# CityU-AIM-Group/HTD

Hardware: AMD Instinct MI355X
Metric: images/sec (1333x800) HTD-R50 train step (higher is better)
Workload: dtype f32; 1 GPU; HTD ResNet-50 FPN fp32 train step fwd+bwd+SGD, batch 4/GPU @ 1333x800 (padded 1344x800), random-init weights, 2000 RPN proposals/img, 512 RoIs/img/stage; global_batch=4, parallelism=dp1, stage2_positives=158, proposals=random-init RPN (few positives: the regression branch is nearly idle)

## Files before the change

htd_amd/csrc/conv_x3.hip:

```cpp
#include <algorithm>
#include <mutex>
#include <type_traits>
#include <unordered_map>

#include <stdlib.h>

#include "common.h"

namespace {

using f32x16 = __attribute__((ext_vector_type(16))) float;
using bf16x8 = __attribute__((ext_vector_type(8))) __bf16;
using bf16x2 = __attribute__((ext_vector_type(2))) __bf16;
using f32x2 = __attribute__((ext_vector_type(2))) float;
using f32x4 = __attribute__((ext_vector_type(4))) float;

using f16x8 = __attribute__((ext_vector_type(8))) _Float16;
using f16x2 = __attribute__((ext_vector_type(2))) _Float16;

constexpr int XK = 16;
constexpr int NCH = 6;

struct H2Scale { float s, inv; };
__device__ __forceinline__ H2Scale h2_scale(const float *amax)
// ... 9 lines not shown
    c.v = __builtin_convertvector(f32x2{a, b}, f16x2);
    h = c.u;
    const f32x2 back = __builtin_convertvector(c.v, f32x2);
    c.v = __builtin_convertvector(f32x2{a - back[0], b - back[1]}, f16x2);
    l = c.u;
}

__device__ __forceinline__ void split3x2(float a, float b, unsigned &h, unsigned &m, unsigned &l)
{
    union { bf16x2 v; unsigned u; } c;
    c.v = __builtin_convertvector(f32x2{a, b}, bf16x2);
    h = c.u;
    const float ra = a - __uint_as_float(h << 16), rb = b - __uint_as_float(h & 0xffff0000u);
    c.v = __builtin_convertvector(f32x2{ra, rb}, bf16x2);
    m = c.u;
    c.v = __builtin_convertvector(f32x2{ra - __uint_as_float(m << 16), rb - __uint_as_float(m & 0xffff0000u)}, bf16x2);
    l = c.u;
}

#ifndef HTD_X3P_EARLY
#define HTD_X3P_EARLY 1
#endif
#ifndef HTD_X3H_NB
#define HTD_X3H_NB 2
#endif
#ifndef HTD_X3H_FRAG_FIRST
#define HTD_X3H_FRAG_FIRST 1
#endif
#ifndef HTD_X3H_OCC4
#define HTD_X3H_OCC4 0
#endif

template <int N>
__device__ __forceinline__ void wait_vm()
{
    asm volatile("s_waitcnt vmcnt(%0)" ::"n"(N) : "memory");
}
__device__ __forceinline__ void landed(f32x4 &a) { asm volatile("" : "+v"(a)::"memory"); }

__device__ __forceinline__ void lds_dma16(const void *src, unsigned lds_dst)
{
    unsigned keep;
    asm volatile("s_mov_b32 %0, m0\n\ts_mov_b32 m0, %2\n\ts_nop 0\n\tglobal_load_lds_dwordx4 %1, off\n\ts_mov_b32 m0, %0"
                 : "=&s"(keep)
                 : "v"(src), "s"(lds_dst)
                 : "memory");
}

using u32x2 = __attribute__((ext_vector_type(2))) unsigned;
template <int OFF>
__device__ __forceinline__ void lds_store8(unsigned addr, unsigned lo, unsigned hi)
{
    const u32x2 v = {lo, hi};
    asm volatile("ds_write_b64 %0, %1 offset:%2" ::"v"(addr), "v"(v), "n"(OFF) : "memory");
}

struct X3Params {
    const float *x;
    const uint4 *wp;
    const float *bias, *residual, *mask_src;
    float *y;
    int Hx, Wx;
    int Ho, Wo;
    int Ci, Co, Cop;
    int kh;
    int stride;
    int ntl;
    int tl_dy[9], tl_dx[9], tl_w[9];
    int o_step, o_h0, o_w0, oH, oW;
    int relu;
    int res_H, res_W;
    float res_sh, res_sw;
    int64_t M;
    int mt, nt;
    int ncs;
    int tiles_a, splits_a, sps_a, splits_b, sps_b;
    int64_t m_rem0;
    float *partial;
    const uint4 *xp;
    uint4 *yp;
    int64_t xp_rows, yp_rows;
    const float *amax, *wscale;
    float *amax_out;
};

__device__ __forceinline__ void block_absmax_out(float mx, float *out, float *red, unsigned seen)
{
    unsigned bits = (mx != mx) ? 0x7fc00000u : __float_as_uint(mx);
    for (int o = 32; o > 0; o >>= 1) bits = max(bits, (unsigned)__shfl_xor((int)bits, o));
    __syncthreads();
    if ((threadIdx.x & 63) == 0) reinterpret_cast<unsigned *>(red)[threadIdx.x >> 6] = bits;
    __syncthreads();
    if (threadIdx.x == 0) {
        const unsigned *r = reinterpret_cast<const unsigned *>(red);
        bits = max(max(r[0], r[1]), max(r[2], r[3]));
        if (bits > seen) __hip_atomic_fetch_max(reinterpret_cast<unsigned *>(out), bits, __ATOMIC_RELAXED, __HIP_MEMORY_SCOPE_AGENT);
    }
}
__device__ __forceinline__ void wave_absmax_out(float mx, float *out, unsigned seen)
{
    unsigned bits = (mx != mx) ? 0x7fc00000u : __float_as_uint(mx);
    for (int o = 32; o > 0; o >>= 1) bits = max(bits, (unsigned)__shfl_xor((int)bits, o));
    if ((threadIdx.x & 63) == 0 && bits > seen)
        __hip_atomic_fetch_max(reinterpret_cast<unsigned *>(out), bits, __ATOMIC_RELAXED, __HIP_MEMORY_SCOPE_AGENT);
}
__device__ __forceinline__ float absmax4(float mx, float4 v)
{
    const float m = fmaxf(fmaxf(fabsf(v.x), fabsf(v.y)), fmaxf(fabsf(v.z), fabsf(v.w)));
    const bool nan = (v.x != v.x) | (v.y != v.y) | (v.z != v.z) | (v.w != v.w);
    return nan ? __uint_as_float(0x7fc00000u) : ((mx != mx) ? mx : fmaxf(mx, m));
}

__device__ __forceinline__ void emit_planes4(uint4 *yp, int64_t rows, int64_t m, int n, float4 v)
{
    unsigned h0, m0, l0, h1, m1, l1;
    split3x2(v.x, v.y, h0, m0, l0);
    split3x2(v.z, v.w, h1, m1, l1);
    char *d = reinterpret_cast<char *>(yp + ((int64_t)(n >> 4) * NCH + ((n >> 3) & 1)) * rows + m) + ((n >> 2) & 1) * 8;
    *reinterpret_cast<uint2 *>(d) = make_uint2(h0, h1);
    *reinterpret_cast<uint2 *>(d + 2 * rows * 16) = make_uint2(m0, m1);
    *reinterpret_cast<uint2 *>(d + 4 * rows * 16) = make_uint2(l0, l1);
}

template <int BM, int KW>
struct Geo {
    static constexpr int RUN = BM + KW - 1;
    static constexpr int PITCH = ((RUN + 1 + 3) / 8) * 8 + 4;
    static constexpr int PASSES = (RUN + 63) / 64;
};

__device__ __forceinline__ int64_t x3_out_off(const X3Params &p, int64_t m, int n)
{
    if (p.o_step == 0) return m * p.Co + n;
    const unsigned mm = (unsigned)m, wo = mm % (unsigned)p.Wo, t = mm / (unsigned)p.Wo;
    const unsigned ho = t % (unsigned)p.Ho, b = t / (unsigned)p.Ho;
    return (((int64_t)b * p.oH + p.o_h0 + p.o_step * (int)ho) * p.oW + p.o_w0 + p.o_step * (int)wo) * p.Co + n;
}

template <int WGM, int WGN, int TM, int TN, bool MF16, typename Acc>
__device__ __forceinline__ void x3_epilogue(const X3Params &p, Acc &acc, uint4 *lds, int64_t m0, int n0, bool part, bool region_b,
                                            int split)
{
    constexpr int BN = WGN * TN * 32;
    constexpr int EPI_STRIDE = BN + 4, EPI_ROWS = WGM * 32;
    constexpr int RBLK = MF16 ? 16 : 32;
    constexpr int CB = TN * 32 / RBLK;
    const int tid = threadIdx.x, lane = tid & 63, wave = tid >> 6;
    const int wm = wave / WGN, wn = wave % WGN;
    const int frow = lane & 31, fhalf = lane >> 5;
    const int lrow = MF16 ? (lane & 15) : frow;
    const int kg = lane >> 4;
    float *le = reinterpret_cast<float *>(lds);
    const bool vec_ok = (p.Co & 3) == 0;
    constexpr int V = BN / 4, RPP = 256 / V;
    float omax = 0.f;
    const unsigned oseen = (p.amax_out != nullptr && !part) ? *reinterpret_cast<const volatile unsigned *>(p.amax_out) : 0u;
    const bool scaled = p.wscale != nullptr;
    float4 cscale = make_float4(1.f, 1.f, 1.f, 1.f);
    if (scaled) {
        const float ia = h2_scale(p.amax).inv;
        const float4 w4 = *reinterpret_cast<const float4 *>(p.wscale + n0 + (tid % V) * 4);
        cscale = make_float4(w4.x * ia, w4.y * ia, w4.z * ia, w4.w * ia);
    }
#pragma unroll
    for (int i = 0; i < TM; ++i) {
        if constexpr (MF16) {
#pragma unroll
            for (int ib = 0; ib < 2; ++ib)
#pragma unroll
                for (int j = 0; j < CB; ++j)
#pragma unroll
                    for (int r = 0; r < 4; ++r)
                        le[(wm * 32 + ib * 16 + 4 * kg + r) * EPI_STRIDE + wn * TN * 32 + j * 16 + lrow] = acc[2 * i + ib][j][r];
        } else {
#pragma unroll
            for (int j = 0; j < TN; ++j)
#pragma unroll
                for (int r = 0; r < 16; ++r) {
                    const int row = wm * 32 + (r & 3) + 8 * (r >> 2) + 4 * fhalf;
                    le[row * EPI_STRIDE + (wn * TN + j) * 32 + frow] = acc[i][j][r];
                }
        }
        __syncthreads();
        const int c4 = tid % V;
        const int n = n0 + c4 * 4;
        constexpr int NPASS = EPI_ROWS / RPP;
        if (vec_ok && !part && p.res_H == 0) {
            const bool col_ok = n < p.Co;
            float4 bv = make_float4(0.f, 0.f, 0.f, 0.f);
            if (p.bias != nullptr && col_ok) bv = *reinterpret_cast<const float4 *>(p.bias + n);
            constexpr int UB = NPASS < 4 ? NPASS : 4;
#pragma unroll
            for (int pass0 = 0; pass0 < NPASS; pass0 += UB) {
                float4 v[UB], rv[UB], mv[UB];
                int64_t o[UB];
                bool ok[UB];
#pragma unroll
                for (int u = 0; u < UB; ++u) {
                    const int row = tid / V + (pass0 + u) * RPP;
                    const int64_t m = m0 + ((row >> 5) * TM + i) * 32 + (row & 31);
                    ok[u] = m < p.M && col_ok;
                    o[u] = x3_out_off(p, ok[u] ? m : 0, n) & -(int64_t)ok[u];
                    v[u] = *reinterpret_cast<const float4 *>(le + row * EPI_STRIDE + c4 * 4);
                    if (scaled) { v[u].x *= cscale.x; v[u].y *= cscale.y; v[u].z *= cscale.z; v[u].w *= cscale.w; }
                }
                if (p.residual != nullptr) {
#pragma unroll
                    for (int u = 0; u < UB; ++u) rv[u] = *reinterpret_cast<const float4 *>(p.residual + o[u]);
                }
                if (p.mask_src != nullptr) {
#pragma unroll
                    for (int u = 0; u < UB; ++u) mv[u] = *reinterpret_cast<const float4 *>(p.mask_src + o[u]);
                }
#pragma unroll
                for (int u = 0; u < UB; ++u) { v[u].x += bv.x; v[u].y += bv.y; v[u].z += bv.z; v[u].w += bv.w; }
                if (p.residual != nullptr) {
#pragma unroll
                    for (int u = 0; u < UB; ++u) { v[u].x += rv[u].x; v[u].y += rv[u].y; v[u].z += rv[u].z; v[u].w += rv[u].w; }
                }
                if (p.relu) {
#pragma unroll
                    for (int u = 0; u < UB; ++u) {
                        v[u].x = fmaxf(v[u].x, 0.f); v[u].y = fmaxf(v[u].y, 0.f); v[u].z = fmaxf(v[u].z, 0.f); v[u].w = fmaxf(v[u].w, 0.f);
                    }
                }
                if (p.mask_src != nullptr) {
#pragma unroll
                    for (int u = 0; u < UB; ++u) {
                        v[u].x = mv[u].x > 0.f ? v[u].x : 0.f; v[u].y = mv[u].y > 0.f ? v[u].y : 0.f;
                        v[u].z = mv[u].z > 0.f ? v[u].z : 0.f; v[u].w = mv[u].w > 0.f ? v[u].w : 0.f;
                    }
                }
#pragma unroll
                for (int u = 0; u < UB; ++u)
                    if (ok[u]) {
                        *reinterpret_cast<float4 *>(p.y + o[u]) = v[u];
                        omax = absmax4(omax, v[u]);
                    }
                if (p.yp != nullptr) {
#pragma unroll
                    for (int u = 0; u < UB; ++u) {
                        const int row = tid / V + (pass0 + u) * RPP;
                        if (ok[u]) emit_planes4(p.yp, p.yp_rows, m0 + ((row >> 5) * TM + i) * 32 + (row & 31), n, v[u]);
                    }
                }
            }
            if (i + 1 < TM) __syncthreads();
            continue;
        }
#pragma unroll
        for (int pass = 0; pass < NPASS; ++pass) {
            const int row = tid / V + pass * RPP;
            const int64_t m = m0 + ((row >> 5) * TM + i) * 32 + (row & 31);
            if (m >= p.M || n >= p.Co) continue;
            float4 v = *reinterpret_cast<const float4 *>(le + row * EPI_STRIDE + c4 * 4);
            if (scaled) { v.x *= cscale.x; v.y *= cscale.y; v.z *= cscale.z; v.w *= cscale.w; }
            const int64_t o = x3_out_off(p, m, n);
            if (part) {
                float *dst = region_b ? p.partial + (p.splits_a > 1 ? (int64_t)p.splits_a * p.m_rem0 * p.Co : 0) +
                                            ((int64_t)split * (p.M - p.m_rem0) + (m - p.m_rem0)) * p.Co + n
                                      : p.partial + ((int64_t)split * p.m_rem0 + m) * p.Co + n;
                if (vec_ok) *reinterpret_cast<float4 *>(dst) = v;
                else {
                    dst[0] = v.x;
                    if (n + 1 < p.Co) dst[1] = v.y;
                    if (n + 2 < p.Co) dst[2] = v.z;
                    if (n + 3 < p.Co) dst[3] = v.w;
                }
                continue;
            }
            if (vec_ok) {
                if (p.bias) {
                    const float4 bv = *reinterpret_cast<const float4 *>(p.bias + n);
                    v.x += bv.x; v.y += bv.y; v.z += bv.z; v.w += bv.w;
                }
                if (p.residual) {
                    int64_t ro = o;
                    if (p.res_H > 0) {
                        const unsigned mm = (unsigned)m, wo = mm % (unsigned)p.Wo, t = mm / (unsigned)p.Wo;
                        const unsigned ho = t % (unsigned)p.Ho, b = t / (unsigned)p.Ho;
                        const int rh = min((int)floorf(ho * p.res_sh), p.res_H - 1);
                        const int rw = min((int)floorf(wo * p.res_sw), p.res_W - 1);
                        ro = (((int64_t)b * p.res_H + rh) * p.res_W + rw) * p.Co + n;
                    }
                    const float4 rv = *reinterpret_cast<const float4 *>(p.residual + ro);
                    v.x += rv.x; v.y += rv.y; v.z += rv.z; v.w += rv.w;
                }
                if (p.relu) { v.x = fmaxf(v.x, 0.f); v.y = fmaxf(v.y, 0.f); v.z = fmaxf(v.z, 0.f); v.w = fmaxf(v.w, 0.f); }
                if (p.mask_src) {
                    const float4 mv = *reinterpret_cast<const float4 *>(p.mask_src + o);
                    v.x = mv.x > 0.f ? v.x : 0.f; v.y = mv.y > 0.f ? v.y : 0.f;
                    v.z = mv.z > 0.f ? v.z : 0.f; v.w = mv.w > 0.f ? v.w : 0.f;
                }
                *reinterpret_cast<float4 *>(p.y + o) = v;
                omax = absmax4(omax, v);
                if (p.yp != nullptr) emit_planes4(p.yp, p.yp_rows, m, n, v);
            } else {
                auto put = [&](int e, float t) {
                    if (n + e >= p.Co) return;
                    t += p.bias ? p.bias[n + e] : 0.f;
                    if (p.residual) t += p.residual[o + e];
                    if (p.relu) t = fmaxf(t, 0.f);
                    if (p.mask_src) t = p.mask_src[o + e] > 0.f ? t : 0.f;
                    p.y[o + e] = t;
                    omax = absmax4(omax, make_float4(t, 0.f, 0.f, 0.f));
                };
                put(0, v.x); put(1, v.y); put(2, v.z); put(3, v.w);
            }
        }
        if (i + 1 < TM) __syncthreads();
    }
    if (p.amax_out != nullptr && !part) block_absmax_out(omax, p.amax_out, le, oseen);
}

template <int WGM, int WGN, int TM, int TN, int KW, int NB, bool H2 = false>
constexpr int x3p_occupancy()
{
    constexpr int BM = WGM * TM * 32, BN = WGN * TN * 32;
    constexpr int NCHL = H2 ? 4 : NCH;
    constexpr int main_bytes = (2 * NCHL * Geo<BM, KW>::PITCH + NB * NCHL * BN) * 16;
    constexpr int epi_bytes = WGM * 32 * (BN + 4) * 4;
    constexpr int by_lds = 163840 / (main_bytes > epi_bytes ? main_bytes : epi_bytes);
    constexpr int by_regs = TM * TN >= 4 ? (H2 && HTD_X3H_OCC4 ? 4 : 3) : 4;
    return by_lds < by_regs ? by_lds : by_regs;
}

template <int WGM, int WGN, int TM, int TN, int KW, bool MF16, int NB, bool H2 = false>
__global__ __launch_bounds__(256, (x3p_occupancy<WGM, WGN, TM, TN, KW, NB, H2>())) void conv_x3p_kernel(X3Params p)
{
    static_assert(!(H2 && MF16), "H2: 32x32x16 form only");
    constexpr int NCHL = H2 ? 4 : NCH;
    constexpr int BM = WGM * TM * 32, BN = WGN * TN * 32;
    using G = Geo<BM, KW>;
    constexpr int PADX = (KW - 1) / 2;
    constexpr int A_VEC = NCHL * G::PITCH;
    constexpr int B_VEC = NCHL * BN;
    constexpr int MAIN_VEC = 2 * A_VEC + NB * B_VEC;
    constexpr int EPI_STRIDE = BN + 4, EPI_ROWS = WGM * 32;
    constexpr int EPI_VEC = EPI_ROWS * EPI_STRIDE / 4;
    constexpr int LDS_VEC = MAIN_VEC > EPI_VEC ? MAIN_VEC : EPI_VEC;
    __shared__ uint4 lds[LDS_VEC];
    uint4 *const lA = lds, *const lB = lds + 2 * A_VEC;
    const unsigned lds_a0 = (unsigned)(size_t)(__attribute__((address_space(3))) void *)lA;

    int bid = blockIdx.x, split = 0, sps = 0;
    bool part = false;
    const bool region_b = bid >= p.tiles_a * p.splits_a;
    if (region_b) {
        const int r = bid - p.tiles_a * p.splits_a;
        bid = p.tiles_a + r / p.splits_b;
        split = r % p.splits_b;
        part = p.splits_b > 1;
        sps = p.sps_b;
    } else if (p.splits_a > 1) {
        split = bid % p.splits_a;
        bid = bid / p.splits_a;
        part = true;
        sps = p.sps_a;
    } else {
        const int q = p.tiles_a / 8, r = p.tiles_a % 8, xcd = bid % 8, idx = bid / 8;
        bid = (xcd < r ? xcd * (q + 1) : r * (q + 1) + (xcd - r) * q) + idx;
    }
    const int tile_m = bid / p.nt, tile_n = bid % p.nt;
    const int64_t m0 = (int64_t)tile_m * BM;
    const int n0 = tile_n * BN;

    const int tid = threadIdx.x, lane = tid & 63, wave = tid >> 6;
    const int wm = wave / WGN, wn = wave % WGN;
    const int frow = lane & 31, fhalf = lane >> 5;
    const int PADY = (p.kh - 1) / 2;

    const int vcol = tid & 3, vrow = tid >> 2;
    const int a_g0 = (int)m0 + vrow - PADX;
    unsigned a_off[KW > 1 ? 1 : G::PASSES];
    bool a_in[KW > 1 ? 1 : G::PASSES];
    unsigned a_tm[KW > 1 ? 1 : G::PASSES];
    if constexpr (KW > 1) {
        a_off[0] = (unsigned)a_g0 * (unsigned)p.Ci + vcol * 4;
        a_in[0] = true;
        a_tm[0] = 0u;
    } else {
#pragma unroll
        for (int i = 0; i < G::PASSES; ++i) {
            const int64_t m = m0 + vrow + 64 * i;
            a_in[i] = vrow + 64 * i < G::RUN && m < p.M;
            const unsigned mm = a_in[i] ? (unsigned)m : 0u;
            const unsigned wo = mm % (unsigned)p.Wo, t = mm / (unsigned)p.Wo;
            const unsigned ho = t % (unsigned)p.Ho, b = t / (unsigned)p.Ho;
            a_off[i] = ((b * (unsigned)p.Hx + ho * (unsigned)p.stride) * (unsigned)p.Wx + wo * (unsigned)p.stride) *
                           (unsigned)p.Ci + vcol * 4;
            unsigned tm = 0x1ffu;
            if (p.ntl > 0) {
                tm = 0u;
                const int hb = (int)(ho * (unsigned)p.stride), wb = (int)(wo * (unsigned)p.stride);
                for (int q = 0; q < p.ntl; ++q)
                    tm |= ((unsigned)(hb + p.tl_dy[q]) < (unsigned)p.Hx && (unsigned)(wb + p.tl_dx[q]) < (unsigned)p.Wx) ? (1u << q) : 0u;
            }
            a_tm[i] = tm;
        }
    }

    constexpr int RBLK = MF16 ? 16 : 32;
    constexpr int RB = TM * 32 / RBLK, CB = TN * 32 / RBLK;
    const int lrow = MF16 ? (lane & 15) : frow;
    const int kg = lane >> 4;
    unsigned vmask[RB];
    const int a_frag0 = (wm * TM * 32 + lrow) * 16;
#pragma unroll
    for (int i = 0; i < RB; ++i) {
        const int r = wm * TM * 32 + i * RBLK + lrow;
        vmask[i] = 0xffffffffu;
// ... 262 lines not shown

    int bbuf = 0, abuf = 0, kx = 0;
    int n1shift = (ky1 - PADY) * p.Wx, n1koff = tap_koff(ky1, cs1);
    int n2shift = (ky2 - PADY) * p.Wx, n2koff = tap_koff(ky2, cs2);
    auto tap = [&](int P, bool TAIL) __attribute__((always_inline)) {
        const bool more = s + 1 < s_end, more2 = s + 2 < s_end;
        if constexpr (H2 && HTD_X3H_FRAG_FIRST) mma_tap(abuf, bbuf, kx, ky * KW, 0);
        const bool issued = issue_b();
        if (!TAIL) {
            if constexpr (KW == 1) {
#pragma unroll
                for (int i = 0; i < NP; ++i) load_pass(ky2, n2koff, i, P * NP + i, more2);
            } else {
                const bool last = kx == KW - 1;
                load_pass(last ? n2shift : n1shift, last ? n2koff : n1koff, last ? 0 : kx + 1, P, last ? more2 : more);
            }
        }
        if constexpr (EARLY) {
            if (TAIL) wait_vm<0>();
            else if (issued) wait_vm<NPT + NI_MIN>();
            else wait_vm<NPT>();
#pragma unroll
            for (int i = 0; i < NPT; ++i) landed(ra[(P ^ 1) * NPT + i]);
            mma_tap(abuf, bbuf, kx, ky * KW, (H2 && HTD_X3H_FRAG_FIRST) ? 1 : 2);
            if constexpr (KW == 1) {
#pragma unroll
                for (int i = 0; i < NP; ++i) store_pass(abuf ^ 1, i, (P ^ 1) * NP + i);
            } else {
                store_pass(abuf ^ 1, kx, P ^ 1);
            }
            constexpr int NM = RB * CB * ((MF16 || H2) ? 3 : 6);
            constexpr int PER = (NPT * 36 + NM - 1) / NM;
            __builtin_amdgcn_sched_group_barrier(0x002, 4, 0);
#pragma unroll
            for (int e = 0; e < NM; ++e) {
                __builtin_amdgcn_sched_group_barrier(0x008, 1, 0);
                __builtin_amdgcn_sched_group_barrier(0x002, PER, 0);
            }
            if (!TAIL) {
                if (DIST >= 2 && issued) wait_vm<NPT + NI_MIN>();
                else wait_vm<NPT>();
            }
        } else {
            mma_tap(abuf, bbuf, kx, ky * KW, (H2 && HTD_X3H_FRAG_FIRST) ? 1 : 2);
            if (TAIL) wait_vm<0>();
            else wait_tap(issued);
#pragma unroll
            for (int i = 0; i < NPT; ++i) landed(ra[(P ^ 1) * NPT + i]);
            if (more) {
                if constexpr (KW == 1) {
#pragma unroll
                    for (int i = 0; i < NP; ++i) store_pass(abuf ^ 1, i, (P ^ 1) * NP + i);
                } else {
                    store_pass(abuf ^ 1, kx, P ^ 1);
                }
            }
        }
        lds_barrier();
        bbuf = bbuf + 1 == NB ? 0 : bbuf + 1;
        if (++kx == KW) {
            kx = 0;
            ++s;
            abuf ^= 1;
            cs = cs1; ky = ky1;
            cs1 = cs2; ky1 = ky2;
            if (++ky2 == p.kh) { ky2 = 0; ++cs2; }
            n1shift = n2shift; n1koff = n2koff;
            n2shift = (ky2 - PADY) * p.Wx;
            n2koff = tap_koff(ky2, cs2);
        }
    };
    const int taps_total = (s_end - s_begin) * KW;
    int t = 0;
#pragma unroll 1
    for (; t + 1 < taps_total; t += 2) {
        tap(0, false);
        tap(1, false);
    }
    if (t < taps_total) tap(0, true);
    wait_vm<0>();
#pragma unroll
    for (int i = 0; i < 2 * NPT; ++i) landed(ra[i]);

    x3_epilogue<WGM, WGN, TM, TN, MF16>(p, acc, lds, m0, n0, part, region_b, split);
}

template <int WGM, int WGN, int TM, int TN, int NS>
constexpr int x3q_occupancy()
{
    constexpr int BM = WGM * TM * 32, BN = WGN * TN * 32;
    constexpr int main_bytes = NS * NCH * (BM + BN) * 16;
    constexpr int epi_bytes = WGM * 32 * (BN + 4) * 4;
    constexpr int by_lds = 163840 / (main_bytes > epi_bytes ? main_bytes : epi_bytes);
    constexpr int by_regs = TM * TN >= 4 ? 3 : 4;
    return by_lds < by_regs ? by_lds : by_regs;
}

template <int WGM, int WGN, int TM, int TN, bool MF16, int NS>
__global__ __launch_bounds__(256, (x3q_occupancy<WGM, WGN, TM, TN, NS>())) void conv_x3q_kernel(X3Params p)
{
    constexpr int BM = WGM * TM * 32, BN = WGN * TN * 32;
    constexpr int A_VEC = NCH * BM, B_VEC = NCH * BN;
    constexpr int MAIN_VEC = NS * (A_VEC + B_VEC);
    constexpr int EPI_VEC = WGM * 32 * (BN + 4) / 4;
    constexpr int LDS_VEC = MAIN_VEC > EPI_VEC ? MAIN_VEC : EPI_VEC;
    __shared__ uint4 lds[LDS_VEC];
    uint4 *const lA = lds, *const lB = lds + NS * A_VEC;
    const unsigned lds_a0 = (unsigned)(size_t)(__attribute__((address_space(3))) void *)lA;
    const unsigned lds_b0 = (unsigned)(size_t)(__attribute__((address_space(3))) void *)lB;

    int bid = blockIdx.x, split = 0, sps = 0;
    bool part = false;
    const bool region_b = bid >= p.tiles_a * p.splits_a;
    if (region_b) {
        const int r = bid - p.tiles_a * p.splits_a;
        bid = p.tiles_a + r / p.splits_b;
        split = r % p.splits_b;
        part = p.splits_b > 1;
        sps = p.sps_b;
    } else if (p.splits_a > 1) {
        split = bid % p.splits_a;
        bid = bid / p.splits_a;
        part = true;
        sps = p.sps_a;
    } else {
        const int q = p.tiles_a / 8, r = p.tiles_a % 8, xcd = bid % 8, idx = bid / 8;
        bid = (xcd < r ? xcd * (q + 1) : r * (q + 1) + (xcd - r) * q) + idx;
    }
    const int tile_m = bid / p.nt, tile_n = bid % p.nt;
    const int64_t m0 = (int64_t)tile_m * BM;
    const int n0 = tile_n * BN;

    const int tid = threadIdx.x, lane = tid & 63, wave = tid >> 6;
    const int wm = wave / WGN, wn = wave % WGN;
    const int frow = lane & 31, fhalf = lane >> 5;
    constexpr int RBLK = MF16 ? 16 : 32;
    constexpr int RB = TM * 32 / RBLK, CB = TN * 32 / RBLK;
    const int lrow = MF16 ? (lane & 15) : frow;
    const int kg = lane >> 4;
    const int a_row = (wm * TM * 32 + lrow) * 16;
    const int a_c0 = (MF16 ? kg * BM * 16 : fhalf * BM * 16) + a_row;
    const int a_c1 = MF16 ? ((kg >> 1) * 4 + (kg & 1)) * BM * 16 + a_row : 0;
    const int b_row = (wn * TN * 32 + lrow) * 16;
    const int b_c0 = (MF16 ? kg * BN * 16 : fhalf * BN * 16) + b_row;
    const int b_c1 = MF16 ? ((1 - (kg >> 1)) * 2 + (kg & 1)) * BN * 16 + b_row : 0;
    const int b_c2 = MF16 ? (((kg >> 1) ? 0 : 4) + (kg & 1)) * BN * 16 + b_row : 0;

    const int total_steps = p.ncs;
    const int s_begin = part ? split * sps : 0;
    const int s_end = part ? min(total_steps, s_begin + sps) : total_steps;

    constexpr int NIA = NCH * BM / 64, NIB = NCH * BN / 64, NI = NIA + NIB, NIW = (NI + 3) / 4;
    const int wave_u = __builtin_amdgcn_readfirstlane(wave);
    const uint4 *src[NIW];
    unsigned dst[NIW], adv[NIW];
#pragma unroll
    for (int k = 0; k < NIW; ++k) {
        const int idx = wave_u + 4 * k;
        if (idx < NIA) {
            const int chunk = idx / (BM / 64), half = idx % (BM / 64);
            src[k] = p.xp + (int64_t)chunk * p.xp_rows + m0 + half * 64 + lane;
            dst[k] = lds_a0 + (unsigned)((chunk * BM + half * 64) * 16);
            adv[k] = (unsigned)(NCH * p.xp_rows);
        } else {
            const int j = (idx < NI ? idx : NIA) - NIA, chunk = j / (BN / 64), half = j % (BN / 64);
            src[k] = p.wp + (int64_t)chunk * p.Cop + n0 + half * 64 + lane;
            dst[k] = lds_b0 + (unsigned)((chunk * BN + half * 64) * 16);
            adv[k] = (unsigned)(NCH * p.Cop);
        }
    }
    auto issue = [&](int s, int stage) __attribute__((always_inline)) {
#pragma unroll
        for (int k = 0; k < NIW; ++k) {
            const int idx = wave_u + 4 * k;
            if (NI % 4 != 0 && idx >= NI) continue;
            const unsigned st = (unsigned)stage * (unsigned)((idx < NIA ? A_VEC : B_VEC) * 16);
            lds_dma16(src[k] + (int64_t)s * adv[k], dst[k] + st);
        }
    };
    auto lds_barrier = [&]() {
        asm volatile("s_waitcnt lgkmcnt(0)" ::: "memory");
        __builtin_amdgcn_s_barrier();
        asm volatile("" ::: "memory");
    };

    using acc_t = typename std::conditional<MF16, f32x4, f32x16>::type;
    acc_t acc[RB][CB];
#pragma unroll
    for (int i = 0; i < RB; ++i)
#pragma unroll
        for (int j = 0; j < CB; ++j)
#pragma unroll
            for (int r = 0; r < (MF16 ? 4 : 16); ++r) acc[i][j][r] = 0.f;

    auto mma = [&](int stage) __attribute__((always_inline)) {
        const char *la = reinterpret_cast<const char *>(lA + stage * A_VEC);
        const char *lb = reinterpret_cast<const char *>(lB + stage * B_VEC);
        if constexpr (MF16) {
            bf16x8 fa01[RB], fa02[RB];
#pragma unroll
            for (int i = 0; i < RB; ++i) {
                fa01[i] = *reinterpret_cast<const bf16x8 *>(la + a_c0 + i * 16 * 16);
                fa02[i] = *reinterpret_cast<const bf16x8 *>(la + a_c1 + i * 16 * 16);
            }
#pragma unroll
            for (int j = 0; j < CB; ++j) {
                const bf16x8 fb01 = *reinterpret_cast<const bf16x8 *>(lb + b_c0 + j * 16 * 16);
                const bf16x8 fb10 = *reinterpret_cast<const bf16x8 *>(lb + b_c1 + j * 16 * 16);
                const bf16x8 fb20 = *reinterpret_cast<const bf16x8 *>(lb + b_c2 + j * 16 * 16);
#pragma unroll
                for (int i = 0; i < RB; ++i) {
                    acc[i][j] = __builtin_amdgcn_mfma_f32_16x16x32_bf16(fa02[i], fb20, acc[i][j], 0, 0, 0);
                    acc[i][j] = __builtin_amdgcn_mfma_f32_16x16x32_bf16(fa01[i], fb10, acc[i][j], 0, 0, 0);
                    acc[i][j] = __builtin_amdgcn_mfma_f32_16x16x32_bf16(fa01[i], fb01, acc[i][j], 0, 0, 0);
                }
            }
        } else {
            bf16x8 fa[RB][3], fb[CB][3];
#pragma unroll
            for (int i = 0; i < RB; ++i)
#pragma unroll
                for (int q = 0; q < 3; ++q) fa[i][q] = *reinterpret_cast<const bf16x8 *>(la + a_c0 + i * 32 * 16 + q * 2 * BM * 16);
#pragma unroll
            for (int j = 0; j < CB; ++j)
#pragma unroll
                for (int q = 0; q < 3; ++q) fb[j][q] = *reinterpret_cast<const bf16x8 *>(lb + b_c0 + j * 32 * 16 + q * 2 * BN * 16);
#pragma unroll
            for (int i = 0; i < RB; ++i)
#pragma unroll
                for (int j = 0; j < CB; ++j) {
                    acc[i][j] = __builtin_amdgcn_mfma_f32_32x32x16_bf16(fa[i][2], fb[j][0], acc[i][j], 0, 0, 0);
                    acc[i][j] = __builtin_amdgcn_mfma_f32_32x32x16_bf16(fa[i][0], fb[j][2], acc[i][j], 0, 0, 0);
                    acc[i][j] = __builtin_amdgcn_mfma_f32_32x32x16_bf16(fa[i][1], fb[j][1], acc[i][j], 0, 0, 0);
                    acc[i][j] = __builtin_amdgcn_mfma_f32_32x32x16_bf16(fa[i][1], fb[j][0], acc[i][j], 0, 0, 0);
                    acc[i][j] = __builtin_amdgcn_mfma_f32_32x32x16_bf16(fa[i][0], fb[j][1], acc[i][j], 0, 0, 0);
                    acc[i][j] = __builtin_amdgcn_mfma_f32_32x32x16_bf16(fa[i][0], fb[j][0], acc[i][j], 0, 0, 0);
                }
        }
    };

    constexpr int KEEP = (NS - 2) * (NI / 4);
#pragma unroll
    for (int d = 0; d < NS - 1; ++d)
        if (s_begin + d < s_end) issue(s_begin + d, d);
    if (s_begin + NS - 2 < s_end) wait_vm<KEEP>();
    else wait_vm<0>();
    lds_barrier();
    int stage = 0, pstage = NS - 1;
#pragma unroll 1
    for (int s = s_begin; s < s_end; ++s) {
        const bool more = s + NS - 1 < s_end;
        if (more) issue(s + NS - 1, pstage);
        mma(stage);
        if (more) wait_vm<KEEP>();
        else wait_vm<0>();
        lds_barrier();
        stage = stage + 1 == NS ? 0 : stage + 1;
        pstage = pstage + 1 == NS ? 0 : pstage + 1;
    }
    x3_epilogue<WGM, WGN, TM, TN, MF16>(p, acc, lds, m0, n0, part, region_b, split);
}

__global__ __launch_bounds__(256) void conv_x3p_splitk_epilogue_kernel(X3Params p)
{
    const int64_t lo = p.splits_a > 1 ? 0 : p.m_rem0 * p.Co, hi = p.splits_b > 1 ? p.M * p.Co : p.m_rem0 * p.Co;
    const int64_t na = p.m_rem0 * p.Co, nb = (p.M - p.m_rem0) * p.Co;
    const float *pb = p.partial + (p.splits_a > 1 ? (int64_t)p.splits_a * na : 0);
    float omax = 0.f;
    const unsigned oseen = p.amax_out != nullptr ? *reinterpret_cast<const volatile unsigned *>(p.amax_out) : 0u;
    for (int64_t o = lo + (int64_t)blockIdx.x * blockDim.x + threadIdx.x; o < hi; o += (int64_t)gridDim.x * blockDim.x) {
        float v = 0.f;
        if (o < na) {
            for (int k = 0; k < p.splits_a; ++k) v += p.partial[(int64_t)k * na + o];
        } else {
            for (int k = 0; k < p.splits_b; ++k) v += pb[(int64_t)k * nb + (o - na)];
        }
        const int n = (int)(o % p.Co);
        if (p.bias) v += p.bias[n];
        if (p.residual) {
            int64_t ro = p.o_step == 0 ? o : x3_out_off(p, o / p.Co, n);
            if (p.res_H > 0) {
                const int64_t m = o / p.Co;
                const unsigned mm = (unsigned)m, wo = mm % (unsigned)p.Wo, t = mm / (unsigned)p.Wo;
                const unsigned ho = t % (unsigned)p.Ho, b = t / (unsigned)p.Ho;
                const int rh = min((int)floorf(ho * p.res_sh), p.res_H - 1);
                const int rw = min((int)floorf(wo * p.res_sw), p.res_W - 1);
                ro = (((int64_t)b * p.res_H + rh) * p.res_W + rw) * p.Co + n;
            }
            v += p.residual[ro];
        }
        if (p.relu) v = fmaxf(v, 0.f);
        const int64_t oo = p.o_step == 0 ? o : x3_out_off(p, o / p.Co, n);
        if (p.mask_src) v = p.mask_src[oo] > 0.f ? v : 0.f;
        p.y[oo] = v;
        omax = absmax4(omax, make_float4(v, 0.f, 0.f, 0.f));
    }
    __shared__ float ored[4];
    if (p.amax_out != nullptr) block_absmax_out(omax, p.amax_out, ored, oseen);
}

__global__ __launch_bounds__(256) void conv_x3p_splitk_epilogue_vec_kernel(X3Params p)
{
    const int C4 = p.Co >> 2;
    const int64_t lo = p.splits_a > 1 ? 0 : p.m_rem0 * C4, hi = p.splits_b > 1 ? p.M * C4 : p.m_rem0 * C4;
    const int64_t na = p.m_rem0 * C4, nb = (p.M - p.m_rem0) * C4;
    const float4 *pa = reinterpret_cast<const float4 *>(p.partial);
    const float4 *pb = pa + (p.splits_a > 1 ? (int64_t)p.splits_a * na : 0);
    float omax = 0.f;
    const unsigned oseen = p.amax_out != nullptr ? *reinterpret_cast<const volatile unsigned *>(p.amax_out) : 0u;
    for (int64_t q = lo + (int64_t)blockIdx.x * blockDim.x + threadIdx.x; q < hi; q += (int64_t)gridDim.x * blockDim.x) {
        float4 v = make_float4(0.f, 0.f, 0.f, 0.f);
        const bool in_a = q < na;
        const float4 *src = in_a ? pa + q : pb + (q - na);
        const int64_t stride = in_a ? na : nb;
        const int splits = in_a ? p.splits_a : p.splits_b;
#pragma unroll 4
        for (int k = 0; k < splits; ++k) {
            const float4 t = src[(int64_t)k * stride];
            v.x += t.x; v.y += t.y; v.z += t.z; v.w += t.w;
        }
        const unsigned m = (unsigned)(q / C4), n = (unsigned)(q - (int64_t)m * C4) * 4u;
        const int64_t o = x3_out_off(p, (int64_t)m, (int)n);
        if (p.bias) {
            const float4 bv = *reinterpret_cast<const float4 *>(p.bias + n);
            v.x += bv.x; v.y += bv.y; v.z += bv.z; v.w += bv.w;
        }
        if (p.residual) {
            int64_t ro = o;
            if (p.res_H > 0) {
                const unsigned wo = m % (unsigned)p.Wo, t = m / (unsigned)p.Wo;
                const unsigned ho = t % (unsigned)p.Ho, b = t / (unsigned)p.Ho;
                const int rh = min((int)floorf(ho * p.res_sh), p.res_H - 1);
                const int rw = min((int)floorf(wo * p.res_sw), p.res_W - 1);
                ro = (((int64_t)b * p.res_H + rh) * p.res_W + rw) * p.Co + n;
            }
            const float4 rv = *reinterpret_cast<const float4 *>(p.residual + ro);
            v.x += rv.x; v.y += rv.y; v.z += rv.z; v.w += rv.w;
        }
        if (p.relu) { v.x = fmaxf(v.x, 0.f); v.y = fmaxf(v.y, 0.f); v.z = fmaxf(v.z, 0.f); v.w = fmaxf(v.w, 0.f); }
        if (p.mask_src) {
            const float4 mv = *reinterpret_cast<const float4 *>(p.mask_src + o);
            v.x = mv.x > 0.f ? v.x : 0.f; v.y = mv.y > 0.f ? v.y : 0.f;
            v.z = mv.z > 0.f ? v.z : 0.f; v.w = mv.w > 0.f ? v.w : 0.f;
        }
        *reinterpret_cast<float4 *>(p.y + o) = v;
        omax = absmax4(omax, v);
        if (p.yp != nullptr) emit_planes4(p.yp, p.yp_rows, (int64_t)m, (int)n, v);
    }
    __shared__ float ored[4];
    if (p.amax_out != nullptr) block_absmax_out(omax, p.amax_out, ored, oseen);
}

__device__ __forceinline__ void x3_planes_element(const float *__restrict__ w, uint4 *__restrict__ out, int Co, int taps,
                                                  int Ci, int Np, int transposed, int64_t e)
{
    const int N = transposed ? Ci : Co, K = transposed ? Co : Ci;
    const int ncs = K / XK;
    const int n = (int)(e % Np);
    const int64_t t2 = e / Np;
    const int cs = (int)(t2 % ncs), tap = (int)(t2 / ncs);
    float v[XK];
    if (n < N) {
        if (!transposed) {
            const float4 *src = reinterpret_cast<const float4 *>(w + ((int64_t)n * taps + tap) * Ci + cs * XK);
#pragma unroll
            for (int q = 0; q < 4; ++q) {
                const float4 f = src[q];
                v[4 * q] = f.x; v[4 * q + 1] = f.y; v[4 * q + 2] = f.z; v[4 * q + 3] = f.w;
            }
        } else {
#pragma unroll
            for (int k = 0; k < XK; ++k) v[k] = w[((int64_t)(cs * XK + k) * taps + (taps - 1 - tap)) * Ci + n];
        }
    } else {
#pragma unroll
        for (int k = 0; k < XK; ++k) v[k] = 0.f;
    }
    unsigned pl[3][8];
#pragma unroll
    for (int k = 0; k < 8; ++k) split3x2(v[2 * k], v[2 * k + 1], pl[0][k], pl[1][k], pl[2][k]);
    uint4 *dst = out + ((int64_t)(tap * ncs + cs) * NCH) * Np + n;
#pragma unroll
    for (int q = 0; q < 3; ++q)
#pragma unroll
        for (int h = 0; h < 2; ++h)
            dst[(int64_t)(q * 2 + h) * Np] = make_uint4(pl[q][4 * h], pl[q][4 * h + 1], pl[q][4 * h + 2], pl[q][4 * h + 3]);
}

__global__ __launch_bounds__(256) void x3_planes_kernel(const float *__restrict__ w, uint4 *__restrict__ out, int Co, int taps,
                                                        int Ci, int Np, int transposed)
{
    const int K = transposed ? Co : Ci;
    const int64_t total = (int64_t)taps * (K / XK) * Np;
    for (int64_t e = (int64_t)blockIdx.x * 256 + threadIdx.x; e < total; e += (int64_t)gridDim.x * 256)
        x3_planes_element(w, out, Co, taps, Ci, Np, transposed, e);
}

struct PlanesDesc {
    const float *w;
    uint4 *out;
    int Co, taps, Ci, transposed;
    int64_t block0;
};

__global__ __launch_bounds__(256) void x3_planes_many_kernel(const PlanesDesc *__restrict__ descs, int n)
{
    int lo = 0, hi = n - 1;
    const int64_t b = blockIdx.x;
// ... 344 lines not shown
    if (g_xtable.empty()) return -1;
    const auto it = g_xtable.find(XKey{M, Co, Ci, taps, epi});
    return it == g_xtable.end() ? -1 : it->second;
}

int choose_cfg(int64_t M, int Co, int Ci, int taps, int epi)
{
    int cfg = forced_cfg();
    if (cfg < 0) cfg = table_cfg(M, Co, Ci, taps, epi);
    if (cfg >= 0) return cfg;
    float best = -1.f;
    static const int cand[4] = {1, 3, 2, 0};
    for (int c : cand) {
        const float sc = cfg_score(c, M, Co);
        if (sc > best * 1.005f) { best = sc; cfg = c; }
    }
    return cfg;
}

static const int g_x3p_mfma = getenv("HTD_X3P_MFMA") ? atoi(getenv("HTD_X3P_MFMA")) : 0;
int x3p_mfma()
{
    if (!g_x3p_tune) return g_x3p_mfma;
    const char *e = getenv("HTD_X3P_MFMA");
    return e ? atoi(e) : 0;
}

int x3p_nb()
{
    if (!g_x3p_tune) return 0;
    const char *e = getenv("HTD_X3P_NB");
    return e ? atoi(e) : 0;
}

template <int TM, int TN, int NB>
void launch_tile_nb(const X3Params &p, int kw, dim3 grid, hipStream_t s)
{
    const int mf = x3p_mfma() ? x3p_mfma() : (kw == 1 ? 16 : 32);
    if (mf == 32) {
        if (kw == 1) hipLaunchKernelGGL((conv_x3p_kernel<2, 2, TM, TN, 1, false, NB>), grid, dim3(256), 0, s, p);
        else hipLaunchKernelGGL((conv_x3p_kernel<2, 2, TM, TN, 3, false, NB>), grid, dim3(256), 0, s, p);
    } else {
        if (kw == 1) hipLaunchKernelGGL((conv_x3p_kernel<2, 2, TM, TN, 1, true, NB>), grid, dim3(256), 0, s, p);
        else hipLaunchKernelGGL((conv_x3p_kernel<2, 2, TM, TN, 3, true, NB>), grid, dim3(256), 0, s, p);
    }
}

template <int TM, int TN>
void launch_tile(const X3Params &p, int kw, dim3 grid, hipStream_t s)
{
#ifdef HTD_X3P_DEEP
    const int nb = x3p_nb();
    if (nb == 3) return launch_tile_nb<TM, TN, 3>(p, kw, grid, s);
    if (nb >= 4) return launch_tile_nb<TM, TN, 4>(p, kw, grid, s);
#endif
    launch_tile_nb<TM, TN, 2>(p, kw, grid, s);
}

static const int g_x3q_mfma = getenv("HTD_X3Q_MFMA") ? atoi(getenv("HTD_X3Q_MFMA")) : 0;
static const int g_x3q_ns = getenv("HTD_X3Q_NS") ? atoi(getenv("HTD_X3Q_NS")) : 0;
int x3q_env(const char *name, int at_load)
{
    if (!g_x3p_tune) return at_load;
    const char *e = getenv(name);
    return e ? atoi(e) : 0;
}

template <int TM, int TN>
void launch_tile_q(const X3Params &p, dim3 grid, hipStream_t s)
{
    const int mf = x3q_env("HTD_X3Q_MFMA", g_x3q_mfma), ns = x3q_env("HTD_X3Q_NS", g_x3q_ns);
    if (mf != 32) {
        if (ns == 3) hipLaunchKernelGGL((conv_x3q_kernel<2, 2, TM, TN, true, 3>), grid, dim3(256), 0, s, p);
        else hipLaunchKernelGGL((conv_x3q_kernel<2, 2, TM, TN, true, 2>), grid, dim3(256), 0, s, p);
    } else {
        if (ns == 3) hipLaunchKernelGGL((conv_x3q_kernel<2, 2, TM, TN, false, 3>), grid, dim3(256), 0, s, p);
        else hipLaunchKernelGGL((conv_x3q_kernel<2, 2, TM, TN, false, 2>), grid, dim3(256), 0, s, p);
    }
}

int launch_x3p(X3Params p, int kw, hipStream_t s, void *workspace)
{
    const int total_steps = p.ncs * p.kh;
    const int epi = (p.residual ? 1 : 0) | (p.mask_src ? 2 : 0) | (p.amax ? 4 : 0);
    const int cfg = choose_cfg(p.M, p.Co, p.Ci, p.kh * kw + (p.ntl > 0 ? 100 : 0), epi);
    const XPlan pl = plan_x3p(cfg, p.M, p.Co, total_steps, kw, workspace != nullptr);
    p.tiles_a = pl.tiles_a; p.splits_a = pl.splits_a; p.sps_a = pl.sps_a; p.splits_b = pl.splits_b; p.sps_b = pl.sps_b;
    p.m_rem0 = pl.m_rem0;
    p.partial = (float *)workspace;
    p.mt = (int)htd::ceil_div(p.M, kXCfg[cfg].bm);
    p.nt = (int)htd::ceil_div(p.Co, kXCfg[cfg].bn);
    HTD_REQUIRE(pl.grid > 0 && pl.grid < (1ll << 31), "conv2d_x3p: bad grid");
    const dim3 grid((unsigned)pl.grid);
    if (p.amax != nullptr && kw == 3) {
        switch (cfg) {
        case 0: hipLaunchKernelGGL((conv_x3p_kernel<2, 2, 1, 1, 3, false, HTD_X3H_NB, true>), grid, dim3(256), 0, s, p); break;
        case 1: hipLaunchKernelGGL((conv_x3p_kernel<2, 2, 2, 2, 3, false, HTD_X3H_NB, true>), grid, dim3(256), 0, s, p); break;
        case 2: hipLaunchKernelGGL((conv_x3p_kernel<2, 2, 2, 1, 3, false, HTD_X3H_NB, true>), grid, dim3(256), 0, s, p); break;
        default: hipLaunchKernelGGL((conv_x3p_kernel<2, 2, 1, 2, 3, false, HTD_X3H_NB, true>), grid, dim3(256), 0, s, p); break;
        }
    } else if (p.amax != nullptr) {
        switch (cfg) {
        case 0: hipLaunchKernelGGL((conv_x3p_kernel<2, 2, 1, 1, 1, false, HTD_X3H_NB, true>), grid, dim3(256), 0, s, p); break;
        case 1: hipLaunchKernelGGL((conv_x3p_kernel<2, 2, 2, 2, 1, false, HTD_X3H_NB, true>), grid, dim3(256), 0, s, p); break;
        case 2: hipLaunchKernelGGL((conv_x3p_kernel<2, 2, 2, 1, 1, false, HTD_X3H_NB, true>), grid, dim3(256), 0, s, p); break;
        default: hipLaunchKernelGGL((conv_x3p_kernel<2, 2, 1, 2, 1, false, HTD_X3H_NB, true>), grid, dim3(256), 0, s, p); break;
        }
    } else if (p.xp != nullptr) {
        switch (cfg) {
        case 0: launch_tile_q<1, 1>(p, grid, s); break;
        case 1: launch_tile_q<2, 2>(p, grid, s); break;
        case 2: launch_tile_q<2, 1>(p, grid, s); break;
        default: launch_tile_q<1, 2>(p, grid, s); break;
        }
    } else {
        switch (cfg) {
        case 0: launch_tile<1, 1>(p, kw, grid, s); break;
        case 1: launch_tile<2, 2>(p, kw, grid, s); break;
        case 2: launch_tile<2, 1>(p, kw, grid, s); break;
        default: launch_tile<1, 2>(p, kw, grid, s); break;
        }
    }
    if (pl.partial_floats > 0) {
        const int64_t rows = (p.splits_a > 1 ? p.m_rem0 : 0) + (p.splits_b > 1 ? p.M - p.m_rem0 : 0);
        if ((p.Co & 3) == 0) {
            const unsigned rb = (unsigned)std::min<int64_t>(htd::ceil_div(rows * (p.Co >> 2), 256), p.amax_out ? 1024 : 4096);
            hipLaunchKernelGGL(conv_x3p_splitk_epilogue_vec_kernel, dim3(rb), dim3(256), 0, s, p);
        } else {
            const unsigned rb = (unsigned)std::min<int64_t>(htd::ceil_div(rows * p.Co, 256), p.amax_out ? 1024 : 4096);
            hipLaunchKernelGGL(conv_x3p_splitk_epilogue_kernel, dim3(rb), dim3(256), 0, s, p);
        }
    }
    return htd::check_launch("conv2d_x3p");
}

bool x3h_strided_ok(int Ci, int Co, int kh, int kw, int stride, int pad)
{
    static const bool on = !(getenv("HTD_X3H_STRIDED") && atoi(getenv("HTD_X3H_STRIDED")) == 0);
    return on && Ci % XK == 0 && Co >= 33 && kh == 3 && kw == 3 && stride == 2 && pad == 1;
}

bool x3p_shape_ok(int Ci, int Co, int kh, int kw, int stride, int pad, int dil)
{
    if (Ci % XK != 0 || Co < 33 || dil != 1 || kh != kw) return false;
    if (kh == 1) return pad == 0 && stride >= 1;
    return kh == 3 && stride == 1 && pad == 1;
}

}

extern "C" int htd_conv2d_x3p_supported(int Ci, int Co, int kh, int kw, int stride, int pad, int dil)
{
    return (!x3p_off() && htd::conv_math() == 1 && x3p_shape_ok(Ci, Co, kh, kw, stride, pad, dil)) ? 1 : 0;
}

int g_conv_h2 = getenv("HTD_CONV_H2") ? atoi(getenv("HTD_CONV_H2")) : 1;
extern "C" int htd_conv2d_set_h2(int on)
{
    const int prev = g_conv_h2;
    if (on == 0 || on == 1) g_conv_h2 = on;
    return prev;
}
extern "C" int htd_conv2d_x3h_supported(int Ci, int Co, int kh, int kw, int stride, int pad, int dil)
{
    return (g_conv_h2 == 1 && htd_conv2d_x3p_supported(Ci, Co, kh, kw, stride, pad, dil)) ? 1 : 0;
}
extern "C" int htd_conv2d_x3h_strided_supported(int Ci, int Co, int kh, int kw, int stride, int pad, int dil)
{
    return (g_conv_h2 == 1 && !x3p_off() && htd::conv_math() == 1 && dil == 1 && x3h_strided_ok(Ci, Co, kh, kw, stride, pad)) ? 1 : 0;
}

extern "C" int htd_conv2d_x3p_tile_table_set(int64_t M, int Co, int Ci, int taps, int epi, int cfg)
{
    HTD_REQUIRE(M > 0 && Co > 0 && Ci > 0 && taps > 0 && epi >= 0 && epi < 8 && cfg < 4,
                "x3p_tile_table_set: bad entry M=%lld Co=%d Ci=%d taps=%d epi=%d cfg=%d", (long long)M, Co, Ci, taps, epi, cfg);
    std::lock_guard<std::mutex> lock(g_xtable_mutex);
    if (cfg < 0) g_xtable.erase(XKey{M, Co, Ci, taps, epi});
// ... 72 lines not shown
                       (const PlanesDescH *)desc, n);
    return htd::check_launch("x3h_planes_many");
}

extern "C" int htd_absmax(const float *x, int64_t n, float *amax, void *stream)
{
    HTD_REQUIRE(x && amax && n > 0 && ((uintptr_t)x & 15) == 0, "absmax: bad arguments");
    const unsigned blocks = (unsigned)std::min<int64_t>(htd::ceil_div(n >> 2, (int64_t)256 * 8) + 1, 2048);
    hipLaunchKernelGGL(absmax_kernel, dim3(blocks), dim3(256), 0, (hipStream_t)stream, x, n, (unsigned *)amax);
    return htd::check_launch("absmax");
}

extern "C" int htd_conv2d_x3_planes_many(const void *desc, int n, int64_t total_blocks, void *stream)
{
    static_assert(sizeof(PlanesDesc) == 40, "PlanesDesc layout is part of the ABI");
    HTD_REQUIRE(desc && n > 0 && total_blocks > 0 && total_blocks < (1ll << 31), "x3_planes_many: bad arguments");
    hipLaunchKernelGGL(x3_planes_many_kernel, dim3((unsigned)total_blocks), dim3(256), 0, (hipStream_t)stream,
                       (const PlanesDesc *)desc, n);
    return htd::check_launch("x3_planes_many");
}

extern "C" int64_t htd_conv2d_x3p_workspace_bytes(int64_t M, int Co, int Ci, int kh, int kw)
{
    int64_t need = 0;
    for (int cfg = 0; cfg < 4; ++cfg) need = std::max(need, plan_x3p(cfg, M, Co, (Ci / XK) * kh, kw, true).partial_floats * 4);
    return need;
}

extern "C" int64_t htd_act_planes_rows(int64_t M) { return M > 0 ? act_rows(M) : 0; }

extern "C" int64_t htd_act_planes_bytes(int64_t M, int C)
{
    if (M <= 0 || C <= 0 || C % XK != 0) return 0;
    return (int64_t)(C / XK) * NCH * act_rows(M) * 16;
}

extern "C" int htd_act_planes(const float *x, void *planes, int64_t M, int C, void *stream)
{
    HTD_REQUIRE(x && planes && M > 0 && C > 0 && C % XK == 0, "act_planes: bad arguments (C %% 16)");
    const unsigned blocks = (unsigned)std::min<int64_t>(htd::ceil_div(M * (C >> 3), (int64_t)256), 65536);
    hipLaunchKernelGGL(act_planes_kernel, dim3(blocks), dim3(256), 0, (hipStream_t)stream, x, (uint4 *)planes, M, C, act_rows(M));
    return htd::check_launch("act_planes");
}

extern "C" int htd_conv2d_fwd_x3q(const float *x, const void *xplanes, const void *wplanes, const float *bias,
                                  const float *residual, int res_h, int res_w, float *y, void *yplanes, float *amax_out, int B, int H,
                                  int W, int Ci, int Co, int kh, int kw, int stride, int pad, int relu, void *workspace, void *stream)
{
    HTD_REQUIRE((x || xplanes) && wplanes && y && B > 0 && H > 0 && W > 0, "conv2d_fwd_x3q: bad arguments");
    HTD_REQUIRE(x3p_shape_ok(Ci, Co, kh, kw, stride, pad, 1), "conv2d_fwd_x3q: unsupported layer Ci=%d Co=%d k=%dx%d s=%d p=%d", Ci,
                Co, kh, kw, stride, pad);
    HTD_REQUIRE(!xplanes || (kh == 1 && stride == 1), "conv2d_fwd_x3q: input planes serve 1x1 / stride-1 layers only");
    HTD_REQUIRE(!yplanes || Co % XK == 0, "conv2d_fwd_x3q: output planes need Co %% 16 == 0 (Co=%d)", Co);
    HTD_REQUIRE((res_h > 0) == (res_w > 0) && res_h >= 0 && (res_h == 0 || ((Co & 3) == 0 && residual)),
                "conv2d_fwd_x3q: bad residual up-sampling arguments");
    X3Params p{};
    p.x = x; p.wp = (const uint4 *)wplanes; p.bias = bias; p.residual = residual; p.y = y;
    p.Hx = H; p.Wx = W;
    p.Ho = (H + 2 * pad - kh) / stride + 1;
    p.Wo = (W + 2 * pad - kw) / stride + 1;
    p.Ci = Ci; p.Co = Co; p.Cop = planes_np(Co); p.kh = kh; p.stride = stride; p.relu = relu;
    p.M = (int64_t)B * p.Ho * p.Wo;
    p.ncs = Ci / XK;
    p.xp = (const uint4 *)xplanes; p.xp_rows = act_rows(p.M);
    p.yp = (uint4 *)yplanes; p.yp_rows = act_rows(p.M);
    p.amax_out = amax_out;
    HTD_REQUIRE((int64_t)B * H * W * Ci < (1ll << 31) && p.M * Co < (1ll << 40), "conv2d_fwd_x3q: operand too large");
    if (res_h > 0) {
        p.res_H = res_h; p.res_W = res_w;
        p.res_sh = (float)res_h / (float)p.Ho; p.res_sw = (float)res_w / (float)p.Wo;
    }
    return launch_x3p(p, kw, (hipStream_t)stream, workspace);
}

extern "C" int htd_conv2d_fwd_x3p(const float *x, const void *wplanes, const float *bias, const float *residual, int res_h,
                                  int res_w, float *y, int B, int H, int W, int Ci, int Co, int kh, int kw, int stride, int pad,
                                  int relu, void *workspace, void *stream)
{
    HTD_REQUIRE(x, "conv2d_fwd_x3p: bad arguments");
    return htd_conv2d_fwd_x3q(x, nullptr, wplanes, bias, residual, res_h, res_w, y, nullptr, nullptr, B, H, W, Ci, Co, kh, kw, stride,
                              pad, relu, workspace, stream);
}

extern "C" int htd_conv2d_bwd_data_x3q(const float *gy, const void *gyplanes, const void *wplanesT, const float *mask_src,
                                       const float *accum, float *gx, void *gxplanes, float *amax_out, int B, int H, int W, int Ci,
                                       int Co, int kh, int kw, int pad, void *workspace, void *stream)
{
    HTD_REQUIRE((gy || gyplanes) && wplanesT && gx && B > 0 && H > 0 && W > 0, "conv2d_bwd_data_x3q: bad arguments");
    HTD_REQUIRE(x3p_shape_ok(Co, Ci, kh, kw, 1, pad, 1), "conv2d_bwd_data_x3q: unsupported layer Ci=%d Co=%d k=%dx%d p=%d", Ci, Co,
                kh, kw, pad);
    HTD_REQUIRE(!gyplanes || kh == 1, "conv2d_bwd_data_x3q: gradient planes serve 1x1 layers only");
    HTD_REQUIRE(!gxplanes || Ci % XK == 0, "conv2d_bwd_data_x3q: output planes need Ci %% 16 == 0 (Ci=%d)", Ci);
    X3Params p{};
    p.x = gy; p.wp = (const uint4 *)wplanesT; p.residual = accum; p.mask_src = mask_src; p.y = gx;
    p.Hx = H; p.Wx = W; p.Ho = H; p.Wo = W;
    p.Ci = Co; p.Co = Ci; p.Cop = planes_np(Ci); p.kh = kh; p.stride = 1;
    p.M = (int64_t)B * H * W;
    p.ncs = Co / XK;
    p.xp = (const uint4 *)gyplanes; p.xp_rows = act_rows(p.M);
    p.yp = (uint4 *)gxplanes; p.yp_rows = act_rows(p.M);
    p.amax_out = amax_out;
    HTD_REQUIRE((int64_t)B * H * W * Co < (1ll << 31), "conv2d_bwd_data_x3q: operand too large");
    return launch_x3p(p, kw, (hipStream_t)stream, workspace);
}

extern "C" int htd_conv2d_bwd_data_x3p(const float *gy, const void *wplanesT, const float *mask_src, const float *accum,
                                       float *gx, int B, int H, int W, int Ci, int Co, int kh, int kw, int pad, void *workspace,
                                       void *stream)
{
    HTD_REQUIRE(gy, "conv2d_bwd_data_x3p: bad arguments");
    return htd_conv2d_bwd_data_x3q(gy, nullptr, wplanesT, mask_src, accum, gx, nullptr, nullptr, B, H, W, Ci, Co, kh, kw, pad,
                                   workspace, stream);
}

extern "C" int htd_conv2d_fwd_x3h(const float *x, const float *amax, const void *wplanes, const float *bias, const float *residual,
                                  int res_h, int res_w, float *y, void *yplanes, float *amax_out, int B, int H, int W, int Ci,
                                  int Co, int kh, int kw, int stride, int pad, int relu, void *workspace, void *stream)
{
    HTD_REQUIRE(!yplanes || Co % XK == 0, "conv2d_fwd_x3h: output planes need Co %% 16 == 0 (Co=%d)", Co);
    HTD_REQUIRE(x && amax && wplanes && y && B > 0 && H > 0 && W > 0, "conv2d_fwd_x3h: bad arguments");
    const bool taps = x3h_strided_ok(Ci, Co, kh, kw, stride, pad);
    HTD_REQUIRE(taps || x3p_shape_ok(Ci, Co, kh, kw, stride, pad, 1), "conv2d_fwd_x3h: unsupported layer Ci=%d Co=%d k=%dx%d s=%d p=%d",
                Ci, Co, kh, kw, stride, pad);
    HTD_REQUIRE(!taps || (!yplanes && res_h == 0), "conv2d_fwd_x3h: strided 3x3 layers write no planes and take no up-sampled residual");
    HTD_REQUIRE((res_h > 0) == (res_w > 0) && res_h >= 0 && (res_h == 0 || ((Co & 3) == 0 && residual)),
                "conv2d_fwd_x3h: bad residual up-sampling arguments");
    X3Params p{};
    p.x = x; p.wp = (const uint4 *)wplanes; p.bias = bias; p.residual = residual; p.y = y;
    p.Hx = H; p.Wx = W;
    p.Ho = (H + 2 * pad - kh) / stride + 1;
    p.Wo = (W + 2 * pad - kw) / stride + 1;
    p.Ci = Ci; p.Co = Co; p.Cop = planes_np(Co); p.kh = kh; p.stride = stride; p.relu = relu;
    p.M = (int64_t)B * p.Ho * p.Wo;
    p.ncs = Ci / XK;
    p.amax = amax;
    p.wscale = reinterpret_cast<const float *>(p.wp + planes_vec(kh * kw, Ci, p.Cop));
    p.yp = (uint4 *)yplanes; p.yp_rows = act_rows(p.M);
    p.amax_out = amax_out;
    HTD_REQUIRE((int64_t)B * H * W * Ci < (1ll << 31) && p.M * Co < (1ll << 40), "conv2d_fwd_x3h: operand too large");
    if (res_h > 0) {
        p.res_H = res_h; p.res_W = res_w;
        p.res_sh = (float)res_h / (float)p.Ho; p.res_sw = (float)res_w / (float)p.Wo;
    }
    if (taps) {
        p.kh = p.ntl = kh * kw;
        for (int t = 0; t < p.ntl; ++t) { p.tl_dy[t] = t / kw - pad; p.tl_dx[t] = t % kw - pad; p.tl_w[t] = t; }
        return launch_x3p(p, 1, (hipStream_t)stream, workspace);
    }
    return launch_x3p(p, kw, (hipStream_t)stream, workspace);
}

extern "C" int htd_conv2d_bwd_data_x3h(const float *gy, const float *amax, const void *wplanesT, const float *mask_src,
                                       const float *accum, float *gx, void *gxplanes, float *amax_out, int B, int H, int W,
                                       int Ci, int Co, int kh, int kw, int pad, void *workspace, void *stream)
{
    HTD_REQUIRE(!gxplanes || Ci % XK == 0, "conv2d_bwd_data_x3h: output planes need Ci %% 16 == 0 (Ci=%d)", Ci);
    HTD_REQUIRE(gy && amax && wplanesT && gx && B > 0 && H > 0 && W > 0, "conv2d_bwd_data_x3h: bad arguments");
    HTD_REQUIRE(x3p_shape_ok(Co, Ci, kh, kw, 1, pad, 1), "conv2d_bwd_data_x3h: unsupported layer Ci=%d Co=%d k=%dx%d p=%d", Ci, Co, kh,
                kw, pad);
    X3Params p{};
    p.x = gy; p.wp = (const uint4 *)wplanesT; p.residual = accum; p.mask_src = mask_src; p.y = gx;
    p.Hx = H; p.Wx = W; p.Ho = H; p.Wo = W;
    p.Ci = Co; p.Co = Ci; p.Cop = planes_np(Ci); p.kh = kh; p.stride = 1;
    p.M = (int64_t)B * H * W;
    p.ncs = Co / XK;
    p.amax = amax;
    p.wscale = reinterpret_cast<const float *>(p.wp + planes_vec(kh * kw, Co, p.Cop));
    p.yp = (uint4 *)gxplanes; p.yp_rows = act_rows(p.M);
    p.amax_out = amax_out;
    HTD_REQUIRE((int64_t)B * H * W * Co < (1ll << 31), "conv2d_bwd_data_x3h: operand too large");
    return launch_x3p(p, kw, (hipStream_t)stream, workspace);
}

namespace {
struct StridedClass { int ntaps; int dy[9], dx[9], w[9]; int Ho, Wo; };
int strided_classes(int H, int W, int kh, int kw, int stride, int pad, StridedClass *cls)
{
    int n = 0;
    for (int c = 0; c < stride * stride; ++c) {
        const int ph = c / stride, pw = c % stride;
        StridedClass &q = cls[c];
        q.ntaps = 0;
        q.Ho = ph < H ? (H - ph + stride - 1) / stride : 0;
        q.Wo = pw < W ? (W - pw + stride - 1) / stride : 0;
        if (q.Ho == 0 || q.Wo == 0) continue;
        for (int ky = 0; ky < kh; ++ky) {
            const int ry = ph + pad - ky;
            if (((ry % stride) + stride) % stride != 0) continue;
            for (int kx = 0; kx < kw; ++kx) {
                const int rx = pw + pad - kx;
                if (((rx % stride) + stride) % stride != 0) continue;
                q.dy[q.ntaps] = ry >= 0 ? ry / stride : -((-ry) / stride);
                q.dx[q.ntaps] = rx >= 0 ? rx / stride : -((-rx) / stride);
                q.w[q.ntaps] = (kh - 1 - ky) * kw + (kw - 1 - kx);
                ++q.ntaps;
            }
        }
        n += q.ntaps > 0;
    }
    return n;
}
bool x3h_strided_dgrad_ok(int Ci, int Co, int kh, int kw, int stride, int pad)
{
    static const bool on = !(getenv("HTD_X3H_STRIDED") && atoi(getenv("HTD_X3H_STRIDED")) == 0);
    return on && Co % XK == 0 && Ci >= 33 && stride == 2 && ((kh == 3 && kw == 3 && pad == 1) || (kh == 1 && kw == 1 && pad == 0));
}
}

extern "C" int htd_conv2d_bwd_data_x3h_strided_supported(int Ci, int Co, int kh, int kw, int stride, int pad, int dil)
{
    return (g_conv_h2 == 1 && !x3p_off() && htd::conv_math() == 1 && dil == 1 && x3h_strided_dgrad_ok(Ci, Co, kh, kw, stride, pad)) ? 1 : 0;
}

extern "C" int64_t htd_conv2d_bwd_data_x3h_strided_workspace_bytes(int B, int H, int W, int Ci, int Co, int kh, int kw, int stride, int pad)
{
    if (!x3h_strided_dgrad_ok(Ci, Co, kh, kw, stride, pad) || B <= 0 || H <= 0 || W <= 0) return 0;
    StridedClass cls[4];
    strided_classes(H, W, kh, kw, stride, pad, cls);
    int64_t need = 0;
    for (int c = 0; c < stride * stride; ++c)
        if (cls[c].ntaps > 0)
            need = std::max(need, htd_conv2d_x3p_workspace_bytes((int64_t)B * cls[c].Ho * cls[c].Wo, Ci, Co, cls[c].ntaps, 1));
    return need;
}

extern "C" int htd_conv2d_bwd_data_x3h_strided(const float *gy, const float *amax, const void *wplanesT, const float *mask_src,
                                               float *gx, float *amax_out, int B, int H, int W, int Ci, int Co, int kh, int kw,
                                               int stride, int pad, void *workspace, void *stream)
{
    HTD_REQUIRE(gy && amax && wplanesT && gx && B > 0 && H > 0 && W > 0, "conv2d_bwd_data_x3h_strided: bad arguments");
    HTD_REQUIRE(x3h_strided_dgrad_ok(Ci, Co, kh, kw, stride, pad), "conv2d_bwd_data_x3h_strided: unsupported layer Ci=%d Co=%d k=%dx%d s=%d p=%d",
                Ci, Co, kh, kw, stride, pad);
    const int Ho = (H + 2 * pad - kh) / stride + 1, Wo = (W + 2 * pad - kw) / stride + 1;
    HTD_REQUIRE(Ho > 0 && Wo > 0 && (int64_t)B * Ho * Wo * Co < (1ll << 31) && (int64_t)B * H * W * Ci < (1ll << 40),
                "conv2d_bwd_data_x3h_strided: bad sizes");
    StridedClass cls[4];
    const int live = strided_classes(H, W, kh, kw, stride, pad, cls);
    if (live < stride * stride) {
        if (hipMemsetAsync(gx, 0, (size_t)B * H * W * Ci * 4, (hipStream_t)stream) != hipSuccess) {
            htd::set_error("conv2d_bwd_data_x3h_strided: memset failed");
            return HTD_ERR_LAUNCH;
        }
    }
    X3Params p{};
    p.x = gy; p.wp = (const uint4 *)wplanesT; p.mask_src = mask_src; p.y = gx;
    p.Hx = Ho; p.Wx = Wo;
    p.Ci = Co; p.Co = Ci; p.Cop = planes_np(Ci); p.stride = 1;
    p.ncs = Co / XK;
    p.amax = amax;
    p.wscale = reinterpret_cast<const float *>(p.wp + planes_vec(kh * kw, Co, p.Cop));
    p.amax_out = amax_out;
    p.o_step = stride; p.oH = H; p.oW = W;
    for (int c = 0; c < stride * stride; ++c) {
        const StridedClass &q = cls[c];
        if (q.ntaps == 0) continue;
        X3Params r = p;
        r.Ho = q.Ho; r.Wo = q.Wo;
        r.M = (int64_t)B * q.Ho * q.Wo;
        r.kh = r.ntl = q.ntaps;
        for (int t = 0; t < q.ntaps; ++t) { r.tl_dy[t] = q.dy[t]; r.tl_dx[t] = q.dx[t]; r.tl_w[t] = q.w[t]; }
        r.o_h0 = c / stride; r.o_w0 = c % stride;
        const int st = launch_x3p(r, 1, (hipStream_t)stream, workspace);
        if (st) return st;
    }
    return HTD_OK;
}
```

htd_amd/dense.py:

```python
import os

import torch
from torch.autograd import Function
from torch.autograd.function import once_differentiable
from torch.multiprocessing.reductions import StorageWeakRef as _StorageWeakRef

from . import capi
from .mmcv_ops import chain_outputs

CL = torch.channels_last
_P = capi.ptr
_S = capi.current_stream_ptr


def _out_hw(H, W, kh, kw, stride, pad, dil):
    return ((H + 2 * pad - (dil * (kh - 1) + 1)) // stride + 1, (W + 2 * pad - (dil * (kw - 1) + 1)) // stride + 1)


def _need_gpu(t, name):
    if not t.is_cuda:
        raise NotImplementedError(f'{name}: only GPU tensors are supported (libhtd_amd.so has no CPU path)')


def _splitk_ws(M, Co, Cred, kh, kw, device):
# ... 198 lines not shown


def _x3h_ok(Cred, Cout, kh, kw, stride, padding, dilation, dtype):
    return dtype == torch.float32 and (kh == 3 or H2_1X1) and \
        bool(capi.lib().htd_conv2d_x3h_supported(Cred, Cout, kh, kw, stride, padding, dilation))


def _amax_slot(device):
    ent = _AMAX_POOL.get(device.index)
    if ent is None or ent[1] >= _AMAX_SLOTS:
        ent = [torch.zeros(_AMAX_SLOTS, device=device, dtype=torch.float32), 0]
        _AMAX_POOL[device.index] = ent
    slot = ent[0][ent[1]:ent[1] + 1]
    ent[1] += 1
    return slot


def absmax(x):
    slot = _amax_slot(x.device)
    capi.call('htd_absmax', _P(x), x.numel(), _P(slot), _S(), work=('byte', 4.0 * x.numel()))
    return slot


H2_GUARD = H2_CHECK or os.environ.get('HTD_H2_GUARD', '0') == '1'
_H2_LAUNCHES = []


def _h2_guard(am_in, out_slot):
    if H2_GUARD and out_slot is not None:
        _H2_LAUNCHES.append((am_in, out_slot))


def h2_check(device=None):
    pairs, _H2_LAUNCHES[:] = list(_H2_LAUNCHES), []
    if not pairs:
        return
    a = torch.cat([p[0].reshape(1) for p in pairs])
    b = torch.cat([p[1].reshape(1) for p in pairs])
    bad = torch.isfinite(a) & ~torch.isfinite(b)
    if bool(bad.any()):
        i = int(torch.nonzero(bad)[0])
        raise RuntimeError(f'htd_amd: H2 convolution launch {i} of {len(pairs)} was given a maximum ({float(a[i])}) smaller than its input '
                           'tensor holds (stale _htd_amax): its output contains infinities')


H2_TRACE = {} if os.environ.get('HTD_H2_TRACE', '0') == '1' else None


def _h2_trace(what, t, weight):
    if H2_TRACE is not None:
        import traceback
        fr = [f for f in traceback.extract_stack(limit=12) if 'dense.py' not in f.filename]
        key = (what, tuple(t.shape), tuple(weight.shape), f'{os.path.basename(fr[-1].filename)}:{fr[-1].lineno}' if fr else '?',
               'grad_fn' if t.grad_fn is not None else ('attr-stale' if hasattr(t, '_htd_amax') else 'no-attr'))
        H2_TRACE[key] = H2_TRACE.get(key, 0) + 1


H2_VIEWS = os.environ.get('HTD_H2_VIEWS', '1') != '0'
_AMAX_BY_PTR = {}


def _dense_layout(t):
    if t.is_contiguous() or (t.dim() == 4 and t.is_contiguous(memory_format=CL)):
        return True
    want = 1
    for size, stride in sorted(((sz, st) for sz, st in zip(t.shape, t.stride()) if sz != 1), key=lambda p: p[1]):
        if stride != want:
            return False
        want *= size
    return True


def tag_amax(t, slot):
    t._htd_amax = (slot, t.data_ptr(), t.numel(), t._version)
    if H2_VIEWS:
        st = t.untyped_storage()
        _AMAX_BY_PTR[t.data_ptr()] = (slot, t.numel(), t._version, st._cdata, _StorageWeakRef(st))


def drop_amax(t):
    if t is not None:
        if hasattr(t, '_htd_amax'):
            del t._htd_amax
        _AMAX_BY_PTR.pop(t.data_ptr(), None)


def carried_amax(t):
    a = getattr(t, '_htd_amax', None)
    if a is None and H2_VIEWS:
        e = _AMAX_BY_PTR.get(t.data_ptr())
        if e is not None and e[1] == t.numel() and e[2] == t._version and not e[4].expired() and \
                t.untyped_storage()._cdata == e[3] and _dense_layout(t):
            a = (e[0], t.data_ptr(), e[1], e[2])
    if a is None or a[1] != t.data_ptr() or a[2] != t.numel() or a[3] != t._version:
        return None
    if H2_CHECK:
        fresh = absmax(t)
        if not torch.equal(fresh, a[0]) and not (torch.isnan(fresh).item() and torch.isnan(a[0]).item()):
            raise RuntimeError(f'stale carried maximum: {float(a[0])} against {float(fresh)} on a tensor of shape {tuple(t.shape)}')
    return a[0]


_STEP_PLANES = {}


def _planes_key(w, transposed):
    return _flip_key(w) + (bool(transposed), )


_ALSO_WANTED = set()


def _planes_h2(w, transposed):
    Co, Ci, kh, kw = w.shape
    cred, cout = (Co, Ci) if transposed else (Ci, Co)
    return kh == kw and _x3h_ok(cred, cout, kh, kw, 1, kh // 2, 1, w.dtype)


def x3_planes(weight, transposed, h2=None):
    if h2 is None:
        h2 = _planes_h2(weight, transposed)
    key = _planes_key(weight, transposed) + (bool(h2), )
    hit = _STEP_PLANES.get(key)
    if hit is not None:
        return hit[1]
    _ALSO_WANTED.add((tuple(weight.shape), bool(transposed), bool(h2)))
    Co, Ci, kh, kw = weight.shape
    nbytes = capi.lib().htd_conv2d_x3_planes_bytes(Co, kh, kw, Ci, int(transposed))
    planes = torch.empty(nbytes // 4, device=weight.device, dtype=torch.int32)
    capi.call('htd_conv2d_x3h_planes' if h2 else 'htd_conv2d_x3_planes', _P(weight), _P(planes), Co, kh, kw, Ci, int(transposed), _S())
    _STEP_PLANES[key] = (weight, planes)
    return planes


def _planes_wanted(w, transposed):
    Co, Ci, kh, kw = w.shape
    cred, cout = (Co, Ci) if transposed else (Ci, Co)
    return w.is_cuda and w.dtype == torch.float32 and kh == kw and kh in (1, 3) and w.is_contiguous(memory_format=CL) and \
        bool(capi.lib().htd_conv2d_x3p_supported(cred, cout, kh, kw, 1, kh // 2, 1))


def planes_many(items):
    import numpy as np
    todo, seen = [], set()
    for w, tr in items:
        w4 = w if w.dim() == 4 else w.view(w.size(0), w.size(1), 1, 1)
        if not _planes_wanted(w4, tr):
            continue
        h2 = _planes_h2(w4, tr)
        for v in ((h2, ) if (tuple(w4.shape), bool(tr), not h2) not in _ALSO_WANTED else (h2, not h2)):
            key = _planes_key(w4, tr) + (v, )
            if key not in _STEP_PLANES and key not in seen:
                seen.add(key)
                todo.append((key, w4, tr))
    if not todo:
        return
    L = capi.lib()
    dev = todo[0][1].device
    for h2 in (False, True):
        part = [t for t in todo if t[0][-1] == h2]
        if not part:
            continue
        sizes = [L.htd_conv2d_x3_planes_bytes(w.size(0), w.size(2), w.size(3), w.size(1), int(tr)) // 4 for _, w, tr in part]
        flat = torch.empty(sum(sizes), device=dev, dtype=torch.int32)
        desc = np.zeros((len(part), 6 if h2 else 5), dtype=np.int64)
        off = block0 = row0 = 0
        for i, ((key, w, tr), n32) in enumerate(zip(part, sizes)):
# ... 149 lines not shown
                  _P(ws), _S(), key='htd_conv2d_fwd_x3p', work=work)
        if out_slot is not None:
            tag_amax(y, out_slot)
        return (y, yp) if emit else y
    work = ('flop', flops, 4.0 * (x.numel() + weight.numel() + y.numel() + (y.numel() if residual is not None else 0)))
    if x.dtype == torch.float32 and rh == 0 and \
            capi.lib().htd_conv2d_x3h_strided_supported(Ci, Co, kh, kw, stride, padding, dilation):
        am = carried_amax(x)
        if am is None:
            _h2_trace('fwd', x, weight)
            if kh * kw * Co >= H2_ABSMAX_MIN_WORK and x.numel() >= H2_ABSMAX_MIN_ELEMS:
                am = absmax(x)
        if am is not None:
            nb = capi.lib().htd_conv2d_x3p_workspace_bytes(B * Ho * Wo, Co, Ci, kh * kw, 1)
            ws = torch.empty(nb // 4, device=x.device, dtype=torch.float32) if nb > 0 else None
            out_slot = _amax_slot(x.device)
            capi.call('htd_conv2d_fwd_x3h', _P(x), _P(am), _P(x3_planes(weight, False, True)), _P(bias), _P(residual), 0, 0, _P(y), None,
                      _P(out_slot), B, H, W, Ci, Co, kh, kw, stride, padding, int(bool(relu)), _P(ws), _S(), work=work)
            tag_amax(y, out_slot)
            _h2_guard(am, out_slot)
            return y
    if _igemm_emits(y, Co):
        slot = _amax_slot(x.device)
        capi.call('htd_conv2d_fwd_amax', _P(x), _P(weight), _P(bias), _P(residual), rh, rw, _P(y), _P(slot), B, H, W, Ci, Co, kh, kw,
                  stride, padding, dilation, int(bool(relu)), _P(_splitk_ws(B * Ho * Wo, Co, Ci, kh, kw, x.device)), _S(),
                  key='htd_conv2d_fwd', work=work)
        tag_amax(y, slot)
        return y
    capi.call('htd_conv2d_fwd', _P(x), _P(weight), _P(bias), _P(residual), rh, rw, _P(y), B, H, W, Ci, Co, kh, kw, stride,
              padding, dilation, int(bool(relu)), _P(_splitk_ws(B * Ho * Wo, Co, Ci, kh, kw, x.device)), _S(), work=work)
    return y


def _igemm_emits(y, C):
    return y.dtype == torch.float32 and C >= 64 and emits('igemm')


def _colsum_raw(g, y=None, bias=None):
    B, Co, Ho, Wo = g.shape
    gm = torch.empty_like(g, memory_format=CL) if y is not None else g
    gb = grad_out(bias) if bias is not None else torch.empty(Co, device=g.device, dtype=g.dtype)
    if g.numel() == 0:
        return gm, gb.zero_()
    ws = torch.empty(2048 * Co, device=g.device, dtype=g.dtype)
    work = ('byte', 4.0 * B * Ho * Wo * Co * (3 if y is not None else 1))
    if _mask_emits(g):
        slot = _amax_slot(g.device)
        capi.call('htd_bias_grad_relu_mask_amax', _P(g), _P(y), _P(gm) if y is not None else None, _P(gb), B * Ho * Wo, Co,
                  _P(ws), _P(slot), _S(), key='htd_bias_grad_relu_mask', work=work)
        tag_amax(gm, slot)
    else:
        capi.call('htd_bias_grad_relu_mask', _P(g), _P(y), _P(gm) if y is not None else None, _P(gb), B * Ho * Wo, Co,
                  _P(ws), _S(), work=work)
    return gm, gb


H2_EMIT_OFF = frozenset(v for v in os.environ.get('HTD_H2_EMIT_OFF', '').split(',') if v)


def emits(kind):
    return kind not in H2_EMIT_OFF and capi.lib().htd_conv2d_set_h2(-1) == 1


def _mask_emits(g):
    return g.dtype == torch.float32 and emits('mask')


def _mask_raw(g, y):
    B, Co, Ho, Wo = g.shape
    gm = torch.empty_like(g, memory_format=CL)
    if g.numel() == 0:
        return gm
    if _mask_emits(g):
        slot = _amax_slot(g.device)
        capi.call('htd_bias_grad_relu_mask_amax', _P(g), _P(y), _P(gm), None, B * Ho * Wo, Co, None, _P(slot), _S(),
                  key='htd_bias_grad_relu_mask', work=('byte', 12.0 * B * Ho * Wo * Co))
        tag_amax(gm, slot)
    else:
        capi.call('htd_bias_grad_relu_mask', _P(g), _P(y), _P(gm), None, B * Ho * Wo, Co, None, _S(),
                  work=('byte', 12.0 * B * Ho * Wo * Co))
    return gm


def _dgrad_raw(g, weight, x_shape, stride, padding, dilation, mask_src=None, accum=None, wT=None, g_planes=None, emit=None):
    gx = _dgrad_raw_(g, weight, x_shape, stride, padding, dilation, mask_src, accum, wT, g_planes, bool(emit))
    if emit is not None:
        return gx if isinstance(gx, tuple) else (gx, None)
    return gx


def _dgrad_raw_(g, weight, x_shape, stride, padding, dilation, mask_src, accum, wT, g_planes, emit):
    B, Ci, H, W = x_shape
    Co, _, kh, kw = weight.shape
    Ho, Wo = g.shape[2], g.shape[3]
    if B == 0:
        return torch.empty((0, Ci, H, W), device=g.device, dtype=g.dtype, memory_format=CL)
    if stride == 1 and _x3p_ok(Co, Ci, kh, kw, 1, padding, dilation, g.dtype):
        gx = torch.empty((B, Ci, H, W), device=g.device, dtype=g.dtype, memory_format=CL)
        nb = capi.lib().htd_conv2d_x3p_workspace_bytes(B * H * W, Ci, Co, kh, kw)
        ws = torch.empty(nb // 4, device=g.device, dtype=torch.float32) if nb > 0 else None
        use_gp = g_planes is not None and kh == 1
        gxp = _act_planes_buf(B * H * W, Ci, g.device) if (emit and Ci % 16 == 0) else None
        work = ('flop', 2.0 * B * Ho * Wo * Co * kh * kw * Ci,
                4.0 * (g.numel() + weight.numel() + gx.numel() * (1 + (mask_src is not None) + (accum is not None))))
        h2 = _x3h_ok(Co, Ci, kh, kw, 1, padding, dilation, g.dtype)
        out_slot = _amax_slot(g.device) if h2 else None
        if h2:
            am = carried_amax(g)
            if am is None:
                _h2_trace('dgrad', g, weight)
            if am is None and kh * kw * Ci >= H2_ABSMAX_MIN_WORK and g.numel() >= H2_ABSMAX_MIN_ELEMS:
                am = absmax(g)
            if am is not None:
                capi.call('htd_conv2d_bwd_data_x3h', _P(g), _P(am), _P(x3_planes(weight, True, True)), _P(mask_src), _P(accum), _P(gx),
                          _P(gxp), _P(out_slot), B, H, W, Ci, Co, kh, kw, padding, _P(ws), _S(), work=work)
                tag_amax(gx, out_slot)
                _h2_guard(am, out_slot)
                return (gx, gxp) if emit else gx
        capi.call('htd_conv2d_bwd_data_x3q', _P(g), _P(g_planes) if use_gp else None, _P(x3_planes(weight, True, False)), _P(mask_src),
                  _P(accum), _P(gx), _P(gxp), _P(out_slot), B, H, W, Ci, Co, kh, kw, padding, _P(ws), _S(),
                  key='htd_conv2d_bwd_data_x3p', work=work)
        if out_slot is not None:
            tag_amax(gx, out_slot)
        return (gx, gxp) if emit else gx
    if stride != 1 and accum is None and g.dtype == torch.float32 and \
            capi.lib().htd_conv2d_bwd_data_x3h_strided_supported(Ci, Co, kh, kw, stride, padding, dilation):
        am = carried_amax(g)
        if am is None:
            _h2_trace('dgrad', g, weight)
            if kh * kw * Ci >= H2_ABSMAX_MIN_WORK and g.numel() >= H2_ABSMAX_MIN_ELEMS:
                am = absmax(g)
        if am is not None:
            gx = torch.empty((B, Ci, H, W), device=g.device, dtype=g.dtype, memory_format=CL)
            nb = capi.lib().htd_conv2d_bwd_data_x3h_strided_workspace_bytes(B, H, W, Ci, Co, kh, kw, stride, padding)
            ws = torch.empty(nb // 4, device=g.device, dtype=torch.float32) if nb > 0 else None
            out_slot = _amax_slot(g.device)
            capi.call('htd_conv2d_bwd_data_x3h_strided', _P(g), _P(am), _P(x3_planes(weight, True, True)), _P(mask_src), _P(gx),
                      _P(out_slot), B, H, W, Ci, Co, kh, kw, stride, padding, _P(ws), _S(), key='htd_conv2d_bwd_data_x3h',
                      work=('flop', 2.0 * B * Ho * Wo * Co * kh * kw * Ci,
                            4.0 * (g.numel() + weight.numel() + gx.numel() * (1 + (mask_src is not None)))))
            tag_amax(gx, out_slot)
            _h2_guard(am, out_slot)
            return gx
    gd, Cod = g, Co
    if Co % 8 != 0:
        Cod = Co + (-Co) % 8
        gd = torch.empty((B, Cod, Ho, Wo), device=g.device, dtype=g.dtype, memory_format=CL)
        if gd.numel():
            capi.call('htd_pad_channels', _P(g), _P(gd), B * Ho * Wo, Co, Cod, _S())
    if wT is None or Cod != Co:
        key = _flip_key(weight)
        hit = _STEP_FLIPS.get(key) if Cod == Co else None
        wT = hit[1] if hit is not None else None
        if wT is None:
            wT = torch.empty(Ci * kh * kw * Cod, device=g.device, dtype=g.dtype)
            if Cod != Co:
                capi.call('htd_conv2d_flip_weights_padded', _P(weight), _P(wT), Co, Cod, kh, kw, Ci, _S())
            else:
                capi.call('htd_conv2d_flip_weights', _P(weight), _P(wT), Co, kh, kw, Ci, _S())
                _STEP_FLIPS[key] = (weight, wT)
    gx = torch.empty((B, Ci, H, W), device=g.device, dtype=g.dtype, memory_format=CL)
    work = ('flop', 2.0 * B * Ho * Wo * Co * kh * kw * Ci,
            4.0 * (g.numel() + weight.numel() + gx.numel() * (1 + (mask_src is not None) + (accum is not None))))
    if _igemm_emits(gx, Ci):
        slot = _amax_slot(g.device)
        capi.call('htd_conv2d_bwd_data_amax', _P(gd), _P(wT), _P(mask_src), _P(accum), _P(gx), _P(slot), B, H, W, Ci, Cod, kh, kw,
                  stride, padding, dilation, _P(_splitk_ws(B * H * W, Ci, Cod, kh, kw, g.device)), _S(),
                  key='htd_conv2d_bwd_data', work=work)
        tag_amax(gx, slot)
        return gx
    capi.call('htd_conv2d_bwd_data', _P(gd), _P(wT), _P(mask_src), _P(accum), _P(gx), B, H, W, Ci, Cod, kh, kw, stride,
              padding, dilation, _P(_splitk_ws(B * H * W, Ci, Cod, kh, kw, g.device)), _S(), work=work)
    return gx


SINK_ACCUMULATE = os.environ.get('HTD_SINK_ACC', '1') != '0'


H2_WGRAD = os.environ.get('HTD_H2_WGRAD', '1') != '0'


def _wgrad_amax(x, g, weight, stride, padding, dilation):
    if not H2_WGRAD or x.dtype != torch.float32:
        return None
    B, Ci, H, W = x.shape
    Co, _, kh, kw = weight.shape
    if B * g.size(2) * g.size(3) == 0 or \
            not capi.lib().htd_conv2d_bwd_weight_h2_supported(B, H, W, Ci, Co, kh, kw, stride, padding, dilation):
        return None
    ax, ag = carried_amax(x), carried_amax(g)
    if ax is None:
        _h2_trace('wgrad x', x, weight)
    if ag is None:
        _h2_trace('wgrad g', g, weight)
    if (ax is None and (kh * kw * Co < H2_ABSMAX_MIN_WORK or x.numel() < H2_ABSMAX_MIN_ELEMS)) or \
            (ag is None and (kh * kw * Ci < H2_ABSMAX_MIN_WORK or g.numel() < H2_ABSMAX_MIN_ELEMS)):
        return None
    return (ax if ax is not None else absmax(x)), (ag if ag is not None else absmax(g))


def _wgrad_launch(x, g, weight, stride, padding, dilation, bias, amax=None):
    B, Ci, H, W = x.shape
    Co, _, kh, kw = weight.shape
    Ho, Wo = g.shape[2], g.shape[3]
    aw = grad_sink_again(weight) if SINK_ACCUMULATE else None
    ab = grad_sink_again(bias) if (aw is not None and torch.is_tensor(bias)) else None
    if aw is not None and (bias is None or ab is not None) and B * Ho * Wo > 0:
        nbytes = capi.lib().htd_conv2d_wgrad_workspace_bytes(B, H, W, Ci, Co, kh, kw, stride, padding, dilation)
        ws = torch.empty(nbytes // 4 + 1, device=g.device, dtype=g.dtype)
        work = ('flop', 2.0 * B * Ho * Wo * Co * kh * kw * Ci, 4.0 * (x.numel() + g.numel() + aw.numel()))
        if amax is not None:
            capi.call('htd_conv2d_bwd_weight_h2', _P(x), _P(g), _P(amax[0]), _P(amax[1]), _P(aw), _P(ab), B, H, W, Ci, Co, kh, kw,
                      stride, padding, dilation, 1, _P(ws), _S(), work=work)
        else:
            capi.call('htd_conv2d_bwd_weight_acc', _P(x), _P(g), _P(aw), _P(ab), B, H, W, Ci, Co, kh, kw, stride, padding,
                      dilation, _P(ws), _S(), key='htd_conv2d_bwd_weight', work=work)
        ent = _GRAD_SINK.get(weight.data_ptr())
        return None, None, not (ent is not None and ent[2] is _TEMP_USED)
    gw, sink_w = grad_out2(weight)
    gb, sink_b = (None, True)
    if bias is not None:
        gb, sink_b = grad_out2(bias) if torch.is_tensor(bias) else (torch.empty(Co, device=g.device, dtype=g.dtype), False)
    if B * Ho * Wo == 0:
        gw.zero_()
        if gb is not None:
            gb.zero_()
        return gw, gb, sink_w and sink_b
    nbytes = capi.lib().htd_conv2d_wgrad_workspace_bytes(B, H, W, Ci, Co, kh, kw, stride, padding, dilation)
    ws = torch.empty(nbytes // 4 + 1, device=g.device, dtype=g.dtype)
    work = ('flop', 2.0 * B * Ho * Wo * Co * kh * kw * Ci, 4.0 * (x.numel() + g.numel() + gw.numel()))
    if amax is not None:
        capi.call('htd_conv2d_bwd_weight_h2', _P(x), _P(g), _P(amax[0]), _P(amax[1]), _P(gw), _P(gb), B, H, W, Ci, Co, kh, kw,
                  stride, padding, dilation, 0, _P(ws), _S(), work=work)
    else:
        capi.call('htd_conv2d_bwd_weight', _P(x), _P(g), _P(gw), _P(gb), B, H, W, Ci, Co, kh, kw, stride, padding,
                  dilation, _P(ws), _S(), work=work)
    return gw, gb, sink_w and sink_b


def _wgrad_raw(x, g, weight, stride, padding, dilation, bias=None, overlap=True):
    amax = _wgrad_amax(x, g, weight, stride, padding, dilation)
    if not overlap or not OVERLAP_WGRAD or (capi.profiling() and not _OVERLAP_IN_PROFILE):
        if OVERLAP_WGRAD and _SIDE and SINK_ACCUMULATE and grad_sink_again(weight) is not None:
            torch.cuda.current_stream().wait_stream(side_stream(g.device))
        return _wgrad_launch(x, g, weight, stride, padding, dilation, bias, amax)[:2]
    main, side = torch.cuda.current_stream(), side_stream(g.device)
    side.wait_stream(main)
    x.record_stream(side)
    g.record_stream(side)
    with torch.cuda.stream(side):
        gw, gb, sinks = _wgrad_launch(x, g, weight, stride, padding, dilation, bias, amax)
    if not sinks and not side_consumed(weight):
        if gw is not None:
            gw.record_stream(main)
        if gb is not None:
            gb.record_stream(main)
        main.wait_stream(side)
    return gw, gb


def _dgrad_joined(galias, g, weight, x_shape, stride, padding, dilation):
    fuse = galias is not None and stride == 1 and galias.dtype == g.dtype and tuple(galias.shape) == tuple(x_shape)
    gx = _dgrad_raw(g, weight, x_shape, stride, padding, dilation, accum=galias.contiguous(memory_format=CL) if fuse else None)
    return gx if (galias is None or fuse) else gx + galias


class Conv2dFunction(Function):
    @staticmethod
    def forward(ctx, x, weight, bias, residual, stride, padding, dilation, relu, res_up=False, chain=False):
        _need_gpu(x, 'conv2d')
        src = x
        x = x.contiguous(memory_format=CL)
        weight = weight.contiguous(memory_format=CL)
        res = residual.contiguous(memory_format=CL) if residual is not None else None
        b = bias.contiguous() if bias is not None else None
        y = _fwd_raw(x, weight, b, res, stride, padding, dilation, relu, res_up)
        ctx.save_for_backward(x, weight, y if relu else None)
        ctx.cfg = (stride, padding, dilation, bool(relu), bias is not None, residual is not None)
        ctx.res_up = tuple(res.shape) if (res_up and res is not None) else None
        ctx.bias_ref = b
        return chain_outputs(ctx, y, (src, ), chain)

    @staticmethod
    @once_differentiable
    def backward(ctx, g, galias=None):
        x, weight, y = ctx.saved_tensors
        stride, padding, dilation, relu, has_bias, has_res = ctx.cfg
        if g is None:
            return (galias, ) + (None, ) * 9
        g = g.contiguous(memory_format=CL)
        need_x, need_w, need_b, need_r = ctx.needs_input_grad[:4]
        gb = gw = None
        want_b = has_bias and need_b
        if relu:
            if want_b and not need_w:
                g, gb = _colsum_raw(g, y, ctx.bias_ref)
            else:
                g = _mask_raw(g, y)
        elif want_b and not need_w:
            gb = _colsum_raw(g, None, ctx.bias_ref)[1]
        gx = _dgrad_joined(galias, g, weight, x.shape, stride, padding, dilation) if need_x else None
        aliases_g = has_res and need_r and ctx.res_up is None
        if need_w:
            gw, gb = _wgrad_raw(x, g, weight, stride, padding, dilation, ctx.bias_ref if want_b else None,
                                overlap=not aliases_g)
        gr = None
        if has_res and need_r:
            gr = g
            if ctx.res_up is not None:
                rB, rC, rh, rw = ctx.res_up
                gr = torch.empty((rB, rC, rh, rw), device=g.device, dtype=g.dtype, memory_format=CL)
                capi.call('htd_upsample_nearest_bwd', _P(g), _P(gr), rB, g.size(2), g.size(3), rh, rw, rC, _S(),
                          work=('byte', 4.0 * (g.numel() + gr.numel())))
        return gx, gw, (gb if (has_bias and need_b) else None), gr, None, None, None, None, None, None


class ConvReluHeadFunction(Function):

    @staticmethod
    def forward(ctx, x, w1, b1, w2, b2, padding, chain):
        _need_gpu(x, 'conv_relu_head')
        src = x
        x = x.contiguous(memory_format=CL)
        w1, w2 = w1.contiguous(memory_format=CL), w2.contiguous(memory_format=CL)
        b1 = b1.contiguous() if b1 is not None else None
        b2 = b2.contiguous() if b2 is not None else None
        h = _fwd_raw(x, w1, b1, None, 1, padding, 1, True)
        y = _fwd_raw(h, w2, b2, None, 1, 0, 1, False)
        ctx.save_for_backward(x, w1, w2, h)
        ctx.cfg = (int(padding), b1, b2)
        return chain_outputs(ctx, y, (src, ), chain)

    @staticmethod
    @once_differentiable
    def backward(ctx, gy, galias=None):
        x, w1, w2, h = ctx.saved_tensors
        padding, b1, b2 = ctx.cfg
        if gy is None:
            return (galias, ) + (None, ) * 6
        need_x, need_w1, need_b1, need_w2, need_b2 = ctx.needs_input_grad[:5]
        gy = gy.contiguous(memory_format=CL)
        gw1 = gb1 = gw2 = gb2 = None
        if need_w2:
            gw2, gb2 = _wgrad_raw(h, gy, w2, 1, 0, 1, b2 if (need_b2 and b2 is not None) else None)
        elif need_b2 and b2 is not None:
            gb2 = _colsum_raw(gy, None, b2)[1]
        gh = _dgrad_raw(gy, w2, h.shape, 1, 0, 1, mask_src=h)
        if need_w1:
            gw1, gb1 = _wgrad_raw(x, gh, w1, 1, padding, 1, b1 if (need_b1 and b1 is not None) else None)
        elif need_b1 and b1 is not None:
            gb1 = _colsum_raw(gh, None, b1)[1]
        gx = _dgrad_joined(galias, gh, w1, x.shape, 1, padding, 1) if need_x else galias
        return gx, gw1, gb1, gw2, gb2, None, None


def conv_relu_head(x, w1, b1, w2, b2, padding=1, chain=False):
    return ConvReluHeadFunction.apply(x, w1, b1, w2, b2, int(padding), bool(chain))



def _gconv_pack(weight, groups, transpose):
    C, cg, kh, kw = weight.shape
    n = capi.lib().htd_gconv2d_packed_floats(C, groups, kh, kw)
    if n <= 0:
        raise ValueError(f'grouped conv2d: {C} channels in {groups} groups is unsupported')
    wp = torch.empty(n, device=weight.device, dtype=weight.dtype)
    capi.call('htd_gconv2d_pack_weights', _P(weight), _P(wp), C, groups, kh, kw, int(transpose), _S())
    return wp


def _gconv_fwd_raw(x, wp, bias, geom, relu, cols_shape=None):
    C, groups, kh, kw, stride, padding, dilation = geom
    B, H, W = cols_shape if cols_shape is not None else (x.size(0), x.size(2), x.size(3))
    Ho, Wo = _out_hw(H, W, kh, kw, stride, padding, dilation)
    y = torch.empty((B, C, Ho, Wo), device=x.device, dtype=x.dtype, memory_format=CL)
    capi.call('htd_gconv2d_fwd', _P(x), _P(wp), _P(bias), _P(y), B, H, W, C, groups, kh, kw, stride, padding, dilation,
              int(bool(relu)), int(cols_shape is not None), _S(),
              work=('flop', 2.0 * B * Ho * Wo * C * kh * kw * (C // groups), 4.0 * (x.numel() + y.numel())))
    return y


def _gconv_dgrad_raw(g, wpT, geom, x_shape, cols=False):
    C, groups, kh, kw, stride, padding, dilation = geom
    B, _, H, W = x_shape
    M = g.size(0) * g.size(2) * g.size(3)
    gx = torch.empty((M, kh * kw, C), device=g.device, dtype=g.dtype) if cols else \
        torch.empty((B, C, H, W), device=g.device, dtype=g.dtype, memory_format=CL)
    capi.call('htd_gconv2d_bwd_data', _P(g), _P(wpT), _P(gx), B, H, W, C, groups, kh, kw, stride, padding, dilation,
              int(cols), _S(), work=('flop', 2.0 * M * C * kh * kw * (C // groups), 4.0 * (g.numel() + gx.numel())))
    return gx


def _gconv_wgrad_raw(x, g, weight, geom, x_shape, cols=False):
    C, groups, kh, kw, stride, padding, dilation = geom
    B, _, H, W = x_shape
    gw = grad_out(weight)
    nbytes = capi.lib().htd_gconv2d_wgrad_workspace_bytes(B, H, W, C, groups, kh, kw, stride, padding, dilation)
    ws = torch.empty(nbytes // 4 + 1, device=g.device, dtype=g.dtype)
    M = g.size(0) * g.size(2) * g.size(3)
    capi.call('htd_gconv2d_bwd_weight', _P(x), _P(g), _P(gw), B, H, W, C, groups, kh, kw, stride, padding, dilation,
              int(cols), _P(ws), _S(), work=('flop', 2.0 * M * C * kh * kw * (C // groups), 4.0 * (x.numel() + g.numel())))
    return gw


class GroupedConv2dFunction(Function):

    @staticmethod
    def forward(ctx, x, weight, bias, stride, padding, dilation, groups, relu):
        _need_gpu(x, 'grouped conv2d')
        x = x.contiguous(memory_format=CL)
        weight = weight.contiguous(memory_format=CL)
        C, cg, kh, kw = weight.shape
        if x.size(1) != C or cg * groups != C:
            raise ValueError(f'grouped conv2d: input {tuple(x.shape)}, weight {tuple(weight.shape)}, groups {groups}')
        if x.dtype != torch.float32:
            raise TypeError('grouped conv2d runs in fp32')
        geom = (C, groups, kh, kw, stride, padding, dilation)
        b = bias.contiguous() if bias is not None else None
        y = _gconv_fwd_raw(x, _gconv_pack(weight, groups, False), b, geom, relu)
        ctx.save_for_backward(x, weight, y if relu else None)
        ctx.geom, ctx.relu, ctx.bias_ref = geom, bool(relu), b
        return y

    @staticmethod
    @once_differentiable
    def backward(ctx, g):
        x, weight, y = ctx.saved_tensors
        g = g.contiguous(memory_format=CL)
        need_x, need_w, need_b = ctx.needs_input_grad[:3]
        gb = None
        if ctx.bias_ref is not None and need_b:
            g, gb = _colsum_raw(g, y if ctx.relu else None, ctx.bias_ref)
        elif ctx.relu:
            g = _mask_raw(g, y)
        gx = _gconv_dgrad_raw(g, _gconv_pack(weight, ctx.geom[1], True), ctx.geom, x.shape) if need_x else None
        gw = _gconv_wgrad_raw(x, g, weight, ctx.geom, x.shape) if need_w else None
        return gx, gw, gb, None, None, None, None, None


def grouped_conv2d(x, weight, bias=None, stride=1, padding=0, dilation=1, groups=1, relu=False):
    return GroupedConv2dFunction.apply(x, weight, bias, int(stride), int(padding), int(dilation), int(groups), bool(relu))


class ResStageFunction(Function):

    @staticmethod
    def forward(ctx, x, strides, dilation, has_ds, *params):
        _need_gpu(x, 'res_stage')
        x = x.contiguous(memory_format=CL)
        params = [t.contiguous(memory_format=CL) if t.dim() == 4 else t.contiguous() for t in params]
        saved, k = [], 0
        for stride, ds in zip(strides, has_ds):
            w1, b1, w2, b2, w3, b3 = params[k:k + 6]
            k += 6
            h1 = _fwd_raw(x, w1, b1, None, 1, 0, 1, True)
            h2, h2p = _fwd_raw(h1, w2, b2, None, stride, dilation, dilation, True,
                               emit=_planes_pay(w3, rows=h1.size(0) * (h1.size(2) // stride) * (h1.size(3) // stride)))
            if ds:
                wd, bd = params[k:k + 2]
                k += 2
                idn = _fwd_raw(x, wd, bd, None, stride, 0, 1, False)
            else:
                idn = x
            out = _fwd_raw(h2, w3, b3, idn, 1, 0, 1, True, x_planes=h2p)
            saved += [x, h1, h2, out]
            x = out
        ctx.save_for_backward(*saved, *params)
        ctx.cfg = (strides, dilation, has_ds)
        ctx.flipped = [take_flipped(t) if t.dim() == 4 else None for t in params]
        return x

    @staticmethod
    @once_differentiable
    def backward(ctx, g):
        strides, dilation, has_ds = ctx.cfg
        nb = len(strides)
        saved, params = ctx.saved_tensors[:4 * nb], ctx.saved_tensors[4 * nb:]
        flipped = ctx.flipped
        offs, k = [], 0
        for ds in has_ds:
            offs.append(k)
            k += 8 if ds else 6
        need = ctx.needs_input_grad
        grads = [None] * len(params)
        g = g.contiguous(memory_format=CL)
        premasked = False
        for i in range(nb - 1, -1, -1):
            x, h1, h2, out = saved[4 * i:4 * i + 4]
            k, stride, ds = offs[i], strides[i], has_ds[i]
            w1, b1, w2, b2, w3, b3 = params[k:k + 6]
            pneed = need[4 + k:4 + k + (8 if ds else 6)]
            first = i == 0
            need_x = need[0] if first else True
            gm3 = g if premasked else _mask_raw(g, out)
            gb3 = None
            if pneed[4]:
                grads[k + 4], gb3 = _wgrad_raw(h2, gm3, w3, 1, 0, 1, True if (pneed[5] or (ds and pneed[7])) else None)
            elif pneed[5] or (ds and pneed[7]):
                gb3 = _colsum_raw(gm3)[1]
            grads[k + 5] = gb3 if pneed[5] else None
            gm2 = _dgrad_raw(gm3, w3, h2.shape, 1, 0, 1, mask_src=h2, wT=flipped[k + 4])
            if pneed[2]:
                grads[k + 2], gb2 = _wgrad_raw(h1, gm2, w2, stride, dilation, dilation, True if pneed[3] else None)
            else:
                gb2 = _colsum_raw(gm2)[1] if pneed[3] else None
            grads[k + 3] = gb2 if pneed[3] else None
            gm1, gm1p = _dgrad_raw(gm2, w2, h1.shape, stride, dilation, dilation, mask_src=h1, wT=flipped[k + 2],
                                   emit=bool(need_x and _planes_pay(w1, True, rows=h1.size(0) * h1.size(2) * h1.size(3))))
            if pneed[0]:
                grads[k], gb1 = _wgrad_raw(x, gm1, w1, 1, 0, 1, True if pneed[1] else None)
            else:
                gb1 = _colsum_raw(gm1)[1] if pneed[1] else None
            grads[k + 1] = gb1 if pneed[1] else None
            acc = gm3
            if ds:
                wd = params[k + 6]
                if pneed[6]:
                    grads[k + 6] = _wgrad_raw(x, gm3, wd, stride, 0, 1)[0]
                grads[k + 7] = gb3 if pneed[7] else None
                acc = _dgrad_raw(gm3, wd, x.shape, stride, 0, 1, wT=flipped[k + 6]) if need_x else None
            if need_x:
                g = _dgrad_raw(gm1, w1, x.shape, 1, 0, 1, mask_src=None if first else x, accum=acc, wT=flipped[k],
                               g_planes=gm1p)
                premasked = not first
            else:
                g = None
        return (g, None, None, None, *grads)


def conv2d_bf16(x, weight, bias=None, stride=1, padding=0, dilation=1, relu=False, residual=None, res_up=False):
    _need_gpu(x, 'conv2d_bf16')
    if x.dtype != torch.bfloat16 or weight.dtype != torch.bfloat16:
        raise TypeError('conv2d_bf16: x and weight must be bfloat16')
    x = x.contiguous(memory_format=CL)
    weight = weight.contiguous(memory_format=CL)
    B, Ci, H, W = x.shape
    Co, _, kh, kw = weight.shape
    Ho, Wo = _out_hw(H, W, kh, kw, stride, padding, dilation)
    y = torch.empty((B, Co, Ho, Wo), device=x.device, dtype=torch.bfloat16, memory_format=CL)
    b = bias.float().contiguous() if bias is not None else None
    res = residual.to(torch.bfloat16).contiguous(memory_format=CL) if residual is not None else None
    if res_up and res is not None:
        if res.size(0) != B or res.size(1) != Co or res.size(2) > Ho or res.size(3) > Wo:
            raise ValueError('conv2d_bf16: up-sampled residual %s does not fit the output %s' % (tuple(res.shape), tuple(y.shape)))
        capi.call('htd_conv2d_fwd_bf16_up', _P(x), _P(weight), _P(b), _P(res), res.size(2), res.size(3), _P(y), B, H, W, Ci,
                  Co, kh, kw, int(stride), int(padding), int(dilation), int(bool(relu)), _S(), key='htd_conv2d_fwd_bf16',
                  work=('flop', 2.0 * B * Ho * Wo * Co * kh * kw * Ci, 2.0 * (x.numel() + weight.numel() + y.numel() + res.numel())))
        return y
    capi.call('htd_conv2d_fwd_bf16', _P(x), _P(weight), _P(b), _P(res), _P(y), B, H, W, Ci, Co, kh, kw, int(stride),
              int(padding), int(dilation), int(bool(relu)), _S(),
              work=('flop', 2.0 * B * Ho * Wo * Co * kh * kw * Ci,
                    2.0 * (x.numel() + weight.numel() + y.numel() * (2 if res is not None else 1))))
    return y


def conv2d_wgrad_bf16(x, gy, weight_shape, stride=1, padding=0, dilation=1, with_bias=False, weight=None, bias=None):
    _need_gpu(x, 'conv2d_wgrad_bf16')
    x = x.contiguous(memory_format=CL)
    gy = gy.contiguous(memory_format=CL)
    B, Ci, H, W = x.shape
    Co, _, kh, kw = weight_shape
    gw = None
    if weight is not None and weight.dtype == torch.float32 and tuple(weight.shape) == tuple(weight_shape):
        gw = grad_out2(weight)[0]
        if not (gw.dim() == 4 and gw.is_contiguous(memory_format=CL)):
            gw = None
    if gw is None:
        gw = torch.empty((Co, Ci, kh, kw), device=x.device, dtype=torch.float32, memory_format=CL)
    nbytes = capi.lib().htd_conv2d_wgrad_bf16_workspace_bytes(B, H, W, Ci, Co, kh, kw, stride, padding, dilation)
    ws = torch.empty(nbytes // 4 + 1, device=x.device, dtype=torch.float32)
    if with_bias:
        gb = grad_out2(bias)[0] if (bias is not None and bias.dtype == torch.float32 and bias.numel() == Co) else \
            torch.empty(Co, device=x.device, dtype=torch.float32)
        capi.call('htd_conv2d_bwd_weight_bf16_bias', _P(x), _P(gy), _P(gw), _P(gb), B, H, W, Ci, Co, kh, kw, int(stride),
                  int(padding), int(dilation), _P(ws), _S(), key='htd_conv2d_bwd_weight_bf16',
                  work=('flop', 2.0 * gy.numel() * kh * kw * Ci, 2.0 * (x.numel() + gy.numel()) + 4.0 * gw.numel()))
        return gw, gb
    capi.call('htd_conv2d_bwd_weight_bf16', _P(x), _P(gy), _P(gw), B, H, W, Ci, Co, kh, kw, int(stride), int(padding),
              int(dilation), _P(ws), _S(), work=('flop', 2.0 * gy.numel() * kh * kw * Ci, 2.0 * (x.numel() + gy.numel()) + 4.0 * gw.numel()))
    return gw


BF16 = torch.bfloat16


def _prep_bf16(weight, want_wT=True):
    weight = weight.contiguous(memory_format=CL)
    Co, Ci, kh, kw = weight.shape
    wb = torch.empty((Co, Ci, kh, kw), device=weight.device, dtype=BF16, memory_format=CL)
    wT = torch.empty((Ci, Co, kh, kw), device=weight.device, dtype=BF16, memory_format=CL) if want_wT else None
    capi.call('htd_weights_prep_bf16', _P(weight), _P(wb), _P(wT), Co, kh, kw, Ci, _S())
    return wb, wT


def _prep_bf16_many(items):
    import numpy as np
    if not items:
        return []
    ws = [w.contiguous(memory_format=CL) for w, _ in items]
    dev = ws[0].device
    total = sum(w.numel() * (2 if want else 1) for w, (_, want) in zip(ws, items))
    flat = torch.empty(total, device=dev, dtype=BF16)
    desc = np.zeros((len(ws), 6), dtype=np.int64)
    out, off, tile0 = [], 0, 0
    for i, (w, (_, want)) in enumerate(zip(ws, items)):
        Co, Ci, kh, kw = w.shape
        wb = flat[off:off + w.numel()].view(Co, kh, kw, Ci).permute(0, 3, 1, 2)
        off += w.numel()
        wT = None
        if want:
# ... 130 lines not shown
        ctx.save_for_backward(*saved, *params)
        ctx.wTs = wTs
        ctx.cfg = (strides, dilation, has_ds)
        return x

    @staticmethod
    @once_differentiable
    def backward(ctx, g):
        strides, dilation, has_ds = ctx.cfg
        nb = len(strides)
        saved, params = ctx.saved_tensors[:4 * nb], ctx.saved_tensors[4 * nb:]
        wTs = ctx.wTs
        offs, k = [], 0
        for ds in has_ds:
            offs.append(k)
            k += 8 if ds else 6
        need = ctx.needs_input_grad
        grads = [None] * len(params)
        g = g.to(BF16).contiguous(memory_format=CL)
        premasked = False
        for i in range(nb - 1, -1, -1):
            x, h1, h2, out = saved[4 * i:4 * i + 4]
            wT1, wT2, wT3, wTd = wTs[4 * i:4 * i + 4]
            k, stride, ds = offs[i], strides[i], has_ds[i]
            w1, b1, w2, b2, w3, b3 = params[k:k + 6]
            pneed = need[4 + k:4 + k + (8 if ds else 6)]
            first = i == 0
            need_x = need[0] if first else True
            gm3 = g if premasked else torch.ops.aten.threshold_backward(g, out, 0)
            want_b3 = pneed[5] or (ds and pneed[7])
            gb3 = None
            if pneed[4] and want_b3 and w3.size(0) % 8 == 0:
                grads[k + 4], gb3 = conv2d_wgrad_bf16(h2, gm3, w3.shape, 1, 0, 1, with_bias=True)
            else:
                if pneed[4]:
                    grads[k + 4] = conv2d_wgrad_bf16(h2, gm3, w3.shape, 1, 0, 1)
                gb3 = _colsum_bf16_raw(gm3) if want_b3 else None
            grads[k + 5] = gb3 if pneed[5] else None
            gm2 = _dgrad_bf16_raw(gm3, wT3, 1, 0, 1, mask_src=h2)
            if pneed[2] and pneed[3]:
                grads[k + 2], grads[k + 3] = conv2d_wgrad_bf16(h1, gm2, w2.shape, stride, dilation, dilation, with_bias=True)
            else:
                if pneed[2]:
                    grads[k + 2] = conv2d_wgrad_bf16(h1, gm2, w2.shape, stride, dilation, dilation)
                grads[k + 3] = _colsum_bf16_raw(gm2) if pneed[3] else None
            gm1 = _dgrad_bf16_any(gm2, wT2, w2, h1.shape, 3, stride, dilation, dilation, mask_src=h1)
            if pneed[0] and pneed[1]:
                grads[k], grads[k + 1] = conv2d_wgrad_bf16(x, gm1, w1.shape, 1, 0, 1, with_bias=True)
            else:
                if pneed[0]:
                    grads[k] = conv2d_wgrad_bf16(x, gm1, w1.shape, 1, 0, 1)
                grads[k + 1] = _colsum_bf16_raw(gm1) if pneed[1] else None
            acc = gm3
            if ds:
                wd = params[k + 6]
                if pneed[6]:
                    grads[k + 6] = conv2d_wgrad_bf16(x, gm3, wd.shape, stride, 0, 1)
                grads[k + 7] = gb3 if pneed[7] else None
                acc = _dgrad_bf16_any(gm3, wTd, wd, x.shape, 1, stride, 0, 1) if need_x else None
            if need_x:
                g = _dgrad_bf16_raw(gm1, wT1, 1, 0, 1, mask_src=None if first else x, accum=acc)
                premasked = not first
            else:
                g = None
        ctx.wTs = None
        return (g, None, None, None, *grads)


def conv2d_bf16_autograd(x, weight, bias=None, stride=1, padding=0, dilation=1, relu=False, residual=None, residual_up=False):
    return Conv2dBf16Function.apply(x, weight, bias, residual, int(stride), int(padding), int(dilation), bool(relu),
                                    bool(residual_up))


def _pad_channels(x, weight, mult=8):
    Ci = x.size(1)
    pad = (-Ci) % mult
    if pad == 0:
        return x, weight
    x = torch.nn.functional.pad(x, (0, 0, 0, 0, 0, pad))
    weight = torch.nn.functional.pad(weight, (0, 0, 0, 0, 0, pad))
    return x.contiguous(memory_format=CL), weight.contiguous(memory_format=CL)


def conv2d(x, weight, bias=None, stride=1, padding=0, dilation=1, relu=False, residual=None, residual_up=False, chain=False):
    if isinstance(stride, (tuple, list)):
        stride, padding, dilation = stride[0], padding[0], dilation[0]
    if x.size(1) % 8 != 0:
        assert not chain
        stem = (STEM7 and x.size(1) == 3 and tuple(weight.shape) == (64, 3, 7, 7) and int(stride) == 2 and int(padding) == 3 and
                int(dilation) == 1 and residual is None and not x.requires_grad and x.dtype == torch.float32 and x.is_cuda and
                capi.lib().htd_conv2d_set_math(-1) == 1)
        x, weight = _pad_channels(x, weight, 4 if stem else 8)
    return Conv2dFunction.apply(x, weight, bias, residual, int(stride), int(padding), int(dilation), relu,
                                bool(residual_up), bool(chain))


def linear(x, weight, bias=None, relu=False):
    M, K = x.shape
    N = weight.size(0)
    if M == 0:
        return x.new_zeros(0, N) + (0 * weight.sum())
    if K % 8 != 0:
        pad = (-K) % 8
        x = torch.nn.functional.pad(x, (0, pad))
        weight = torch.nn.functional.pad(weight, (0, pad))
        K += pad
    x4 = x.contiguous().view(M, 1, 1, K).permute(0, 3, 1, 2)
    w4 = weight.contiguous().view(N, 1, 1, K).permute(0, 3, 1, 2)
    if x.dtype == torch.bfloat16 and K % 32 == 0 and N % 8 == 0:
        y = Conv2dBf16Function.apply(x4, w4, bias, None, 1, 0, 1, relu)
    else:
        y = Conv2dFunction.apply(x4.float() if x.dtype != torch.float32 else x4, w4, bias, None, 1, 0, 1, relu)
    return y.permute(0, 2, 3, 1).reshape(M, N)


BGEMM_BWD_LIMITS = os.environ.get('HTD_BGEMM_BWD_LIMITS', '1') != '0'


class BatchedGemmNT(Function):

    @staticmethod
    def _run(a, b, counts=None, limit=0):
        G, M, K = a.shape
        N = b.size(1)
        c = torch.empty(G, M, N, device=a.device, dtype=a.dtype)
        if counts is not None and limit and M % 128 == 0:
            capi.call('htd_bgemm_nt_counts', _P(a), _P(b), _P(c), G, M, N, K, _P(counts), int(limit), _S(),
                      work=('flop', 2.0 * G * M * N * K))
        else:
            capi.call('htd_bgemm_nt', _P(a), _P(b), _P(c), G, M, N, K, _S(), work=('flop', 2.0 * G * M * N * K))
        return c

    @staticmethod
    def forward(ctx, a, b, counts=None, limit=0):
        _need_gpu(a, 'bgemm_nt')
        ctx.gram = a is b
        a, b = a.contiguous(), b.contiguous()
        ctx.save_for_backward(a, b)
        ctx.counts, ctx.limit = counts, int(limit)
        return BatchedGemmNT._run(a, b, counts, limit)

    @staticmethod
    @once_differentiable
    def backward(ctx, gc):
        a, b = ctx.saved_tensors
        gc = gc.contiguous()
        ga = gb = None
        counts, lim = (ctx.counts, ctx.limit) if BGEMM_BWD_LIMITS else (None, 0)
        lim_a = (lim & 1) | ((lim & 4) >> 1) | ((lim & 2) << 1)
        lim_b = ((lim & 2) >> 1) | ((lim & 4) >> 1) | ((lim & 1) << 2)
        if ctx.gram and ctx.needs_input_grad[0] and ctx.needs_input_grad[1]:
            return BatchedGemmNT._run(gc + gc.transpose(1, 2), a.transpose(1, 2).contiguous(), counts, lim_a), None, None, None
        if ctx.needs_input_grad[0]:
            ga = BatchedGemmNT._run(gc, b.transpose(1, 2).contiguous(), counts, lim_a)
        if ctx.needs_input_grad[1]:
            gb = BatchedGemmNT._run(gc.transpose(1, 2).contiguous(), a.transpose(1, 2).contiguous(), counts, lim_b)
        return ga, gb, None, None


def bgemm_nt(a, b, counts=None, limit=0):
    return BatchedGemmNT.apply(a, b, counts, int(limit))


def roofline_report(prof, peak_tflops, peak_gbs, peak_bf16_tflops=2500.0):
    prof = dict(prof)
    parts = [prof.pop(k) for k in ('htd_conv2d_fwd', 'htd_conv2d_bwd_data') if k in prof]
    if parts:
        prof['conv_igemm_kernel (htd_conv2d_fwd + htd_conv2d_bwd_data)'] = (
            sum(p[0] for p in parts), sum(p[1] for p in parts), 'flop', sum(p[3] for p in parts), sum(p[4] for p in parts))
    parts = [prof.pop(k) for k in ('htd_conv2d_fwd_x3p', 'htd_conv2d_bwd_data_x3p') if k in prof]
    if parts:
        prof['conv_x3p_kernel (htd_conv2d_fwd_x3p + htd_conv2d_bwd_data_x3p)'] = (
            sum(p[0] for p in parts), sum(p[1] for p in parts), 'flop', sum(p[3] for p in parts), sum(p[4] for p in parts))
    parts = [prof.pop(k) for k in ('htd_conv2d_fwd_bf16', 'htd_conv2d_dgrad_bf16') if k in prof]
    if parts:
        prof['conv_bf16_kernel (htd_conv2d_fwd_bf16 + htd_conv2d_dgrad_bf16)'] = (
            sum(p[0] for p in parts), sum(p[1] for p in parts), 'flop', sum(p[3] for p in parts), sum(p[4] for p in parts))
# ... 38 lines not shown
```

htd_amd/detector/bricks.py:

```python
import torch
import torch.nn as nn
import torch.nn.functional as F

from .. import mmcv_ops as M
from ..registry import CONV_LAYERS

CL = torch.channels_last


def dense_conv2d(x, weight, bias=None, stride=1, padding=0, dilation=1, relu=False, residual=None, residual_up=False,
                 chain=False):
    from .. import dense
    if x.dtype == torch.bfloat16:
        y = dense.conv2d_bf16_autograd(x, weight, bias, stride, padding, dilation, relu, residual, residual_up)
        return (y, x) if chain else y
    return dense.conv2d(x, weight, bias, stride, padding, dilation, relu, residual, residual_up, chain)


@CONV_LAYERS.register_module('Conv')
@CONV_LAYERS.register_module('Conv2d')
class Conv2d(nn.Conv2d):

    def __init__(self, *args, **kwargs):
        super().__init__(*args, **kwargs)
        assert self.padding_mode == 'zeros'
        assert self.groups == 1 or (self.in_channels == self.out_channels and self.bias is None), \
            'grouped convs: the in == out, bias-free 3x3 of the ResNeXt bottleneck'
        self.weight.data = self.weight.data.contiguous(memory_format=CL)

    def _apply(self, fn, recurse=True):
        super()._apply(fn, recurse)
        self.weight.data = self.weight.data.contiguous(memory_format=CL)
        return self

    def forward(self, x, relu=False, residual=None, weight=None, bias=None, residual_up=False, chain=False):
        w = self.weight if weight is None else weight
        b = self.bias if bias is None else bias
        if self.groups > 1:
            from .. import dense
            assert residual is None and not chain
            dt = x.dtype
            y = dense.grouped_conv2d(x.float() if dt != torch.float32 else x, w, b, self.stride[0], self.padding[0],
                                     self.dilation[0], self.groups, relu)
            return y.to(dt) if dt != torch.float32 else y
        return dense_conv2d(x, w, b, self.stride[0], self.padding[0], self.dilation[0], relu, residual, residual_up, chain)


@CONV_LAYERS.register_module('ConvWS')
class ConvWS2d(Conv2d):

    def __init__(self, in_channels, out_channels, kernel_size, stride=1, padding=0, dilation=1, groups=1, bias=True,
                 eps=1e-5):
        super().__init__(in_channels, out_channels, kernel_size, stride=stride, padding=padding, dilation=dilation,
                         groups=groups, bias=bias)
        self.eps = eps

    def standardized_weight(self):
        return M.weight_standardize(self.weight, self.eps)

    def forward(self, x, relu=False, residual=None, weight=None, bias=None, residual_up=False, chain=False):
        assert weight is None, 'ConvWS2d standardises its own weight'
        return super().forward(x, relu=relu, residual=residual, weight=self.standardized_weight(), bias=bias,
                               residual_up=residual_up, chain=chain)


def build_conv_layer(cfg, *args, **kwargs):
    cfg_ = dict(type='Conv2d') if cfg is None else dict(cfg)
    layer_type = cfg_.pop('type')
    cls = CONV_LAYERS.get(layer_type)
    if cls is None:
        raise KeyError(f'Unrecognized conv type {layer_type}')
    return cls(*args, **kwargs, **cfg_)


def build_norm_layer(cfg, num_features, postfix=''):
    cfg_ = dict(cfg)
    layer_type = cfg_.pop('type')
    requires_grad = cfg_.pop('requires_grad', True)
    cfg_.setdefault('eps', 1e-5)
    if layer_type in ('BN', 'BN2d'):
        layer, abbr = nn.BatchNorm2d(num_features, **cfg_), 'bn'
    elif layer_type == 'GN':
        assert 'num_groups' in cfg_
        layer, abbr = nn.GroupNorm(num_channels=num_features, **cfg_), 'gn'
    else:
        raise KeyError(f'Unrecognized norm type {layer_type}')
    for p in layer.parameters():
        p.requires_grad = requires_grad
    return abbr + str(postfix), layer


class _BNFold(torch.autograd.Function):

    @staticmethod
    def forward(ctx, w, gamma, beta, mean, var, eps):
        from .. import capi
        w = w.contiguous(memory_format=CL)
        Co = w.size(0)
        K = w.numel() // Co
        wf = torch.empty_like(w, memory_format=CL)
        bf = torch.empty(Co, device=w.device, dtype=w.dtype)
        capi.call('htd_bn_fold_fwd', capi.ptr(w), capi.ptr(gamma), capi.ptr(beta), capi.ptr(mean), capi.ptr(var),
                  float(eps), capi.ptr(wf), capi.ptr(bf), Co, K, capi.current_stream_ptr())
        ctx.save_for_backward(w, gamma, mean, var)
        ctx.eps = float(eps)
        ctx.beta_ref = beta
        from .. import dense
        dense.mark_side_consumed(wf)
        return wf, bf

    @staticmethod
    @torch.autograd.function.once_differentiable
    def backward(ctx, gwf, gbf):
        from .. import capi
        w, gamma, mean, var = ctx.saved_tensors
        Co = w.size(0)
        K = w.numel() // Co
        gwf = gwf.contiguous(memory_format=CL)
        gbf = gbf.contiguous()
        from .. import dense

        def launch():
            (gw, s1), (gg, s2), (gb, s3) = dense.grad_out2(w), dense.grad_out2(gamma), dense.grad_out2(ctx.beta_ref)
            capi.call('htd_bn_fold_bwd', capi.ptr(w), capi.ptr(gamma), capi.ptr(mean), capi.ptr(var), ctx.eps,
                      capi.ptr(gwf), capi.ptr(gbf), capi.ptr(gw), capi.ptr(gg), capi.ptr(gb), Co, K,
                      capi.current_stream_ptr())
            return (gw, gg, gb), s1 and s2 and s3
        if not dense.OVERLAP_WGRAD or (capi.profiling() and not dense._OVERLAP_IN_PROFILE):
            return launch()[0] + (None, None, None)
        main, side = torch.cuda.current_stream(), dense.side_stream(gwf.device)
        side.wait_stream(main)
        gwf.record_stream(side)
        gbf.record_stream(side)
        with torch.cuda.stream(side):
            outs, all_sinks = launch()
        if not all_sinks:
            for t in outs:
                t.record_stream(main)
            main.wait_stream(side)
        return outs + (None, None, None)


class _BNFoldMany(torch.autograd.Function):

    @staticmethod
    def forward(ctx, eps, want_flips, want_planes, *tensors):
# ... 199 lines not shown
```

htd_amd/detector/fpn.py:

```python
import os

import torch
import torch.nn as nn
import torch.nn.functional as F

from ..registry import NECKS
from .bricks import ConvModule, xavier_init


FUSED_TOP_DOWN = os.environ.get('HTD_FPN_FUSED', '1') != '0'


@NECKS.register_module()
class FPN(nn.Module):
    def __init__(self, in_channels, out_channels, num_outs, start_level=0, end_level=-1, add_extra_convs=False,
                 extra_convs_on_inputs=True, relu_before_extra_convs=False, no_norm_on_lateral=False, conv_cfg=None,
                 norm_cfg=None, act_cfg=None, upsample_cfg=dict(mode='nearest')):
        super().__init__()
        assert isinstance(in_channels, list)
        self.in_channels, self.out_channels = in_channels, out_channels
        self.num_ins, self.num_outs = len(in_channels), num_outs
        self.upsample_cfg = dict(upsample_cfg)
        if end_level == -1:
            self.backbone_end_level = self.num_ins
            assert num_outs >= self.num_ins - start_level
        else:
            self.backbone_end_level = end_level
            assert end_level <= len(in_channels) and num_outs == end_level - start_level
        self.start_level, self.end_level = start_level, end_level
        self.relu_before_extra_convs, self.no_norm_on_lateral = relu_before_extra_convs, no_norm_on_lateral
        assert isinstance(add_extra_convs, (str, bool))
        if isinstance(add_extra_convs, str):
            assert add_extra_convs in ('on_input', 'on_lateral', 'on_output')
        elif add_extra_convs:
            add_extra_convs = 'on_input' if extra_convs_on_inputs else 'on_output'
        self.add_extra_convs = add_extra_convs
        self.lateral_convs = nn.ModuleList()
        self.fpn_convs = nn.ModuleList()
        for i in range(self.start_level, self.backbone_end_level):
            self.lateral_convs.append(ConvModule(in_channels[i], out_channels, 1, conv_cfg=conv_cfg,
                                                 norm_cfg=norm_cfg if not no_norm_on_lateral else None,
                                                 act_cfg=act_cfg, inplace=False))
            self.fpn_convs.append(ConvModule(out_channels, out_channels, 3, padding=1, conv_cfg=conv_cfg,
                                             norm_cfg=norm_cfg, act_cfg=act_cfg, inplace=False))
        extra_levels = num_outs - self.backbone_end_level + self.start_level
        if self.add_extra_convs and extra_levels >= 1:
            for i in range(extra_levels):
                cin = in_channels[self.backbone_end_level - 1] if i == 0 and self.add_extra_convs == 'on_input' else out_channels
                self.fpn_convs.append(ConvModule(cin, out_channels, 3, stride=2, padding=1, conv_cfg=conv_cfg, norm_cfg=norm_cfg,
                                                 act_cfg=act_cfg, inplace=False))

    def _extra_levels(self, inputs, laterals, outs):
        n = len(self.lateral_convs)
        if self.num_outs <= n:
            return outs
        if not self.add_extra_convs:
            for _ in range(self.num_outs - n):
                outs.append(outs[-1][:, :, ::2, ::2])
            return outs
        source = dict(on_input=inputs[self.backbone_end_level - 1], on_lateral=laterals[-1], on_output=outs[-1])
        outs.append(self.fpn_convs[n](source[self.add_extra_convs]))
        for i in range(n + 1, self.num_outs):
            outs.append(self.fpn_convs[i](F.relu(outs[-1]) if self.relu_before_extra_convs else outs[-1]))
        return outs

    def init_weights(self):
        for m in self.modules():
            if isinstance(m, nn.Conv2d):
                xavier_init(m, distribution='uniform')

    def _fused_top_down(self, inputs):
        if not inputs[0].is_cuda or inputs[0].dtype not in (torch.float32, torch.bfloat16) or \
                any(t.dtype != inputs[0].dtype for t in inputs) or \
                self.upsample_cfg.get('mode', 'nearest') != 'nearest' or \
                self.out_channels % 4 != 0 or not getattr(self, 'fused_top_down', FUSED_TOP_DOWN):
            return False
        if 'scale_factor' in self.upsample_cfg:
            sf = self.upsample_cfg['scale_factor']
            shapes = [t.shape[2:] for t in inputs[self.start_level:self.backbone_end_level]]
            if any(int(b[0] * sf) != a[0] or int(b[1] * sf) != a[1] for a, b in zip(shapes[:-1], shapes[1:])):
                return False
        return all(not m.with_norm and not m.with_activation for m in self.lateral_convs)

    def forward(self, inputs):
        assert len(inputs) == len(self.in_channels)
        n = len(self.lateral_convs)
        if self._fused_top_down(inputs):
            laterals, outs_chain = [None] * n, [None] * n
            chain = inputs[0].is_cuda and inputs[0].dtype == torch.float32 and torch.is_grad_enabled() and \
                self.add_extra_convs != 'on_lateral' and \
                all(not c.with_norm and not c.with_activation and getattr(c, 'compute_dtype', None) is None
                    for c in self.fpn_convs[:n])
            for i in range(n - 1, -1, -1):
                m = self.lateral_convs[i]
                up = laterals[i + 1] if i + 1 < n else None
                laterals[i] = m.conv(inputs[i + self.start_level], residual=up, residual_up=up is not None)
                if chain and i > 0:
                    outs_chain[i], laterals[i] = self.fpn_convs[i].conv(laterals[i], chain=True)
            if chain:
                outs = [outs_chain[i] if i > 0 else self.fpn_convs[0](laterals[0]) for i in range(n)]
                return tuple(self._extra_levels(inputs, laterals, outs))
        else:
            laterals = [conv(inputs[i + self.start_level]) for i, conv in enumerate(self.lateral_convs)]
            for i in range(n - 1, 0, -1):
                if 'scale_factor' in self.upsample_cfg:
                    up = F.interpolate(laterals[i], **self.upsample_cfg)
                else:
                    up = F.interpolate(laterals[i], size=laterals[i - 1].shape[2:], **self.upsample_cfg)
                laterals[i - 1] = laterals[i - 1] + up
        outs = [self.fpn_convs[i](laterals[i]) for i in range(n)]
        return tuple(self._extra_levels(inputs, laterals, outs))
```

htd_amd/detector/resnet.py:

```python
import math
import os

import torch
import torch.nn as nn
from torch.nn.modules.batchnorm import _BatchNorm

from .. import mmcv_ops as M
from ..dense import ResStageBf16Function, ResStageFunction
from ..registry import BACKBONES
from .bricks import ConvWS2d, build_conv_layer, build_norm_layer, constant_init, frozen_bn_fold, frozen_bn_fold_many, kaiming_init

CL = torch.channels_last
FUSE_BF16_STAGE = os.environ.get('HTD_BF16_STAGE', '1') != '0'


def conv_bn(conv, bn, x, relu=False, residual=None):
    if isinstance(bn, nn.GroupNorm):
        y = conv(x)
        if y.is_cuda and y.dtype == torch.float32:
            return M.group_norm_map(y, bn.weight, bn.bias, bn.num_groups, bn.eps, relu, residual)
        y = bn(y)
        if residual is not None:
            y = y + residual
        return torch.relu(y) if relu else y
    if isinstance(conv, ConvWS2d):
        raise NotImplementedError('ConvWS under a BatchNorm: no config has it (the BN fold would have to follow the standardisation)')
    if bn.training:
        y = bn(conv(x))
        if residual is not None:
            y = y + residual
        return torch.relu(y) if relu else y
    w, b = frozen_bn_fold(conv.weight, bn)
    return conv(x, relu=relu, residual=residual, weight=w, bias=b)


class Bottleneck(nn.Module):
    expansion = 4

    def __init__(self, inplanes, planes, stride=1, dilation=1, downsample=None, style='pytorch', with_cp=False,
                 conv_cfg=None, norm_cfg=dict(type='BN'), dcn=None, plugins=None, groups=1, base_width=4,
                 base_channels=64):
        super().__init__()
        assert style in ['pytorch', 'caffe']
        assert dcn is None or isinstance(dcn, dict)
        assert plugins is None, 'plugins are outside the HTD path'
        self.inplanes, self.planes, self.stride, self.dilation = inplanes, planes, stride, dilation
        self.style, self.with_cp, self.conv_cfg, self.norm_cfg = style, with_cp, conv_cfg, norm_cfg
        self.dcn, self.with_dcn = dcn, dcn is not None
        self.conv1_stride, self.conv2_stride = (1, stride) if style == 'pytorch' else (stride, 1)
        self.groups = groups
        width = planes if groups == 1 else math.floor(planes * (base_width / base_channels)) * groups
        self.width = width
        gkw = dict(groups=groups) if groups != 1 else {}
        self.norm1_name, norm1 = build_norm_layer(norm_cfg, width, postfix=1)
        self.norm2_name, norm2 = build_norm_layer(norm_cfg, width, postfix=2)
        self.norm3_name, norm3 = build_norm_layer(norm_cfg, planes * self.expansion, postfix=3)
        self.conv1 = build_conv_layer(conv_cfg, inplanes, width, kernel_size=1, stride=self.conv1_stride, bias=False)
        self.add_module(self.norm1_name, norm1)
        fallback_on_stride = False
        if self.with_dcn:
            dcn = dict(dcn)
            fallback_on_stride = dcn.pop('fallback_on_stride', False)
        if not self.with_dcn or fallback_on_stride:
            self.conv2 = build_conv_layer(conv_cfg, width, width, kernel_size=3, stride=self.conv2_stride,
                                          padding=dilation, dilation=dilation, bias=False, **gkw)
        else:
            assert conv_cfg is None, 'conv_cfg must be None for DCN'
            self.conv2 = build_conv_layer(dcn, width, width, kernel_size=3, stride=self.conv2_stride,
                                          padding=dilation, dilation=dilation, bias=False, **gkw)
        self.add_module(self.norm2_name, norm2)
        self.conv3 = build_conv_layer(conv_cfg, width, planes * self.expansion, kernel_size=1, bias=False)
        self.add_module(self.norm3_name, norm3)
        self.relu = nn.ReLU(inplace=True)
        self.downsample = downsample

    @property
    def norm1(self):
        return getattr(self, self.norm1_name)

    @property
    def norm2(self):
        return getattr(self, self.norm2_name)

    @property
    def norm3(self):
        return getattr(self, self.norm3_name)

    def forward(self, x):
        out = conv_bn(self.conv1, self.norm1, x, relu=True)
        if hasattr(self.conv2, 'conv_offset') and (self.norm2.training or not out.is_cuda or
                                                   not getattr(self, 'fuse_dcn_bn', True) or
                                                   type(self.conv2).__name__ != 'DeformConv2dPack'):
            out = torch.relu(self.norm2(self.conv2(out)))
        elif hasattr(self.conv2, 'conv_offset'):
            w, b = frozen_bn_fold(self.conv2.weight, self.norm2)
            dt = out.dtype
            if dt == torch.bfloat16 and self.groups == 1:
                out = self.conv2(out, relu=True, weight=w, bias=b)
            else:
                out = self.conv2(out.float() if dt != torch.float32 else out, relu=True, weight=w, bias=b)
                out = out.to(dt) if dt != torch.float32 else out
        else:
            out = conv_bn(self.conv2, self.norm2, out, relu=True)
        identity = x if self.downsample is None else conv_bn(self.downsample[0], self.downsample[1], x)
        return conv_bn(self.conv3, self.norm3, out, relu=True, residual=identity)


class ResLayer(nn.Sequential):
    def __init__(self, block, inplanes, planes, num_blocks, stride=1, avg_down=False, conv_cfg=None,
                 norm_cfg=dict(type='BN'), downsample_first=True, **kwargs):
        assert not avg_down and downsample_first, 'ResNetV1d / hourglass variants are outside the HTD path'
        self.block = block
        downsample = None
        if stride != 1 or inplanes != planes * block.expansion:
            downsample = nn.Sequential(
                build_conv_layer(conv_cfg, inplanes, planes * block.expansion, kernel_size=1, stride=stride, bias=False),
                build_norm_layer(norm_cfg, planes * block.expansion)[1])
        layers = [block(inplanes=inplanes, planes=planes, stride=stride, downsample=downsample, conv_cfg=conv_cfg,
                        norm_cfg=norm_cfg, **kwargs)]
        inplanes = planes * block.expansion
        for _ in range(1, num_blocks):
            layers.append(block(inplanes=inplanes, planes=planes, stride=1, conv_cfg=conv_cfg, norm_cfg=norm_cfg,
                                **kwargs))
        super().__init__(*layers)

    def _fusable(self):
        for blk in self:
            if not isinstance(blk, Bottleneck) or blk.with_dcn or blk.style != 'pytorch' or blk.groups != 1:
                return False
            bns = [blk.norm1, blk.norm2, blk.norm3] + ([blk.downsample[1]] if blk.downsample is not None else [])
            if any(bn.training or not isinstance(bn, nn.BatchNorm2d) for bn in bns):
                return False
        return True

    def forward(self, x):
        if not x.is_cuda or x.dtype not in (torch.float32, torch.bfloat16) or not self._fusable() or \
                (x.dtype == torch.bfloat16 and not FUSE_BF16_STAGE):
            return super().forward(x)
        pairs = []
        for blk in self:
            pairs += [(blk.conv1.weight, blk.norm1), (blk.conv2.weight, blk.norm2), (blk.conv3.weight, blk.norm3)]
            if blk.downsample is not None:
                pairs.append((blk.downsample[0].weight, blk.downsample[1]))
        params = frozen_bn_fold_many(pairs, want_flips=x.dtype == torch.float32 and
                                     (x.requires_grad or any(w.requires_grad for w, _ in pairs)),
                                     want_planes=x.dtype == torch.float32)
        strides, has_ds = tuple(blk.conv2_stride for blk in self), tuple(blk.downsample is not None for blk in self)
        stage = ResStageFunction if x.dtype == torch.float32 else ResStageBf16Function
        return stage.apply(x, strides, self[0].dilation, has_ds, *params)


@BACKBONES.register_module()
class ResNet(nn.Module):
    arch_settings = {50: (Bottleneck, (3, 4, 6, 3)), 101: (Bottleneck, (3, 4, 23, 3)), 152: (Bottleneck, (3, 8, 36, 3))}

    def __init__(self, depth, in_channels=3, stem_channels=None, base_channels=64, num_stages=4,
                 strides=(1, 2, 2, 2), dilations=(1, 1, 1, 1), out_indices=(0, 1, 2, 3), style='pytorch',
                 deep_stem=False, avg_down=False, frozen_stages=-1, conv_cfg=None,
                 norm_cfg=dict(type='BN', requires_grad=True), norm_eval=True, dcn=None,
                 stage_with_dcn=(False, False, False, False), plugins=None, with_cp=False, zero_init_residual=True):
        super().__init__()
        if depth not in self.arch_settings:
            raise KeyError(f'invalid depth {depth} for resnet')
        assert not deep_stem and not avg_down and plugins is None
        self.depth = depth
        stem_channels = base_channels if stem_channels is None else stem_channels
        self.stem_channels, self.base_channels, self.num_stages = stem_channels, base_channels, num_stages
        assert 1 <= num_stages <= 4
        self.strides, self.dilations = strides, dilations
        assert len(strides) == len(dilations) == num_stages
        self.out_indices = out_indices
        assert max(out_indices) < num_stages
        self.style, self.deep_stem, self.avg_down, self.frozen_stages = style, deep_stem, avg_down, frozen_stages
        self.conv_cfg, self.norm_cfg, self.with_cp, self.norm_eval = conv_cfg, norm_cfg, with_cp, norm_eval
        self.dcn, self.stage_with_dcn = dcn, stage_with_dcn
        if dcn is not None:
            assert len(stage_with_dcn) == num_stages
        self.zero_init_residual = zero_init_residual
        self.block, stage_blocks = self.arch_settings[depth]
        self.stage_blocks = stage_blocks[:num_stages]
        self.inplanes = stem_channels
        self.conv1 = build_conv_layer(conv_cfg, in_channels, stem_channels, kernel_size=7, stride=2, padding=3,
                                      bias=False)
        self.norm1_name, norm1 = build_norm_layer(norm_cfg, stem_channels, postfix=1)
        self.add_module(self.norm1_name, norm1)
        self.relu = nn.ReLU(inplace=True)
        self.maxpool = nn.MaxPool2d(kernel_size=3, stride=2, padding=1)
        self.res_layers = []
        for i, num_blocks in enumerate(self.stage_blocks):
            planes = base_channels * 2**i
            res_layer = self.make_res_layer(block=self.block, inplanes=self.inplanes, planes=planes,
                                            num_blocks=num_blocks, stride=strides[i], dilation=dilations[i],
                                            style=style, avg_down=avg_down, with_cp=with_cp, conv_cfg=conv_cfg,
                                            norm_cfg=norm_cfg, dcn=self.dcn if self.stage_with_dcn[i] else None)
            self.inplanes = planes * self.block.expansion
            name = f'layer{i + 1}'
            self.add_module(name, res_layer)
            self.res_layers.append(name)
        self._freeze_stages()
        self.feat_dim = self.block.expansion * base_channels * 2**(len(self.stage_blocks) - 1)

    def make_res_layer(self, **kwargs):
        return ResLayer(**kwargs)

    @property
    def norm1(self):
        return getattr(self, self.norm1_name)

    def _freeze_stages(self):
        if self.frozen_stages >= 0:
            self.norm1.eval()
            for m in [self.conv1, self.norm1]:
                for p in m.parameters():
                    p.requires_grad = False
        for i in range(1, self.frozen_stages + 1):
            m = getattr(self, f'layer{i}')
            m.eval()
            for p in m.parameters():
                p.requires_grad = False

    def init_weights(self, pretrained=None):
        if isinstance(pretrained, str):
            from ..checkpoint import load_checkpoint
            load_checkpoint(self, pretrained, strict=False)
        elif pretrained is None:
            for m in self.modules():
                if isinstance(m, nn.Conv2d):
                    kaiming_init(m)
                elif isinstance(m, (_BatchNorm, nn.GroupNorm)):
                    constant_init(m, 1)
            if self.dcn is not None:
                for m in self.modules():
                    if isinstance(m, Bottleneck) and hasattr(m.conv2, 'conv_offset'):
                        constant_init(m.conv2.conv_offset, 0)
            if self.zero_init_residual:
                for m in self.modules():
                    if isinstance(m, Bottleneck):
                        constant_init(m.norm3, 0)
        else:
            raise TypeError('pretrained must be a str or None')

    def forward(self, x):
        x = x.contiguous(memory_format=CL)
        x = conv_bn(self.conv1, self.norm1, x, relu=True)
        mp = self.maxpool
        if x.is_cuda and x.size(1) % 4 == 0 and not mp.ceil_mode and mp.dilation == 1:
            x = M.max_pool2d(x, mp.kernel_size, mp.stride, mp.padding)
        else:
            x = mp(x)
        if getattr(self, 'compute_dtype', torch.float32) == torch.bfloat16 and x.is_cuda:
            x = x.to(torch.bfloat16)
        outs = []
        for i, name in enumerate(self.res_layers):
            x = getattr(self, name)(x)
            if i in self.out_indices:
                outs.append(x)
        return tuple(outs)

    def train(self, mode=True):
        super().train(mode)
        self._freeze_stages()
        if mode and self.norm_eval:
            for m in self.modules():
                if isinstance(m, _BatchNorm):
                    m.eval()
        return self


@BACKBONES.register_module()
class ResNeXt(ResNet):

    def __init__(self, groups=1, base_width=4, **kwargs):
        self.groups, self.base_width = groups, base_width
        super().__init__(**kwargs)

    def make_res_layer(self, **kwargs):
        return ResLayer(groups=self.groups, base_width=self.base_width, base_channels=self.base_channels, **kwargs)
```

include/htd_amd.h:

```cpp
#ifndef HTD_AMD_H
#define HTD_AMD_H

#include <stdint.h>

#ifdef __cplusplus
extern "C" {
#endif

#define HTD_OK 0
#define HTD_ERR_ARG 1
#define HTD_ERR_LAUNCH 2

const char *htd_last_error(void);
#define HTD_ABI_VERSION 8
int htd_abi_version(void);

int htd_roi_align_fwd(const float *feat, const float *rois, const int64_t *roi_level, int level,
                      float *out, int64_t n, int B, int C, int H, int W, int ph, int pw, float spatial_scale,
                      int sampling_ratio, int aligned, void *stream);
int htd_roi_align_bwd(const float *grad_out, const float *rois, const int64_t *roi_level, int level,
                      float *grad_feat, int64_t n, int B, int C, int H, int W, int ph, int pw,
                      float spatial_scale, int sampling_ratio, int aligned, void *stream);
int htd_roi_align_levels_fwd(const float *const *feats, const int *H, const int *W, const float *scales, int L,
                             const float *rois, const int64_t *roi_level, float *out, int64_t n, int B, int C, int ph, int pw,
// ... 67 lines not shown
int64_t htd_conv2d_workspace_bytes(int64_t M, int Co, int Ci, int kh, int kw);
int htd_conv2d_set_math(int mode);
int htd_conv2d_tile_table_set(int64_t M, int Co, int Ci, int taps, int epi, int cfg);
int htd_conv2d_tile_table_clear(void);
int htd_conv2d_tile_query(int64_t M, int Co, int Ci, int taps, int epi);
int htd_conv2d_fwd(const float *x, const float *w, const float *bias, const float *residual, int res_h,
                   int res_w, float *y, int B, int H, int W, int Ci, int Co, int kh, int kw, int stride,
                   int pad, int dil, int relu, void *workspace, void *stream);
int htd_bgemm_nt(const float *a, const float *b, float *c, int G, int M, int N, int K, void *stream);
int htd_bgemm_nt_counts(const float *a, const float *b, float *c, int G, int M, int N, int K, const int64_t *counts, int limit,
                        void *stream);
int htd_conv2d_flip_weights(const float *w, float *wT, int Co, int kh, int kw, int Ci, void *stream);
int htd_conv2d_flip_weights_padded(const float *w, float *wT, int Co, int Co_padded, int kh, int kw, int Ci, void *stream);
int htd_pad_channels(const float *x, float *y, int64_t rows, int C, int C_padded, void *stream);
int htd_conv2d_bwd_data(const float *gy, const float *wT, const float *mask_src, const float *accum, float *gx,
                        int B, int H, int W, int Ci, int Co, int kh, int kw, int stride, int pad, int dil,
                        void *workspace, void *stream);
int htd_conv2d_fwd_amax(const float *x, const float *w, const float *bias, const float *residual, int res_h, int res_w,
                        float *y, float *amax_out, int B, int H, int W, int Ci, int Co, int kh, int kw, int stride, int pad,
                        int dil, int relu, void *workspace, void *stream);
int htd_conv2d_bwd_data_amax(const float *gy, const float *wT, const float *mask_src, const float *accum, float *gx,
                             float *amax_out, int B, int H, int W, int Ci, int Co, int kh, int kw, int stride, int pad,
                             int dil, void *workspace, void *stream);
int64_t htd_conv2d_wgrad_workspace_bytes(int B, int H, int W, int Ci, int Co, int kh, int kw,
                                         int stride, int pad, int dil);
int htd_conv2d_bwd_weight(const float *x, const float *gy, float *gw, float *gbias, int B, int H, int W,
                          int Ci, int Co, int kh, int kw, int stride, int pad, int dil, void *workspace,
                          void *stream);
int htd_conv2d_bwd_weight_acc(const float *x, const float *gy, float *gw, float *gbias, int B, int H, int W, int Ci,
                              int Co, int kh, int kw, int stride, int pad, int dil, void *workspace, void *stream);
int htd_bias_grad_relu_mask(const float *g, const float *y, float *gm, float *gbias, int64_t rows,
                            int C, void *workspace, void *stream);
int htd_bias_grad_relu_mask_amax(const float *g, const float *y, float *gm, float *gbias, int64_t rows, int C,
                                 void *workspace, float *amax_out, void *stream);
int64_t htd_conv2d_stem7_workspace_bytes(void);
int htd_conv2d_stem7_fwd(const float *x, const float *w, const float *bias, float *y, int B, int H, int W, int relu,
                         void *workspace, void *stream);
int htd_conv2d_x3p_supported(int Ci, int Co, int kh, int kw, int stride, int pad, int dil);
int htd_conv2d_x3p_tile_table_set(int64_t M, int Co, int Ci, int taps, int epi, int cfg);
int htd_conv2d_x3p_tile_table_clear(void);
int htd_conv2d_x3p_tile_query(int64_t M, int Co, int Ci, int taps, int epi);
int htd_conv2d_x3p_plan_query(int cfg, int64_t M, int Co, int Ci, int kh, int kw, int64_t *out);
int64_t htd_conv2d_x3_planes_bytes(int Co, int kh, int kw, int Ci, int transposed);
int htd_conv2d_x3_planes(const float *w, void *planes, int Co, int kh, int kw, int Ci, int transposed, void *stream);
int htd_conv2d_x3_planes_many(const void *desc, int n, int64_t total_blocks, void *stream);
int64_t htd_conv2d_x3p_workspace_bytes(int64_t M, int Co, int Ci, int kh, int kw);
int htd_conv2d_fwd_x3p(const float *x, const void *wplanes, const float *bias, const float *residual, int res_h,
                       int res_w, float *y, int B, int H, int W, int Ci, int Co, int kh, int kw, int stride, int pad,
                       int relu, void *workspace, void *stream);
int htd_conv2d_bwd_data_x3p(const float *gy, const void *wplanesT, const float *mask_src, const float *accum,
                            float *gx, int B, int H, int W, int Ci, int Co, int kh, int kw, int pad, void *workspace,
                            void *stream);
int64_t htd_act_planes_rows(int64_t M);
int64_t htd_act_planes_bytes(int64_t M, int C);
int htd_act_planes(const float *x, void *planes, int64_t M, int C, void *stream);
int htd_conv2d_fwd_x3q(const float *x, const void *xplanes, const void *wplanes, const float *bias, const float *residual,
                       int res_h, int res_w, float *y, void *yplanes, float *amax_out, int B, int H, int W, int Ci, int Co, int kh, int kw,
                       int stride, int pad, int relu, void *workspace, void *stream);
int htd_conv2d_bwd_data_x3q(const float *gy, const void *gyplanes, const void *wplanesT, const float *mask_src,
                            const float *accum, float *gx, void *gxplanes, float *amax_out, int B, int H, int W, int Ci, int Co, int kh, int kw,
                            int pad, void *workspace, void *stream);

int htd_conv2d_set_h2(int on);
int htd_conv2d_bwd_weight_h2_supported(int B, int H, int W, int Ci, int Co, int kh, int kw, int stride, int pad, int dil);
int htd_conv2d_bwd_weight_h2(const float *x, const float *gy, const float *amax_x, const float *amax_g, float *gw,
                             float *gbias, int B, int H, int W, int Ci, int Co, int kh, int kw, int stride, int pad,
                             int dil, int accumulate, void *workspace, void *stream);
int htd_conv2d_x3h_supported(int Ci, int Co, int kh, int kw, int stride, int pad, int dil);
int htd_conv2d_x3h_strided_supported(int Ci, int Co, int kh, int kw, int stride, int pad, int dil);
int htd_conv2d_bwd_data_x3h_strided_supported(int Ci, int Co, int kh, int kw, int stride, int pad, int dil);
int64_t htd_conv2d_bwd_data_x3h_strided_workspace_bytes(int B, int H, int W, int Ci, int Co, int kh, int kw, int stride, int pad);
int htd_conv2d_bwd_data_x3h_strided(const float *gy, const float *amax, const void *wplanesT, const float *mask_src, float *gx,
                                    float *amax_out, int B, int H, int W, int Ci, int Co, int kh, int kw, int stride, int pad,
                                    void *workspace, void *stream);
int htd_absmax(const float *x, int64_t n, float *amax, void *stream);
int htd_conv2d_x3h_planes(const float *w, void *planes, int Co, int kh, int kw, int Ci, int transposed, void *stream);
int htd_conv2d_x3h_planes_many(const void *desc, int n, int64_t total_blocks, int64_t total_rows, void *stream);
int htd_conv2d_fwd_x3h(const float *x, const float *amax, const void *wplanes, const float *bias, const float *residual,
                       int res_h, int res_w, float *y, void *yplanes, float *amax_out, int B, int H, int W, int Ci,
                       int Co, int kh, int kw, int stride, int pad, int relu, void *workspace, void *stream);
int htd_conv2d_bwd_data_x3h(const float *gy, const float *amax, const void *wplanesT, const float *mask_src,
                            const float *accum, float *gx, void *gxplanes, float *amax_out, int B, int H, int W,
                            int Ci, int Co, int kh, int kw, int pad, void *workspace, void *stream);

int64_t htd_deform_columns_bytes(int B, int H, int W, int C, int kh, int kw, int stride, int pad, int dil);
int htd_deform_im2col(const float *x, const float *offset, const float *mask, float *columns, int B,
                      int H, int W, int C, int kh, int kw, int stride, int pad, int dil,
                      int deform_groups, void *stream);
int htd_deform_col2im(const float *x, const float *offset, const float *mask, const float *gcolumns,
                      float *gx, float *goffset, float *gmask, int B, int H, int W, int C, int kh,
                      int kw, int stride, int pad, int dil, int deform_groups, void *stream);
int htd_deform_im2col_bf16(const void *x, const float *offset, const float *mask, void *columns, int B, int H, int W,
                           int C, int kh, int kw, int stride, int pad, int dil, int deform_groups, void *stream);
int htd_deform_col2im_bf16(const void *x, const float *offset, const float *mask, const void *gcolumns, float *gx,
                           float *goffset, float *gmask, int B, int H, int W, int C, int kh, int kw, int stride, int pad,
                           int dil, int deform_groups, void *stream);

int htd_global_avg_pool_fwd(const float *x, float *out, int64_t B, int P, int C, void *stream);
int htd_global_avg_pool_bwd(const float *g, float *gx, int64_t B, int P, int C, void *stream);
int htd_global_avg_pool_bwd_acc(const float *g, float *gx, int64_t B, int P, int C, void *stream);

int htd_group_norm_relu_fwd(const float *x, const float *gamma, const float *beta, float *y,
                            float *mean, float *rstd, int64_t n, int P, int C, int G, float eps,
                            int relu, void *stream);
int htd_group_norm_relu_bwd(const float *x, const float *y, const float *gamma, const float *mean,
                            const float *rstd, const float *gy, float *gx, float *ggamma,
                            float *gbeta, int64_t n, int P, int C, int G, int relu, void *stream);
int htd_group_norm_relu_bwd_ws(const float *x, const float *y, const float *gamma, const float *mean, const float *rstd,
                               const float *gy, float *gx, float *ggamma, float *gbeta, int64_t n, int P, int C, int G,
                               int relu, void *workspace, void *stream);
int htd_group_norm_relu_fwd_amax(const float *x, const float *gamma, const float *beta, float *y, float *mean, float *rstd,
                                 int64_t n, int P, int C, int G, float eps, int relu, float *amax_out, void *stream);
int htd_group_norm_bwd_amax_supported(int P, int C, int G);
int htd_group_norm_relu_bwd_amax(const float *x, const float *y, const float *gamma, const float *mean, const float *rstd,
                                 const float *gy, float *gx, float *ggamma, float *gbeta, int64_t n, int P, int C, int G,
                                 int relu, void *workspace, float *amax_out, void *stream);
int htd_fuse_global_bwd_global_ws(const float *grad, const float *rois, float *grad_global, int64_t n, int P, int C, int B,
                                  void *workspace, void *stream);

int htd_group_norm_map_slab(int P, int C);
int64_t htd_group_norm_map_workspace_bytes(int64_t n, int P, int C, int G);
int htd_group_norm_map_fwd(const float *x, const float *residual, const float *gamma, const float *beta, float *y, float *mean,
                           float *rstd, int64_t n, int P, int C, int G, float eps, int relu, void *workspace, float *amax_out,
                           void *stream);
int htd_group_norm_map_bwd(const float *x, const float *y, const float *gamma, const float *mean, const float *rstd,
                           const float *gy, float *gx, float *gres, float *ggamma, float *gbeta, int64_t n, int P, int C, int G,
                           int relu, void *workspace, float *amax_out, void *stream);

int htd_weight_standardize_fwd(const float *w, float *w_hat, float *mean, float *inv, int Co, int K, float eps, void *stream);
int htd_weight_standardize_bwd(const float *w, const float *mean, const float *inv, const float *g_hat, float *gw, int Co, int K,
                               float eps, void *stream);

int htd_bn_fold_fwd(const float *w, const float *gamma, const float *beta, const float *mean,
                    const float *var, float eps, float *w_folded, float *b_folded, int Co, int K,
                    void *stream);
int htd_bn_fold_bwd(const float *w, const float *gamma, const float *mean, const float *var, float eps,
                    const float *gw_folded, const float *gb_folded, float *gw, float *ggamma,
                    float *gbeta, int Co, int K, void *stream);
int htd_bn_fold_many_fwd(const void *desc, int n_layers, int total_tiles, float eps, void *stream);
int htd_bn_fold_many_bwd(const void *desc, int n_layers, int total_rows, float eps, void *stream);

int64_t htd_max_iou_assign_workspace_bytes(int B, int A, int K);
int htd_max_iou_assign(const float *boxes, int box_shared, const uint8_t *box_valid, const float *gts,
                       const uint8_t *gt_valid, int B, int A, int K, float pos_iou_thr, float neg_iou_thr,
                       float min_pos_iou, int match_low_quality, int64_t *assigned, float *max_overlaps,
                       void *workspace, void *stream);

int htd_roi_targets(const float *boxes, const float *gt_boxes, const int64_t *gt_labels, const uint8_t *is_pos,
                    const uint8_t *valid, int64_t n, int num_classes, const float *means4, const float *stds4,
                    int64_t *labels, float *label_weights, float *bbox_targets, float *bbox_weights, void *stream);
int htd_delta2bbox_clip(const float *rois, const float *deltas, const float *lim_wh, const uint8_t *keep, int64_t n,
                        int64_t rows_per_img, const float *means4, const float *stds4, float wh_ratio_clip,
                        float *out, void *stream);
int htd_map_roi_levels(const float *rois, int64_t *lvls, int64_t n, int num_levels, float finest_scale, void *stream);
int htd_rpn_heads_gather(const float *const *y, const int64_t *pix, int L, int B, int C, int na, float *cls, float *reg,
                         void *stream);
int htd_rpn_heads_scatter(const float *gcls, const float *greg, float *const *gy, const int64_t *pix, int L, int B, int C,
                          int na, void *stream);
int htd_static_samples_finish(const float *gts, const uint8_t *gvalid, const int64_t *glabels, const float *props,
                              const int64_t *assigned, const int64_t *order, const int64_t *counts, int B, int K, int P,
                              int A, int S, int add_gt, float *boxes, uint8_t *valid, uint8_t *is_pos,
                              float *pos_gt_boxes, int64_t *pos_gt_labels, uint8_t *pos_is_gt, void *stream);

int htd_roi_head_loss_partial_rows(void);
int htd_roi_head_loss(const float *cls_score, const int64_t *labels, const float *label_weights, const float *bbox_pred,
                      const float *bbox_targets, const float *bbox_weights, int64_t n, int NC, int num_fg, float beta,
// ... 236 lines not shown
```

Baseline: 121.6 images/sec.

## Fuse strided 1x1 dgrad into joined 1x1 dgrad epilogue and chain ResNet stages

Adds an accum2 operand to the 1x1 data-gradient conv epilogues, so a compact strided 1x1 dgrad result is added at stride-aligned positions instead of being written through a memset and scatter pass. ResNet stages can now chain with the next stage and the FPN laterals, passing stage outputs and a ReLU mask so backward gradients are merged in one kernel rather than through separate accumulation passes. This is meant to cut memsets, extra full-tensor read/write passes and kernel launches in the backbone backward. In exchange it adds new kernel instantiations, a smaller epilogue unroll when accum2 is on, and more complex autograd plumbing.

```diff
diff --git a/htd_amd/csrc/conv_x3.hip b/htd_amd/csrc/conv_x3.hip
--- a/htd_amd/csrc/conv_x3.hip
+++ b/htd_amd/csrc/conv_x3.hip
@@ -115,7 +115,22 @@
     int64_t xp_rows, yp_rows;
     const float *amax, *wscale;
     float *amax_out;
+    const float *accum2;
+    int a2_step, a2_H, a2_W;
 };
+
+__device__ __forceinline__ int64_t x3_a2_off(const X3Params &p, int64_t m, int n)
+{
+    const unsigned mm = (unsigned)m, wo = mm % (unsigned)p.Wo, t = mm / (unsigned)p.Wo;
+    const unsigned ho = t % (unsigned)p.Ho, b = t / (unsigned)p.Ho, s = (unsigned)p.a2_step;
+    if (ho % s != 0 || wo % s != 0) return -1;
+    return (((int64_t)b * p.a2_H + ho / s) * p.a2_W + wo / s) * p.Co + n;
+}
+__device__ __forceinline__ float4 x3_a2_load4(const X3Params &p, int64_t m, int n)
+{
+    const int64_t ao = x3_a2_off(p, m, n);
+    return ao >= 0 ? *reinterpret_cast<const float4 *>(p.accum2 + ao) : make_float4(0.f, 0.f, 0.f, 0.f);
+}
 
 __device__ __forceinline__ void block_absmax_out(float mx, float *out, float *red, unsigned seen)
 {
@@ -170,7 +185,7 @@
     return (((int64_t)b * p.oH + p.o_h0 + p.o_step * (int)ho) * p.oW + p.o_w0 + p.o_step * (int)wo) * p.Co + n;
 }
 
-template <int WGM, int WGN, int TM, int TN, bool MF16, typename Acc>
+template <int WGM, int WGN, int TM, int TN, bool MF16, bool A2, typename Acc>
 __device__ __forceinline__ void x3_epilogue(const X3Params &p, Acc &acc, uint4 *lds, int64_t m0, int n0, bool part, bool region_b,
                                             int split)
 {
@@ -222,10 +237,11 @@
             const bool col_ok = n < p.Co;
             float4 bv = make_float4(0.f, 0.f, 0.f, 0.f);
             if (p.bias != nullptr && col_ok) bv = *reinterpret_cast<const float4 *>(p.bias + n);
-            constexpr int UB = NPASS < 4 ? NPASS : 4;
+            constexpr int UBMAX = A2 ? 2 : 4;
+            constexpr int UB = NPASS < UBMAX ? NPASS : UBMAX;
 #pragma unroll
             for (int pass0 = 0; pass0 < NPASS; pass0 += UB) {
-                float4 v[UB], rv[UB], mv[UB];
+                float4 v[UB], rv[UB], mv[UB], av[UB];
                 int64_t o[UB];
                 bool ok[UB];
 #pragma unroll
@@ -236,6 +252,7 @@
                     o[u] = x3_out_off(p, ok[u] ? m : 0, n) & -(int64_t)ok[u];
                     v[u] = *reinterpret_cast<const float4 *>(le + row * EPI_STRIDE + c4 * 4);
                     if (scaled) { v[u].x *= cscale.x; v[u].y *= cscale.y; v[u].z *= cscale.z; v[u].w *= cscale.w; }
+                    if constexpr (A2) av[u] = ok[u] ? x3_a2_load4(p, m, n) : make_float4(0.f, 0.f, 0.f, 0.f);
                 }
                 if (p.residual != nullptr) {
 #pragma unroll
@@ -247,6 +264,10 @@
                 }
 #pragma unroll
                 for (int u = 0; u < UB; ++u) { v[u].x += bv.x; v[u].y += bv.y; v[u].z += bv.z; v[u].w += bv.w; }
+                if constexpr (A2) {
+#pragma unroll
+                    for (int u = 0; u < UB; ++u) { v[u].x += av[u].x; v[u].y += av[u].y; v[u].z += av[u].z; v[u].w += av[u].w; }
+                }
                 if (p.residual != nullptr) {
 #pragma unroll
                     for (int u = 0; u < UB; ++u) { v[u].x += rv[u].x; v[u].y += rv[u].y; v[u].z += rv[u].z; v[u].w += rv[u].w; }
@@ -306,6 +327,10 @@
                 if (p.bias) {
                     const float4 bv = *reinterpret_cast<const float4 *>(p.bias + n);
                     v.x += bv.x; v.y += bv.y; v.z += bv.z; v.w += bv.w;
+                }
+                if constexpr (A2) {
+                    const float4 av = x3_a2_load4(p, m, n);
+                    v.x += av.x; v.y += av.y; v.z += av.z; v.w += av.w;
                 }
                 if (p.residual) {
                     int64_t ro = o;
@@ -329,9 +354,11 @@
                 omax = absmax4(omax, v);
                 if (p.yp != nullptr) emit_planes4(p.yp, p.yp_rows, m, n, v);
             } else {
+                const int64_t ao = A2 ? x3_a2_off(p, m, n) : -1;
                 auto put = [&](int e, float t) {
                     if (n + e >= p.Co) return;
                     t += p.bias ? p.bias[n + e] : 0.f;
+                    if constexpr (A2) t += ao >= 0 ? p.accum2[ao + e] : 0.f;
                     if (p.residual) t += p.residual[o + e];
                     if (p.relu) t = fmaxf(t, 0.f);
                     if (p.mask_src) t = p.mask_src[o + e] > 0.f ? t : 0.f;
@@ -358,8 +385,8 @@
     return by_lds < by_regs ? by_lds : by_regs;
 }
 
-template <int WGM, int WGN, int TM, int TN, int KW, bool MF16, int NB, bool H2 = false>
-__global__ __launch_bounds__(256, (x3p_occupancy<WGM, WGN, TM, TN, KW, NB, H2>())) void conv_x3p_kernel(X3Params p)
+template <int WGM, int WGN, int TM, int TN, int KW, bool MF16, int NB, bool H2, bool A2>
+__device__ __forceinline__ void conv_x3p_body(const X3Params &p)
 {
     static_assert(!(H2 && MF16), "H2: 32x32x16 form only");
     constexpr int NCHL = H2 ? 4 : NCH;
@@ -788,7 +815,19 @@
 #pragma unroll
     for (int i = 0; i < 2 * NPT; ++i) landed(ra[i]);
 
-    x3_epilogue<WGM, WGN, TM, TN, MF16>(p, acc, lds, m0, n0, part, region_b, split);
+    x3_epilogue<WGM, WGN, TM, TN, MF16, A2>(p, acc, lds, m0, n0, part, region_b, split);
+}
+
+template <int WGM, int WGN, int TM, int TN, int KW, bool MF16, int NB, bool H2 = false>
+__global__ __launch_bounds__(256, (x3p_occupancy<WGM, WGN, TM, TN, KW, NB, H2>())) void conv_x3p_kernel(X3Params p)
+{
+    conv_x3p_body<WGM, WGN, TM, TN, KW, MF16, NB, H2, false>(p);
+}
+
+template <int WGM, int WGN, int TM, int TN, bool MF16, int NB, bool H2>
+__global__ __launch_bounds__(256, (x3p_occupancy<WGM, WGN, TM, TN, 1, NB, H2>())) void conv_x3p_a2_kernel(X3Params p)
+{
+    conv_x3p_body<WGM, WGN, TM, TN, 1, MF16, NB, H2, true>(p);
 }
 
 template <int WGM, int WGN, int TM, int TN, int NS>
@@ -802,7 +841,7 @@
     return by_lds < by_regs ? by_lds : by_regs;
 }
 
-template <int WGM, int WGN, int TM, int TN, bool MF16, int NS>
+template <int WGM, int WGN, int TM, int TN, bool MF16, int NS, bool A2 = false>
 __global__ __launch_bounds__(256, (x3q_occupancy<WGM, WGN, TM, TN, NS>())) void conv_x3q_kernel(X3Params p)
 {
     constexpr int BM = WGM * TM * 32, BN = WGN * TN * 32;
@@ -964,7 +1003,7 @@
         stage = stage + 1 == NS ? 0 : stage + 1;
         pstage = pstage + 1 == NS ? 0 : pstage + 1;
     }
-    x3_epilogue<WGM, WGN, TM, TN, MF16>(p, acc, lds, m0, n0, part, region_b, split);
+    x3_epilogue<WGM, WGN, TM, TN, MF16, A2>(p, acc, lds, m0, n0, part, region_b, split);
 }
 
 __global__ __launch_bounds__(256) void conv_x3p_splitk_epilogue_kernel(X3Params p)
@@ -983,6 +1022,10 @@
         }
         const int n = (int)(o % p.Co);
         if (p.bias) v += p.bias[n];
+        if (p.accum2) {
+            const int64_t ao = x3_a2_off(p, o / p.Co, n);
+            v += ao >= 0 ? p.accum2[ao] : 0.f;
+        }
         if (p.residual) {
             int64_t ro = p.o_step == 0 ? o : x3_out_off(p, o / p.Co, n);
             if (p.res_H > 0) {
@@ -1030,6 +1073,10 @@
         if (p.bias) {
             const float4 bv = *reinterpret_cast<const float4 *>(p.bias + n);
             v.x += bv.x; v.y += bv.y; v.z += bv.z; v.w += bv.w;
+        }
+        if (p.accum2) {
+            const float4 av = x3_a2_load4(p, (int64_t)m, (int)n);
+            v.x += av.x; v.y += av.y; v.z += av.z; v.w += av.w;
         }
         if (p.residual) {
             int64_t ro = o;
@@ -1540,7 +1587,7 @@
 int launch_x3p(X3Params p, int kw, hipStream_t s, void *workspace)
 {
     const int total_steps = p.ncs * p.kh;
-    const int epi = (p.residual ? 1 : 0) | (p.mask_src ? 2 : 0) | (p.amax ? 4 : 0);
+    const int epi = ((p.residual || p.accum2) ? 1 : 0) | (p.mask_src ? 2 : 0) | (p.amax ? 4 : 0);
     const int cfg = choose_cfg(p.M, p.Co, p.Ci, p.kh * kw + (p.ntl > 0 ? 100 : 0), epi);
     const XPlan pl = plan_x3p(cfg, p.M, p.Co, total_steps, kw, workspace != nullptr);
     p.tiles_a = pl.tiles_a; p.splits_a = pl.splits_a; p.sps_a = pl.sps_a; p.splits_b = pl.splits_b; p.sps_b = pl.sps_b;
@@ -1550,7 +1597,31 @@
     p.nt = (int)htd::ceil_div(p.Co, kXCfg[cfg].bn);
     HTD_REQUIRE(pl.grid > 0 && pl.grid < (1ll << 31), "conv2d_x3p: bad grid");
     const dim3 grid((unsigned)pl.grid);
-    if (p.amax != nullptr && kw == 3) {
+    if (p.accum2 != nullptr) {
+        HTD_REQUIRE(kw == 1 && p.o_step == 0 && p.res_H == 0, "conv2d_x3p: accum2 is an operand of the 1x1 data gradients");
+        if (p.amax != nullptr) {
+            switch (cfg) {
+            case 0: hipLaunchKernelGGL((conv_x3p_a2_kernel<2, 2, 1, 1, false, HTD_X3H_NB, true>), grid, dim3(256), 0, s, p); break;
+            case 1: hipLaunchKernelGGL((conv_x3p_a2_kernel<2, 2, 2, 2, false, HTD_X3H_NB, true>), grid, dim3(256), 0, s, p); break;
+            case 2: hipLaunchKernelGGL((conv_x3p_a2_kernel<2, 2, 2, 1, false, HTD_X3H_NB, true>), grid, dim3(256), 0, s, p); break;
+            default: hipLaunchKernelGGL((conv_x3p_a2_kernel<2, 2, 1, 2, false, HTD_X3H_NB, true>), grid, dim3(256), 0, s, p); break;
+            }
+        } else if (p.xp != nullptr) {
+            switch (cfg) {
+            case 0: hipLaunchKernelGGL((conv_x3q_kernel<2, 2, 1, 1, true, 2, true>), grid, dim3(256), 0, s, p); break;
+            case 1: hipLaunchKernelGGL((conv_x3q_kernel<2, 2, 2, 2, true, 2, true>), grid, dim3(256), 0, s, p); break;
+            case 2: hipLaunchKernelGGL((conv_x3q_kernel<2, 2, 2, 1, true, 2, true>), grid, dim3(256), 0, s, p); break;
+            default: hipLaunchKernelGGL((conv_x3q_kernel<2, 2, 1, 2, true, 2, true>), grid, dim3(256), 0, s, p); break;
+            }
+        } else {
+            switch (cfg) {
+            case 0: hipLaunchKernelGGL((conv_x3p_a2_kernel<2, 2, 1, 1, true, 2, false>), grid, dim3(256), 0, s, p); break;
+            case 1: hipLaunchKernelGGL((conv_x3p_a2_kernel<2, 2, 2, 2, true, 2, false>), grid, dim3(256), 0, s, p); break;
+            case 2: hipLaunchKernelGGL((conv_x3p_a2_kernel<2, 2, 2, 1, true, 2, false>), grid, dim3(256), 0, s, p); break;
+            default: hipLaunchKernelGGL((conv_x3p_a2_kernel<2, 2, 1, 2, true, 2, false>), grid, dim3(256), 0, s, p); break;
+            }
+        }
+    } else if (p.amax != nullptr && kw == 3) {
         switch (cfg) {
         case 0: hipLaunchKernelGGL((conv_x3p_kernel<2, 2, 1, 1, 3, false, HTD_X3H_NB, true>), grid, dim3(256), 0, s, p); break;
         case 1: hipLaunchKernelGGL((conv_x3p_kernel<2, 2, 2, 2, 3, false, HTD_X3H_NB, true>), grid, dim3(256), 0, s, p); break;
@@ -1789,9 +1860,21 @@
                               pad, relu, workspace, stream);
 }
 
-extern "C" int htd_conv2d_bwd_data_x3q(const float *gy, const void *gyplanes, const void *wplanesT, const float *mask_src,
-                                       const float *accum, float *gx, void *gxplanes, float *amax_out, int B, int H, int W, int Ci,
-                                       int Co, int kh, int kw, int pad, void *workspace, void *stream)
+namespace {
+bool set_accum2(X3Params &p, const float *accum2, int step, int H, int W)
+{
+    if (!accum2) return true;
+    if (step < 2) return false;
+    p.accum2 = accum2; p.a2_step = step;
+    p.a2_H = (H + step - 1) / step; p.a2_W = (W + step - 1) / step;
+    return true;
+}
+}
+
+extern "C" int htd_conv2d_bwd_data_x3q_joined(const float *gy, const void *gyplanes, const void *wplanesT, const float *mask_src,
+                                              const float *accum, const float *accum2, int a2_step, float *gx, void *gxplanes,
+                                              float *amax_out, int B, int H, int W, int Ci, int Co, int kh, int kw, int pad,
+                                              void *workspace, void *stream)
 {
     HTD_REQUIRE((gy || gyplanes) && wplanesT && gx && B > 0 && H > 0 && W > 0, "conv2d_bwd_data_x3q: bad arguments");
     HTD_REQUIRE(x3p_shape_ok(Co, Ci, kh, kw, 1, pad, 1), "conv2d_bwd_data_x3q: unsupported layer Ci=%d Co=%d k=%dx%d p=%d", Ci, Co,
@@ -1807,8 +1890,17 @@
     p.xp = (const uint4 *)gyplanes; p.xp_rows = act_rows(p.M);
     p.yp = (uint4 *)gxplanes; p.yp_rows = act_rows(p.M);
     p.amax_out = amax_out;
+    HTD_REQUIRE(set_accum2(p, accum2, a2_step, H, W), "conv2d_bwd_data_x3q: accum2 needs a step of 2 or more (step=%d)", a2_step);
     HTD_REQUIRE((int64_t)B * H * W * Co < (1ll << 31), "conv2d_bwd_data_x3q: operand too large");
     return launch_x3p(p, kw, (hipStream_t)stream, workspace);
+}
+
+extern "C" int htd_conv2d_bwd_data_x3q(const float *gy, const void *gyplanes, const void *wplanesT, const float *mask_src,
+                                       const float *accum, float *gx, void *gxplanes, float *amax_out, int B, int H, int W, int Ci,
+                                       int Co, int kh, int kw, int pad, void *workspace, void *stream)
+{
+    return htd_conv2d_bwd_data_x3q_joined(gy, gyplanes, wplanesT, mask_src, accum, nullptr, 0, gx, gxplanes, amax_out, B, H, W, Ci, Co,
+                                          kh, kw, pad, workspace, stream);
 }
 
 extern "C" int htd_conv2d_bwd_data_x3p(const float *gy, const void *wplanesT, const float *mask_src, const float *accum,
@@ -1857,9 +1949,10 @@
     return launch_x3p(p, kw, (hipStream_t)stream, workspace);
 }
 
-extern "C" int htd_conv2d_bwd_data_x3h(const float *gy, const float *amax, const void *wplanesT, const float *mask_src,
-                                       const float *accum, float *gx, void *gxplanes, float *amax_out, int B, int H, int W,
-                                       int Ci, int Co, int kh, int kw, int pad, void *workspace, void *stream)
+extern "C" int htd_conv2d_bwd_data_x3h_joined(const float *gy, const float *amax, const void *wplanesT, const float *mask_src,
+                                              const float *accum, const float *accum2, int a2_step, float *gx, void *gxplanes,
+                                              float *amax_out, int B, int H, int W, int Ci, int Co, int kh, int kw, int pad,
+                                              void *workspace, void *stream)
 {
     HTD_REQUIRE(!gxplanes || Ci % XK == 0, "conv2d_bwd_data_x3h: output planes need Ci %% 16 == 0 (Ci=%d)", Ci);
     HTD_REQUIRE(gy && amax && wplanesT && gx && B > 0 && H > 0 && W > 0, "conv2d_bwd_data_x3h: bad arguments");
@@ -1875,8 +1968,17 @@
     p.wscale = reinterpret_cast<const float *>(p.wp + planes_vec(kh * kw, Co, p.Cop));
     p.yp = (uint4 *)gxplanes; p.yp_rows = act_rows(p.M);
     p.amax_out = amax_out;
+    HTD_REQUIRE(set_accum2(p, accum2, a2_step, H, W), "conv2d_bwd_data_x3h: accum2 needs a step of 2 or more (step=%d)", a2_step);
     HTD_REQUIRE((int64_t)B * H * W * Co < (1ll << 31), "conv2d_bwd_data_x3h: operand too large");
     return launch_x3p(p, kw, (hipStream_t)stream, workspace);
+}
+
+extern "C" int htd_conv2d_bwd_data_x3h(const float *gy, const float *amax, const void *wplanesT, const float *mask_src,
+                                       const float *accum, float *gx, void *gxplanes, float *amax_out, int B, int H, int W,
+                                       int Ci, int Co, int kh, int kw, int pad, void *workspace, void *stream)
+{
+    return htd_conv2d_bwd_data_x3h_joined(gy, amax, wplanesT, mask_src, accum, nullptr, 0, gx, gxplanes, amax_out, B, H, W, Ci, Co, kh,
+                                          kw, pad, workspace, stream);
 }
 
 namespace {
@@ -1931,11 +2033,13 @@
     return need;
 }
 
-extern "C" int htd_conv2d_bwd_data_x3h_strided(const float *gy, const float *amax, const void *wplanesT, const float *mask_src,
-                                               float *gx, float *amax_out, int B, int H, int W, int Ci, int Co, int kh, int kw,
-                                               int stride, int pad, void *workspace, void *stream)
+namespace {
+int bwd_data_x3h_strided(const float *gy, const float *amax, const void *wplanesT, const float *mask_src, float *gx, float *amax_out,
+                         int B, int H, int W, int Ci, int Co, int kh, int kw, int stride, int pad, bool compact, void *workspace,
+                         void *stream)
 {
     HTD_REQUIRE(gy && amax && wplanesT && gx && B > 0 && H > 0 && W > 0, "conv2d_bwd_data_x3h_strided: bad arguments");
+    HTD_REQUIRE(!compact || (kh == 1 && kw == 1 && !mask_src), "conv2d_bwd_data_x3h_strided: the compact form is the 1x1 layers', unmasked");
     HTD_REQUIRE(x3h_strided_dgrad_ok(Ci, Co, kh, kw, stride, pad), "conv2d_bwd_data_x3h_strided: unsupported layer Ci=%d Co=%d k=%dx%d s=%d p=%d",
                 Ci, Co, kh, kw, stride, pad);
     const int Ho = (H + 2 * pad - kh) / stride + 1, Wo = (W + 2 * pad - kw) / stride + 1;
@@ -1943,7 +2047,7 @@
                 "conv2d_bwd_data_x3h_strided: bad sizes");
     StridedClass cls[4];
     const int live = strided_classes(H, W, kh, kw, stride, pad, cls);
-    if (live < stride * stride) {
+    if (live < stride * stride && !compact) {
         if (hipMemsetAsync(gx, 0, (size_t)B * H * W * Ci * 4, (hipStream_t)stream) != hipSuccess) {
             htd::set_error("conv2d_bwd_data_x3h_strided: memset failed");
             return HTD_ERR_LAUNCH;
@@ -1957,7 +2061,7 @@
     p.amax = amax;
     p.wscale = reinterpret_cast<const float *>(p.wp + planes_vec(kh * kw, Co, p.Cop));
     p.amax_out = amax_out;
-    p.o_step = stride; p.oH = H; p.oW = W;
+    if (!compact) { p.o_step = stride; p.oH = H; p.oW = W; }
     for (int c = 0; c < stride * stride; ++c) {
         const StridedClass &q = cls[c];
         if (q.ntaps == 0) continue;
@@ -1972,3 +2076,18 @@
     }
     return HTD_OK;
 }
+}
+
+extern "C" int htd_conv2d_bwd_data_x3h_strided(const float *gy, const float *amax, const void *wplanesT, const float *mask_src,
+                                               float *gx, float *amax_out, int B, int H, int W, int Ci, int Co, int kh, int kw,
+                                               int stride, int pad, void *workspace, void *stream)
+{
+    return bwd_data_x3h_strided(gy, amax, wplanesT, mask_src, gx, amax_out, B, H, W, Ci, Co, kh, kw, stride, pad, false, workspace, stream);
+}
+
+extern "C" int htd_conv2d_bwd_data_x3h_strided_compact(const float *gy, const float *amax, const void *wplanesT, float *gxc,
+                                                       float *amax_out, int B, int H, int W, int Ci, int Co, int stride,
+                                                       void *workspace, void *stream)
+{
+    return bwd_data_x3h_strided(gy, amax, wplanesT, nullptr, gxc, amax_out, B, H, W, Ci, Co, 1, 1, stride, 0, true, workspace, stream);
+}
diff --git a/htd_amd/dense.py b/htd_amd/dense.py
--- a/htd_amd/dense.py
+++ b/htd_amd/dense.py
@@ -304,7 +304,17 @@
     if t is not None:
         if hasattr(t, '_htd_amax'):
             del t._htd_amax
+        if hasattr(t, '_htd_premasked'):
+            del t._htd_premasked
         _AMAX_BY_PTR.pop(t.data_ptr(), None)
+
+
+def tag_premasked(g, y):
+    g._htd_premasked = (y.data_ptr(), y._version, tuple(y.shape), g.data_ptr(), g._version)
+
+
+def premasked_by(g, y):
+    return getattr(g, '_htd_premasked', None) == (y.data_ptr(), y._version, tuple(y.shape), g.data_ptr(), g._version)
 
 
 def carried_amax(t):
@@ -620,19 +630,56 @@
     return gm
 
 
-def _dgrad_raw(g, weight, x_shape, stride, padding, dilation, mask_src=None, accum=None, wT=None, g_planes=None, emit=None):
-    gx = _dgrad_raw_(g, weight, x_shape, stride, padding, dilation, mask_src, accum, wT, g_planes, bool(emit))
+def _dgrad_raw(g, weight, x_shape, stride, padding, dilation, mask_src=None, accum=None, wT=None, g_planes=None, emit=None,
+               accum2=None):
+    gx = _dgrad_raw_(g, weight, x_shape, stride, padding, dilation, mask_src, accum, wT, g_planes, bool(emit), accum2)
     if emit is not None:
         return gx if isinstance(gx, tuple) else (gx, None)
     return gx
 
 
-def _dgrad_raw_(g, weight, x_shape, stride, padding, dilation, mask_src, accum, wT, g_planes, emit):
+def _accum2_ok(weight, dtype):
+    Co, Ci, kh, kw = weight.shape
+    return kh == 1 and _x3p_ok(Co, Ci, kh, kw, 1, 0, 1, dtype)
+
+
+def _shortcut_dgrad_compact(g, weight, x_shape, stride):
+    B, Ci, H, W = x_shape
+    Co, _, kh, kw = weight.shape
+    if B == 0 or kh != 1 or kw != 1 or stride == 1 or g.dtype != torch.float32 or \
+            not capi.lib().htd_conv2d_bwd_data_x3h_strided_supported(Ci, Co, 1, 1, stride, 0, 1):
+        return None
+    am = carried_amax(g)
+    if am is None:
+        _h2_trace('dgrad', g, weight)
+        if Ci >= H2_ABSMAX_MIN_WORK and g.numel() >= H2_ABSMAX_MIN_ELEMS:
+            am = absmax(g)
+    if am is None:
+        return None
+    Ho, Wo = g.shape[2], g.shape[3]
+    gxc = torch.empty((B, Ci, Ho, Wo), device=g.device, dtype=g.dtype, memory_format=CL)
+    nb = capi.lib().htd_conv2d_bwd_data_x3h_strided_workspace_bytes(B, H, W, Ci, Co, 1, 1, stride, 0)
+    ws = torch.empty(nb // 4, device=g.device, dtype=torch.float32) if nb > 0 else None
+    out_slot = _amax_slot(g.device)
+    capi.call('htd_conv2d_bwd_data_x3h_strided_compact', _P(g), _P(am), _P(x3_planes(weight, True, True)), _P(gxc), _P(out_slot),
+              B, H, W, Ci, Co, stride, _P(ws), _S(), key='htd_conv2d_bwd_data_x3h',
+              work=('flop', 2.0 * B * Ho * Wo * Co * Ci, 4.0 * (g.numel() + weight.numel() + gxc.numel())))
+    tag_amax(gxc, out_slot)
+    _h2_guard(am, out_slot)
+    return gxc
+
+
+def _dgrad_raw_(g, weight, x_shape, stride, padding, dilation, mask_src, accum, wT, g_planes, emit, accum2=None):
     B, Ci, H, W = x_shape
     Co, _, kh, kw = weight.shape
     Ho, Wo = g.shape[2], g.shape[3]
     if B == 0:
         return torch.empty((0, Ci, H, W), device=g.device, dtype=g.dtype, memory_format=CL)
+    if accum2 is not None:
+        a2, a2_step = accum2
+        if stride != 1 or kh != 1 or not _x3p_ok(Co, Ci, kh, kw, 1, padding, dilation, g.dtype) or \
+                tuple(a2.shape) != (B, Ci, -(-H // a2_step), -(-W // a2_step)) or not a2.is_contiguous(memory_format=CL):
+            raise ValueError('dgrad: no compact operand of shape %s on this launch' % (tuple(a2.shape), ))
     if stride == 1 and _x3p_ok(Co, Ci, kh, kw, 1, padding, dilation, g.dtype):
         gx = torch.empty((B, Ci, H, W), device=g.device, dtype=g.dtype, memory_format=CL)
         nb = capi.lib().htd_conv2d_x3p_workspace_bytes(B * H * W, Ci, Co, kh, kw)
@@ -640,7 +687,8 @@
         use_gp = g_planes is not None and kh == 1
         gxp = _act_planes_buf(B * H * W, Ci, g.device) if (emit and Ci % 16 == 0) else None
         work = ('flop', 2.0 * B * Ho * Wo * Co * kh * kw * Ci,
-                4.0 * (g.numel() + weight.numel() + gx.numel() * (1 + (mask_src is not None) + (accum is not None))))
+                4.0 * (g.numel() + weight.numel() + gx.numel() * (1 + (mask_src is not None) + (accum is not None)) +
+                       (accum2[0].numel() if accum2 is not None else 0)))
         h2 = _x3h_ok(Co, Ci, kh, kw, 1, padding, dilation, g.dtype)
         out_slot = _amax_slot(g.device) if h2 else None
         if h2:
@@ -650,14 +698,24 @@
             if am is None and kh * kw * Ci >= H2_ABSMAX_MIN_WORK and g.numel() >= H2_ABSMAX_MIN_ELEMS:
                 am = absmax(g)
             if am is not None:
-                capi.call('htd_conv2d_bwd_data_x3h', _P(g), _P(am), _P(x3_planes(weight, True, True)), _P(mask_src), _P(accum), _P(gx),
-                          _P(gxp), _P(out_slot), B, H, W, Ci, Co, kh, kw, padding, _P(ws), _S(), work=work)
+                if accum2 is not None:
+                    capi.call('htd_conv2d_bwd_data_x3h_joined', _P(g), _P(am), _P(x3_planes(weight, True, True)), _P(mask_src),
+                              _P(accum), _P(accum2[0]), accum2[1], _P(gx), _P(gxp), _P(out_slot), B, H, W, Ci, Co, kh, kw, padding,
+                              _P(ws), _S(), key='htd_conv2d_bwd_data_x3h', work=work)
+                else:
+                    capi.call('htd_conv2d_bwd_data_x3h', _P(g), _P(am), _P(x3_planes(weight, True, True)), _P(mask_src), _P(accum),
+                              _P(gx), _P(gxp), _P(out_slot), B, H, W, Ci, Co, kh, kw, padding, _P(ws), _S(), work=work)
                 tag_amax(gx, out_slot)
                 _h2_guard(am, out_slot)
                 return (gx, gxp) if emit else gx
-        capi.call('htd_conv2d_bwd_data_x3q', _P(g), _P(g_planes) if use_gp else None, _P(x3_planes(weight, True, False)), _P(mask_src),
-                  _P(accum), _P(gx), _P(gxp), _P(out_slot), B, H, W, Ci, Co, kh, kw, padding, _P(ws), _S(),
-                  key='htd_conv2d_bwd_data_x3p', work=work)
+        if accum2 is not None:
+            capi.call('htd_conv2d_bwd_data_x3q_joined', _P(g), _P(g_planes) if use_gp else None, _P(x3_planes(weight, True, False)),
+                      _P(mask_src), _P(accum), _P(accum2[0]), accum2[1], _P(gx), _P(gxp), _P(out_slot), B, H, W, Ci, Co, kh, kw,
+                      padding, _P(ws), _S(), key='htd_conv2d_bwd_data_x3p', work=work)
+        else:
+            capi.call('htd_conv2d_bwd_data_x3q', _P(g), _P(g_planes) if use_gp else None, _P(x3_planes(weight, True, False)),
+                      _P(mask_src), _P(accum), _P(gx), _P(gxp), _P(out_slot), B, H, W, Ci, Co, kh, kw, padding, _P(ws), _S(),
+                      key='htd_conv2d_bwd_data_x3p', work=work)
         if out_slot is not None:
             tag_amax(gx, out_slot)
         return (gx, gxp) if emit else gx
@@ -797,15 +855,18 @@
     return gw, gb
 
 
-def _dgrad_joined(galias, g, weight, x_shape, stride, padding, dilation):
+def _dgrad_joined(galias, g, weight, x_shape, stride, padding, dilation, mask_src=None):
     fuse = galias is not None and stride == 1 and galias.dtype == g.dtype and tuple(galias.shape) == tuple(x_shape)
-    gx = _dgrad_raw(g, weight, x_shape, stride, padding, dilation, accum=galias.contiguous(memory_format=CL) if fuse else None)
-    return gx if (galias is None or fuse) else gx + galias
+    if galias is None or fuse:
+        return _dgrad_raw(g, weight, x_shape, stride, padding, dilation, mask_src=mask_src,
+                          accum=galias.contiguous(memory_format=CL) if fuse else None)
+    gx = _dgrad_raw(g, weight, x_shape, stride, padding, dilation) + galias
+    return gx if mask_src is None else _mask_raw(gx, mask_src)
 
 
 class Conv2dFunction(Function):
     @staticmethod
-    def forward(ctx, x, weight, bias, residual, stride, padding, dilation, relu, res_up=False, chain=False):
+    def forward(ctx, x, weight, bias, residual, stride, padding, dilation, relu, res_up=False, chain=False, mask_in=False):
         _need_gpu(x, 'conv2d')
         src = x
         x = x.contiguous(memory_format=CL)
@@ -817,6 +878,7 @@
         ctx.cfg = (stride, padding, dilation, bool(relu), bias is not None, residual is not None)
         ctx.res_up = tuple(res.shape) if (res_up and res is not None) else None
         ctx.bias_ref = b
+        ctx.mask_in = bool(mask_in)
         return chain_outputs(ctx, y, (src, ), chain)
 
     @staticmethod
@@ -825,7 +887,7 @@
         x, weight, y = ctx.saved_tensors
         stride, padding, dilation, relu, has_bias, has_res = ctx.cfg
         if g is None:
-            return (galias, ) + (None, ) * 9
+            return (galias, ) + (None, ) * 10
         g = g.contiguous(memory_format=CL)
         need_x, need_w, need_b, need_r = ctx.needs_input_grad[:4]
         gb = gw = None
@@ -837,7 +899,11 @@
                 g = _mask_raw(g, y)
         elif want_b and not need_w:
             gb = _colsum_raw(g, None, ctx.bias_ref)[1]
-        gx = _dgrad_joined(galias, g, weight, x.shape, stride, padding, dilation) if need_x else None
+        gx = None
+        if need_x:
+            gx = _dgrad_joined(galias, g, weight, x.shape, stride, padding, dilation, mask_src=x if ctx.mask_in else None)
+            if ctx.mask_in:
+                tag_premasked(gx, x)
         aliases_g = has_res and need_r and ctx.res_up is None
         if need_w:
             gw, gb = _wgrad_raw(x, g, weight, stride, padding, dilation, ctx.bias_ref if want_b else None,
@@ -850,7 +916,7 @@
                 gr = torch.empty((rB, rC, rh, rw), device=g.device, dtype=g.dtype, memory_format=CL)
                 capi.call('htd_upsample_nearest_bwd', _P(g), _P(gr), rB, g.size(2), g.size(3), rh, rw, rC, _S(),
                           work=('byte', 4.0 * (g.numel() + gr.numel())))
-        return gx, gw, (gb if (has_bias and need_b) else None), gr, None, None, None, None, None, None
+        return gx, gw, (gb if (has_bias and need_b) else None), gr, None, None, None, None, None, None, None
 
 
 class ConvReluHeadFunction(Function):
@@ -983,8 +1049,9 @@
 class ResStageFunction(Function):
 
     @staticmethod
-    def forward(ctx, x, strides, dilation, has_ds, *params):
+    def forward(ctx, x, strides, dilation, has_ds, chain, mask_in, *params):
         _need_gpu(x, 'res_stage')
+        src = x
         x = x.contiguous(memory_format=CL)
         params = [t.contiguous(memory_format=CL) if t.dim() == 4 else t.contiguous() for t in params]
         saved, k = [], 0
@@ -1005,12 +1072,15 @@
             x = out
         ctx.save_for_backward(*saved, *params)
         ctx.cfg = (strides, dilation, has_ds)
+        ctx.mask_in = bool(mask_in)
         ctx.flipped = [take_flipped(t) if t.dim() == 4 else None for t in params]
-        return x
+        return chain_outputs(ctx, x, (src, ), chain)
 
     @staticmethod
     @once_differentiable
-    def backward(ctx, g):
+    def backward(ctx, g, galias=None):
+        if g is None:
+            return (galias, ) + (None, ) * (len(ctx.needs_input_grad) - 1)
         strides, dilation, has_ds = ctx.cfg
         nb = len(strides)
         saved, params = ctx.saved_tensors[:4 * nb], ctx.saved_tensors[4 * nb:]
@@ -1022,12 +1092,12 @@
         need = ctx.needs_input_grad
         grads = [None] * len(params)
         g = g.contiguous(memory_format=CL)
-        premasked = False
+        premasked = premasked_by(g, saved[4 * nb - 1])
         for i in range(nb - 1, -1, -1):
             x, h1, h2, out = saved[4 * i:4 * i + 4]
             k, stride, ds = offs[i], strides[i], has_ds[i]
             w1, b1, w2, b2, w3, b3 = params[k:k + 6]
-            pneed = need[4 + k:4 + k + (8 if ds else 6)]
+            pneed = need[6 + k:6 + k + (8 if ds else 6)]
             first = i == 0
             need_x = need[0] if first else True
             gm3 = g if premasked else _mask_raw(g, out)
@@ -1050,20 +1120,34 @@
             else:
                 gb1 = _colsum_raw(gm1)[1] if pneed[1] else None
             grads[k + 1] = gb1 if pneed[1] else None
-            acc = gm3
+            acc, acc2 = gm3, None
             if ds:
                 wd = params[k + 6]
                 if pneed[6]:
                     grads[k + 6] = _wgrad_raw(x, gm3, wd, stride, 0, 1)[0]
                 grads[k + 7] = gb3 if pneed[7] else None
-                acc = _dgrad_raw(gm3, wd, x.shape, stride, 0, 1, wT=flipped[k + 6]) if need_x else None
+                acc = None
+                if need_x and stride != 1 and _accum2_ok(w1, gm1.dtype):
+                    acc2 = _shortcut_dgrad_compact(gm3, wd, x.shape, stride)
+                if need_x and acc2 is None:
+                    acc = _dgrad_raw(gm3, wd, x.shape, stride, 0, 1, wT=flipped[k + 6])
             if need_x:
-                g = _dgrad_raw(gm1, w1, x.shape, 1, 0, 1, mask_src=None if first else x, accum=acc, wT=flipped[k],
-                               g_planes=gm1p)
+                join = galias if first else None
+                msk = x if (not first or ctx.mask_in) else None
+                if join is not None and (acc is not None or join.dtype != gm1.dtype or tuple(join.shape) != tuple(x.shape)):
+                    g = _dgrad_raw(gm1, w1, x.shape, 1, 0, 1, accum=acc, wT=flipped[k], g_planes=gm1p,
+                                   accum2=(acc2, stride) if acc2 is not None else None) + join
+                    g = g if msk is None else _mask_raw(g, msk)
+                else:
+                    g = _dgrad_raw(gm1, w1, x.shape, 1, 0, 1, mask_src=msk, wT=flipped[k], g_planes=gm1p,
+                                   accum=acc if join is None else join.contiguous(memory_format=CL),
+                                   accum2=(acc2, stride) if acc2 is not None else None)
                 premasked = not first
+                if first and msk is not None:
+                    tag_premasked(g, x)
             else:
-                g = None
-        return (g, None, None, None, *grads)
+                g = galias if first else None
+        return (g, None, None, None, None, None, *grads)
 
 
 def conv2d_bf16(x, weight, bias=None, stride=1, padding=0, dilation=1, relu=False, residual=None, res_up=False):
@@ -1360,17 +1444,18 @@
     return x.contiguous(memory_format=CL), weight.contiguous(memory_format=CL)
 
 
-def conv2d(x, weight, bias=None, stride=1, padding=0, dilation=1, relu=False, residual=None, residual_up=False, chain=False):
+def conv2d(x, weight, bias=None, stride=1, padding=0, dilation=1, relu=False, residual=None, residual_up=False, chain=False,
+           mask_in=False):
     if isinstance(stride, (tuple, list)):
         stride, padding, dilation = stride[0], padding[0], dilation[0]
     if x.size(1) % 8 != 0:
-        assert not chain
+        assert not chain and not mask_in
         stem = (STEM7 and x.size(1) == 3 and tuple(weight.shape) == (64, 3, 7, 7) and int(stride) == 2 and int(padding) == 3 and
                 int(dilation) == 1 and residual is None and not x.requires_grad and x.dtype == torch.float32 and x.is_cuda and
                 capi.lib().htd_conv2d_set_math(-1) == 1)
         x, weight = _pad_channels(x, weight, 4 if stem else 8)
     return Conv2dFunction.apply(x, weight, bias, residual, int(stride), int(padding), int(dilation), relu,
-                                bool(residual_up), bool(chain))
+                                bool(residual_up), bool(chain), bool(mask_in))
 
 
 def linear(x, weight, bias=None, relu=False):
diff --git a/htd_amd/detector/bricks.py b/htd_amd/detector/bricks.py
--- a/htd_amd/detector/bricks.py
+++ b/htd_amd/detector/bricks.py
@@ -9,12 +9,12 @@
 
 
 def dense_conv2d(x, weight, bias=None, stride=1, padding=0, dilation=1, relu=False, residual=None, residual_up=False,
-                 chain=False):
+                 chain=False, mask_in=False):
     from .. import dense
     if x.dtype == torch.bfloat16:
         y = dense.conv2d_bf16_autograd(x, weight, bias, stride, padding, dilation, relu, residual, residual_up)
         return (y, x) if chain else y
-    return dense.conv2d(x, weight, bias, stride, padding, dilation, relu, residual, residual_up, chain)
+    return dense.conv2d(x, weight, bias, stride, padding, dilation, relu, residual, residual_up, chain, mask_in)
 
 
 @CONV_LAYERS.register_module('Conv')
@@ -33,17 +33,18 @@
         self.weight.data = self.weight.data.contiguous(memory_format=CL)
         return self
 
-    def forward(self, x, relu=False, residual=None, weight=None, bias=None, residual_up=False, chain=False):
+    def forward(self, x, relu=False, residual=None, weight=None, bias=None, residual_up=False, chain=False, mask_in=False):
         w = self.weight if weight is None else weight
         b = self.bias if bias is None else bias
         if self.groups > 1:
             from .. import dense
-            assert residual is None and not chain
+            assert residual is None and not chain and not mask_in
             dt = x.dtype
             y = dense.grouped_conv2d(x.float() if dt != torch.float32 else x, w, b, self.stride[0], self.padding[0],
                                      self.dilation[0], self.groups, relu)
             return y.to(dt) if dt != torch.float32 else y
-        return dense_conv2d(x, w, b, self.stride[0], self.padding[0], self.dilation[0], relu, residual, residual_up, chain)
+        return dense_conv2d(x, w, b, self.stride[0], self.padding[0], self.dilation[0], relu, residual, residual_up, chain,
+                            mask_in)
 
 
 @CONV_LAYERS.register_module('ConvWS')
@@ -58,10 +59,10 @@
     def standardized_weight(self):
         return M.weight_standardize(self.weight, self.eps)
 
-    def forward(self, x, relu=False, residual=None, weight=None, bias=None, residual_up=False, chain=False):
+    def forward(self, x, relu=False, residual=None, weight=None, bias=None, residual_up=False, chain=False, mask_in=False):
         assert weight is None, 'ConvWS2d standardises its own weight'
         return super().forward(x, relu=relu, residual=residual, weight=self.standardized_weight(), bias=bias,
-                               residual_up=residual_up, chain=chain)
+                               residual_up=residual_up, chain=chain, mask_in=mask_in)
 
 
 def build_conv_layer(cfg, *args, **kwargs):
diff --git a/htd_amd/detector/fpn.py b/htd_amd/detector/fpn.py
--- a/htd_amd/detector/fpn.py
+++ b/htd_amd/detector/fpn.py
@@ -94,7 +94,10 @@
             for i in range(n - 1, -1, -1):
                 m = self.lateral_convs[i]
                 up = laterals[i + 1] if i + 1 < n else None
-                laterals[i] = m.conv(inputs[i + self.start_level], residual=up, residual_up=up is not None)
+                src = inputs[i + self.start_level]
+                mask_in = src.dtype == torch.float32 and src.requires_grad and torch.is_grad_enabled() and \
+                    getattr(src, '_htd_stage_out', False)
+                laterals[i] = m.conv(src, residual=up, residual_up=up is not None, **(dict(mask_in=True) if mask_in else {}))
                 if chain and i > 0:
                     outs_chain[i], laterals[i] = self.fpn_convs[i].conv(laterals[i], chain=True)
             if chain:
diff --git a/htd_amd/detector/resnet.py b/htd_amd/detector/resnet.py
--- a/htd_amd/detector/resnet.py
+++ b/htd_amd/detector/resnet.py
@@ -12,6 +12,7 @@
 
 CL = torch.channels_last
 FUSE_BF16_STAGE = os.environ.get('HTD_BF16_STAGE', '1') != '0'
+STAGE_CHAIN = os.environ.get('HTD_STAGE_CHAIN', '1') != '0'
 
 
 def conv_bn(conv, bn, x, relu=False, residual=None):
@@ -133,10 +134,11 @@
                 return False
         return True
 
-    def forward(self, x):
+    def forward(self, x, chain=False):
         if not x.is_cuda or x.dtype not in (torch.float32, torch.bfloat16) or not self._fusable() or \
                 (x.dtype == torch.bfloat16 and not FUSE_BF16_STAGE):
-            return super().forward(x)
+            out = super().forward(x)
+            return (out, x) if chain else out
         pairs = []
         for blk in self:
             pairs += [(blk.conv1.weight, blk.norm1), (blk.conv2.weight, blk.norm2), (blk.conv3.weight, blk.norm3)]
@@ -146,8 +148,15 @@
                                      (x.requires_grad or any(w.requires_grad for w, _ in pairs)),
                                      want_planes=x.dtype == torch.float32)
         strides, has_ds = tuple(blk.conv2_stride for blk in self), tuple(blk.downsample is not None for blk in self)
-        stage = ResStageFunction if x.dtype == torch.float32 else ResStageBf16Function
-        return stage.apply(x, strides, self[0].dilation, has_ds, *params)
+        if x.dtype != torch.float32:
+            out = ResStageBf16Function.apply(x, strides, self[0].dilation, has_ds, *params)
+            return (out, x) if chain else out
+        mask_in = STAGE_CHAIN and torch.is_grad_enabled() and x.requires_grad and getattr(x, '_htd_stage_out', False)
+        res = ResStageFunction.apply(x, strides, self[0].dilation, has_ds, bool(chain and mask_in), bool(mask_in), *params)
+        out, alias = res if (chain and mask_in) else (res, x)
+        if STAGE_CHAIN:
+            out._htd_stage_out = True
+        return (out, alias) if chain else out
 
 
 @BACKBONES.register_module()
@@ -252,7 +261,10 @@
             x = x.to(torch.bfloat16)
         outs = []
         for i, name in enumerate(self.res_layers):
-            x = getattr(self, name)(x)
+            if i > 0 and i - 1 in self.out_indices:
+                x, outs[-1] = getattr(self, name)(x, chain=True)
+            else:
+                x = getattr(self, name)(x)
             if i in self.out_indices:
                 outs.append(x)
         return tuple(outs)
diff --git a/include/htd_amd.h b/include/htd_amd.h
--- a/include/htd_amd.h
+++ b/include/htd_amd.h
@@ -173,6 +173,16 @@
 int htd_conv2d_bwd_data_x3h(const float *gy, const float *amax, const void *wplanesT, const float *mask_src,
                             const float *accum, float *gx, void *gxplanes, float *amax_out, int B, int H, int W,
                             int Ci, int Co, int kh, int kw, int pad, void *workspace, void *stream);
+int htd_conv2d_bwd_data_x3h_strided_compact(const float *gy, const float *amax, const void *wplanesT, float *gxc, float *amax_out,
+                                            int B, int H, int W, int Ci, int Co, int stride, void *workspace, void *stream);
+int htd_conv2d_bwd_data_x3h_joined(const float *gy, const float *amax, const void *wplanesT, const float *mask_src,
+                                   const float *accum, const float *accum2, int a2_step, float *gx, void *gxplanes,
+                                   float *amax_out, int B, int H, int W, int Ci, int Co, int kh, int kw, int pad,
+                                   void *workspace, void *stream);
+int htd_conv2d_bwd_data_x3q_joined(const float *gy, const void *gyplanes, const void *wplanesT, const float *mask_src,
+                                   const float *accum, const float *accum2, int a2_step, float *gx, void *gxplanes,
+                                   float *amax_out, int B, int H, int W, int Ci, int Co, int kh, int kw, int pad,
+                                   void *workspace, void *stream);
 
 int64_t htd_deform_columns_bytes(int B, int H, int W, int C, int kh, int kw, int stride, int pad, int dil);
 int htd_deform_im2col(const float *x, const float *offset, const float *mask, float *columns, int B,
```

Result: no change. 121.4 images/sec (-0.2%).
